# Dave-he/unet-watermark

Hardware: AMD Instinct MI355X
Metric: train_images_per_sec (higher is better)
Workload: dtype f32 storage and accumulation; the convolution products of the encoder and decoder layers (3x3, 7x7 stem, stride-2 and 1x1 layers: forward, data gradients, and the weight gradients of the stride-1 3x3 layers and the stem) as fp16x3 splits - every fp32 operand = two fp16 halves (22 mantissa bits), a*b; 1 GPU; Unet-resnet34 512x512 bs16/GPU train step: fwd + Dice + bwd + Adam (BASELINE.json configs[1]); global_batch=16, parallelism=dp1, grad_allreduce=none

## Files before the change

include/uwm.h:

```cpp
#ifndef UWM_H
#define UWM_H
#include <stddef.h>
#include <stdint.h>

#ifdef __cplusplus
extern "C" {
#endif

typedef struct uwm_model* uwm_handle;
typedef void* uwm_stream;

enum { UWM_ENC_RESNET18 = 18, UWM_ENC_RESNET34 = 34, UWM_ENC_RESNET50 = 50,
       UWM_ENC_EFFICIENTNET_B0 = 100, UWM_ENC_EFFICIENTNET_B1 = 101, UWM_ENC_EFFICIENTNET_B2 = 102,
       UWM_ENC_EFFICIENTNET_B3 = 103, UWM_ENC_EFFICIENTNET_B4 = 104, UWM_ENC_EFFICIENTNET_B5 = 105,
       UWM_ENC_EFFICIENTNET_B6 = 106, UWM_ENC_EFFICIENTNET_B7 = 107 };
enum { UWM_ARCH_UNET = 0, UWM_ARCH_UNETPLUSPLUS = 1 };
enum { UWM_T_F32 = 0, UWM_T_I64 = 1, UWM_T_U8 = 2, UWM_T_I32 = 3 };
enum { UWM_KIND_CONV_W = 0, UWM_KIND_BIAS = 1, UWM_KIND_BN_GAMMA = 2, UWM_KIND_BN_BETA = 3,
       UWM_KIND_BN_MEAN = 4, UWM_KIND_BN_VAR = 5 };
enum { UWM_ARENA_PARAM = 0, UWM_ARENA_BUFFER = 1 };
enum { UWM_PREC_F32 = 0, UWM_PREC_BF16X3 = 1, UWM_PREC_BF16X3_ALL = 2, UWM_PREC_F16X3 = 3, UWM_PREC_F16X3_ALL = 4,
       UWM_PREC_F16X1 = 5, UWM_PREC_F16X3_BWD2 = 6 };

typedef struct {
// ... 96 lines not shown
                            uwm_stream stream);
int  uwm_set_winograd(int on);
int  uwm_set_winograd_mode(uwm_handle h, int mode);
int  uwm_get_winograd_mode(uwm_handle h);
int  uwm_set_precision(uwm_handle h, int mode);
int  uwm_get_precision(uwm_handle h);
int  uwm_set_precision_fill(uwm_handle h, int min_workgroups);
int  uwm_set_routing_batch(uwm_handle h, int batch);
int  uwm_routing_enable(uwm_handle h, int on);
long long uwm_routing_dump(uwm_handle h, char* buf, long long cap, int clear);
int  uwm_set_drop_connect(uwm_handle h, const float* rowscale);
int  uwm_op_depthwise(int mode, const float* a, const float* b, int k, int stride, int pad_begin, int N, int H, int W, int C,
                      int Ho, int Wo, const float* addend, float* out, float* scratch, uwm_stream stream);
long long uwm_op_depthwise_scratch_floats(int k, int N, int C, int Ho, int Wo);
int  uwm_num_mbconv_blocks(uwm_handle h);
float uwm_mbconv_drop_rate(uwm_handle h, int block);
int  uwm_resize_threshold(const float* logits, int ld, int N, int h, int w, int H, int W, float threshold,
                          int apply_sigmoid, uint8_t* mask, float* resized, uwm_stream stream);

enum { UWM_MASK_WATERMARK = 0, UWM_MASK_TEXT = 1, UWM_MASK_MIXED = 2 };
enum { UWM_MORPH_RECT = 0, UWM_MORPH_ELLIPSE = 2 };
int    uwm_mask_element(int shape, int kw, int kh, uint8_t* out);
size_t uwm_mask_workspace_bytes(int N, int H, int W);
int    uwm_optimize_mask(const uint8_t* in, uint8_t* out, int N, int H, int W, int mask_type, long long* summary,
                         void* workspace, size_t workspace_bytes, uwm_stream stream);
int    uwm_op_morph(const uint8_t* in, uint8_t* out, int N, int H, int W, int dilate, int shape, int kw, int kh,
                    int iterations, void* workspace, size_t workspace_bytes, uwm_stream stream);
int    uwm_op_components(const uint8_t* in, int32_t* labels ,
                         int32_t* areas , int N, int H, int W,
                         void* workspace, size_t workspace_bytes, uwm_stream stream);

int  uwm_set_side_stream(uwm_handle h, int on);

int  uwm_prof_enable(int on);
int  uwm_prof_collect(double* out, int max_classes);
const char* uwm_prof_class_name(int cls);

int  uwm_debug_lookup(uwm_handle h, const char* key, long long* offset, long long* count);

typedef struct {
  const float* ptr; const float* scale; const float* shift;
  int C, H, W, up, relu;
} uwm_src;
int  uwm_op_preprocess_u8_nhwc4(const uint8_t* images, long long npix, int C, const float* mean, const float* std, float* out,
                                uwm_stream stream);
int  uwm_op_set_igemm_f16x3(int on);
int  uwm_op_conv(const uwm_src* s0, const uwm_src* s1, const float* w, int wrows, int Kpad, int kh, int kw, int stride,
                 int pad, int N, int Cout, const float* bias, float* y, double* stats, int cfg, uwm_stream stream);
int  uwm_op_dgrad(const float* dy, int N, int Ho, int Wo, int Cout, const float* wd, int Cin, int KpadD, int kh, int kw,
                  int stride, int pad, int H, int W, const float* addend, const float* mask, const float* mscale,
                  const float* mshift, float* dx, uwm_stream stream);
int  uwm_op_wgrad(const uwm_src* s0, const uwm_src* s1, const float* dy, int N, int Ho, int Wo, int Cout, int wrows,
                  int Kpad, int kh, int kw, int stride, int pad, float* dw, int force_igemm, uwm_stream stream);
int  uwm_op_pack_dgrad(const float* w, int Cout, int Kpad, int ntaps, int Cin, float* wd, int KpadD, int CoutP,
                       uwm_stream stream);
int  uwm_op_maxpool(const uwm_src* in, int N, float* out, uint8_t* idx, uwm_stream stream);
int  uwm_op_maxpool_backward(const float* gout, const uint8_t* idx, const float* addend, const uwm_src* in, int N,
                             float* gin, uwm_stream stream);
int  uwm_op_bn_backward(const float* g, const float* y, const float* mean, const float* rstd, const float* gamma,
                        double* scratch2c, float* dy, float* dgamma, float* dbeta, long long npix, int C, uwm_stream stream);
int  uwm_op_bn_backward_act(const float* g, const float* y, const float* mean, const float* rstd, const float* gamma,
                            const float* scale, const float* shift, const float* se_s, const float* gpool, int N, long long hw,
                            int C, double* scratch2c, float* dy, float* dgamma, float* dbeta, float* xmax, uwm_stream stream);
int  uwm_op_dgrad_upsplit(const float* dy, int N, int H, int W, int Cout, const float* wd, int C0, int C1, int KpadD,
                          float* gprev, const float* pmask, const float* pscale, const float* pshift, float* gskip,
                          uwm_stream stream);
int  uwm_op_upsplit(const float* dcat, int N, int H, int W, int C0, int C1, float* gprev, const float* pmask,
                    const float* pscale, const float* pshift, float* gskip, uwm_stream stream);
int  uwm_op_residual(const float* y, const float* s2, const float* b2, const float* id, const float* sd, const float* bd,
                     float* out, long long npix, int C, uwm_stream stream);

#ifdef __cplusplus
}
#endif
#endif
```

unet-watermark_amd/_lib.py:

```python
from __future__ import annotations

import ctypes as C
import os
import subprocess
import sys
from pathlib import Path

os.environ.setdefault("GPU_MAX_HW_QUEUES", "8")

_PKG_DIR = Path(__file__).resolve().parent
_CSRC = _PKG_DIR / "csrc"
LIB_PATH = _PKG_DIR / "libuwm.so"
SOURCES = ["conv_igemm.hip", "conv_patch.hip", "conv_patch16.hip", "conv_wino.hip", "conv_wino8.hip", "conv_wino_x3.hip", "conv_f16x3.hip", "conv_f16x3v2.hip", "conv_stem_f16x3.hip", "conv_up2.hip", "conv_up2_f16.hip", "conv_c16_f16.hip", "conv_gemm.hip", "conv_head.hip", "mbconv.hip", "wgrad_igemm.hip", "wgrad_patch.hip", "wgrad_wino.hip", "wgrad_f16x3.hip", "wgrad_c16.hip", "wgrad_gemm.hip", "wgrad_stem.hip", "elementwise.hip", "loss.hip", "mask_post.hip", "uwm_model.hip"]
HIP_ARCH = "gfx950"
EXTRA_FLAGS = {name: ["-Xclang", "-target-feature", "-Xclang", "-packed-fp32-ops"]
               for name in ("conv_f16x3.hip", "conv_f16x3v2.hip", "wgrad_f16x3.hip", "conv_stem_f16x3.hip")}


class uwm_unet_desc(C.Structure):
    _fields_ = [("encoder", C.c_int), ("in_channels", C.c_int), ("classes", C.c_int),
                ("decoder_channels", C.c_int * 5), ("bn_eps", C.c_float), ("bn_momentum", C.c_float), ("arch", C.c_int)]


class uwm_tensor_info(C.Structure):
# ... 49 lines not shown
    "uwm_adam_clip": (I, [P, P, P, P, L, F, F, F, F, F, L, F, F, P, P]),
    "uwm_adam_graph": (I, [P, P, P, P, L, P, P, P]),
    "uwm_adamw": (I, [P, P, P, P, L, F, F, F, F, F, L, F, P]),
    "uwm_adamw_clip": (I, [P, P, P, P, L, F, F, F, F, F, L, F, F, P, P]),
    "uwm_adamw_graph": (I, [P, P, P, P, L, P, P, P]),
    "uwm_sgd": (I, [P, P, P, L, F, F, F, L, F, F, P, P]),
    "uwm_scale": (I, [P, L, F, P]),
    "uwm_set_winograd": (I, [I]),
    "uwm_set_winograd_mode": (I, [P, I]),
    "uwm_get_winograd_mode": (I, [P]),
    "uwm_set_precision": (I, [P, I]),
    "uwm_get_precision": (I, [P]),
    "uwm_set_precision_fill": (I, [P, I]),
    "uwm_set_routing_batch": (I, [P, I]),
    "uwm_routing_enable": (I, [P, I]),
    "uwm_routing_dump": (L, [P, C.c_char_p, L, I]),
    "uwm_allreduce_grads": (I, [P, P, I, I, P]),
    "uwm_grad_arena": (P, [P]),
    "uwm_set_join_stream": (I, [P, P]),
    "uwm_set_drop_connect": (I, [P, P]),
    "uwm_op_depthwise": (I, [I, P, P, I, I, I, I, I, I, I, I, I, P, P, P, P]),
    "uwm_op_depthwise_scratch_floats": (L, [I, I, I, I, I]),
    "uwm_num_mbconv_blocks": (I, [P]),
    "uwm_mbconv_drop_rate": (F, [P, I]),
    "uwm_preprocess_u8": (I, [P, I, I, I, I, C.POINTER(C.c_float), C.POINTER(C.c_float), P, P, P]),
    "uwm_preprocess_mask_u8": (I, [P, I, I, I, I, P, P, P]),
    "uwm_resize_threshold": (I, [P, I, I, I, I, I, I, F, I, P, P, P]),
    "uwm_mask_element": (I, [I, I, I, P]),
    "uwm_mask_workspace_bytes": (Z, [I, I, I]),
    "uwm_optimize_mask": (I, [P, P, I, I, I, I, P, P, Z, P]),
    "uwm_op_morph": (I, [P, P, I, I, I, I, I, I, I, I, P, Z, P]),
    "uwm_op_components": (I, [P, P, P, I, I, I, P, Z, P]),
    "uwm_set_side_stream": (I, [P, I]),
    "uwm_prof_enable": (I, [I]),
    "uwm_prof_collect": (I, [C.POINTER(C.c_double), I]),
    "uwm_prof_class_name": (C.c_char_p, [I]),
    "uwm_debug_lookup": (I, [P, C.c_char_p, C.POINTER(L), C.POINTER(L)]),
    "uwm_op_set_igemm_f16x3": (I, [I]),
    "uwm_op_conv": (I, [C.POINTER(uwm_src), C.POINTER(uwm_src), P, I, I, I, I, I, I, I, I, P, P, P, I, P]),
    "uwm_op_dgrad": (I, [P, I, I, I, I, P, I, I, I, I, I, I, I, I, P, P, P, P, P, P]),
    "uwm_op_wgrad": (I, [C.POINTER(uwm_src), C.POINTER(uwm_src), P, I, I, I, I, I, I, I, I, I, I, P, I, P]),
    "uwm_op_pack_dgrad": (I, [P, I, I, I, I, P, I, I, P]),
    "uwm_op_maxpool": (I, [C.POINTER(uwm_src), I, P, P, P]),
    "uwm_op_maxpool_backward": (I, [P, P, P, C.POINTER(uwm_src), I, P, P]),
    "uwm_op_bn_backward": (I, [P, P, P, P, P, P, P, P, P, L, I, P]),
    "uwm_op_bn_backward_act": (I, [P, P, P, P, P, P, P, P, P, I, L, I, P, P, P, P, P, P]),
    "uwm_op_dgrad_upsplit": (I, [P, I, I, I, I, P, I, I, I, P, P, P, P, P, P]),
    "uwm_op_upsplit": (I, [P, I, I, I, I, I, P, P, P, P, P, P]),
    "uwm_op_residual": (I, [P, P, P, P, P, P, P, L, I, P]),
}

_lib = None


def build_library(force: bool = False, verbose: bool = False) -> Path:
    srcs = [_CSRC / s for s in SOURCES]
    hdrs = [_CSRC / "uwm_kernels.h", _PKG_DIR.parent / "include" / "uwm.h"] + sorted(_CSRC.glob("*.inc"))
    if LIB_PATH.exists() and not force:
        newest = max(p.stat().st_mtime for p in srcs + hdrs)
        if LIB_PATH.stat().st_mtime >= newest:
            return LIB_PATH
    hipcc = os.environ.get("HIPCC", "/opt/rocm/bin/hipcc")
    objdir = _PKG_DIR / "build"
    objdir.mkdir(exist_ok=True)
    procs = []
    hdr_m = max(p.stat().st_mtime for p in hdrs + [Path(__file__)])
    for s in srcs:
        o = objdir / (s.stem + ".o")
        if not force and o.exists() and o.stat().st_mtime >= max(s.stat().st_mtime, hdr_m):
            procs.append((None, None, o))
            continue
        cmd = [hipcc, f"--offload-arch={HIP_ARCH}", "-O3", "-std=c++17", "-fPIC"] + EXTRA_FLAGS.get(s.name, []) + ["-c", str(s), "-o", str(o)]
        procs.append((cmd, subprocess.Popen(cmd, stdout=subprocess.PIPE, stderr=subprocess.STDOUT), o))
    objs = []
    for cmd, p, o in procs:
        if p is None:
            objs.append(str(o))
            continue
        out, _ = p.communicate()
        if p.returncode != 0:
            raise RuntimeError(f"hipcc failed: {' '.join(cmd)}\n{out.decode(errors='replace')}")
        if verbose and out:
            sys.stderr.write(out.decode(errors="replace"))
        objs.append(str(o))
    cmd = [hipcc, f"--offload-arch={HIP_ARCH}", "-shared", "-fPIC", "-o", str(LIB_PATH)] + objs
    r = subprocess.run(cmd, stdout=subprocess.PIPE, stderr=subprocess.STDOUT)
    if r.returncode != 0:
        raise RuntimeError(f"link failed: {' '.join(cmd)}\n{r.stdout.decode(errors='replace')}")
    return LIB_PATH


def lib():
    global _lib
    if _lib is not None:
        return _lib
    global LIB_PATH
    if os.environ.get("UWM_LIB"):
        LIB_PATH = Path(os.environ["UWM_LIB"])
    if not LIB_PATH.exists():
        raise RuntimeError(
            f"{LIB_PATH} not found: the HIP extension is not built. Run `python -c 'import __graft_entry__ as g; "
            f"g.build()'` (needs hipcc). There is no CPU fallback for this path.")
    try:
        h = C.CDLL(str(LIB_PATH))
    except OSError as e:
        raise RuntimeError(f"cannot load {LIB_PATH}: {e}") from e
    for name, (res, args) in SIGNATURES.items():
        fn = getattr(h, name)
        fn.restype = res
        fn.argtypes = args
    _lib = h
    return _lib


def check(rc: int, exc=RuntimeError):
    if rc != 0:
        msg = lib().uwm_last_error().decode(errors="replace")
        raise exc(msg)


def stream_ptr(device=None) -> int:
    import torch
    return torch.cuda.current_stream(device).cuda_stream


class _NoGuard:
    def __enter__(self):
        return self

    def __exit__(self, *a):
        return False


_NOGUARD = _NoGuard()


def on_device(t):
    import torch
    if t.device.type == "cuda" and t.device.index is not None and t.device.index != torch.cuda.current_device():
        return torch.cuda.device(t.device)
# ... 15 lines not shown
```

unet-watermark_amd/csrc/conv_f16x3.hip:

```cpp
#include "uwm_kernels.h"

namespace uwm {

typedef float f4 __attribute__((ext_vector_type(4)));
typedef _Float16 h8 __attribute__((ext_vector_type(8)));
typedef _Float16 h4 __attribute__((ext_vector_type(4)));

#ifndef UWM_F16_ABL
#define UWM_F16_ABL 0
#endif
constexpr int kFT = 16, kFP = kFT + 2, kFPP = kFP * kFP;
constexpr int kFPix = 40;
constexpr int kFBuf = kFPP * kFPix;
constexpr int kFKs = 5;
constexpr int kFRounds = (kFPP * 4 + 255) / 256;

__host__ __device__ inline int f16x3_nj_(int rows) { return ((rows + 63) / 64) * 4; }
int f16x3_nj(int rows) { return f16x3_nj_(rows); }
size_t f16x3_bank_floats(int rows, int chans) {
  const size_t halfs = (size_t)(chans / 16) * kFKs * f16x3_nj(rows) * 2 * 64 * 8;
  return halfs / 2 + (size_t)f16x3_nj(rows) * 16;
}
size_t f16x3_rinv_off(int rows, int chans) { return f16x3_rinv_off_floats(rows, chans); }

// ... 110 lines not shown
      const int by = b >> 3, bx = b & 7;
      const int y = row0 + 2 * by, x = 2 * bx;
      const int ho = hb + y, wo = wb + x;
      if (ho < a.Ho && wo < a.Wo) {
        const float* q = R + (y * 16 + x) * kQLd + cq * 4;
        f4 v = (*(const f4*)q + *(const f4*)(q + kQLd) + *(const f4*)(q + 16 * kQLd) + *(const f4*)(q + 17 * kQLd)) * rs;
        const size_t o2 = (((size_t)n * (a.Ho >> 1) + (ho >> 1)) * (a.Wo >> 1) + (wo >> 1)) * a.up_c0 + co;
        if (a.up_mask) {
          f4 mk = *(const f4*)(a.up_mask + o2);
          const f4 yr = mk;
          if (a.up_mscale) mk = mk * msc + msh;
          v.x = mk.x > 0.f ? v.x : 0.f; v.y = mk.y > 0.f ? v.y : 0.f;
          v.z = mk.z > 0.f ? v.z : 0.f; v.w = mk.w > 0.f ? v.w : 0.f;
          if (bnb) { ps_ += v; pq_ += v * ((yr - bmu) * brs); }
        }
        if (a.up_accum) v += *(const f4*)(a.out_up + o2);
        *(f4*)(a.out_up + o2) = v;
      }
    }
  } else {
    const int c1n = a.Cout - a.up_c0;
#pragma unroll 4
    for (int r = 0; r < NROWS * 4; ++r) {
      const int p = r * 4 + sub;
      const int y = row0 + (p >> 4), x = p & 15;
      const int ho = hb + y, wo = wb + x;
      if (ho < a.Ho && wo < a.Wo)
        *(f4*)(a.out + (((size_t)n * a.Ho + ho) * a.Wo + wo) * c1n + (co - a.up_c0)) = *(const f4*)(R + (y * 16 + x) * kQLd + cq * 4) * rs;
    }
  }
}

__device__ __forceinline__ float clamp_h(float v) { return __builtin_amdgcn_fmed3f(v, -65504.f, 65504.f); }

template <int NJ, int NP = 3>
__global__ __launch_bounds__(256, (NJ == 1 ? 4 : 2)) void conv_f16x3_kernel(const ConvArgs a) {
  constexpr bool kOne = NJ == 1;
  constexpr int kCo = 16 * NJ;
  constexpr int kCQ = 4 * NJ, kSub = 64 / kCQ;
  extern __shared__ __attribute__((aligned(16))) _Float16 hsm[];

  const int tid = threadIdx.x, lane = tid & 63, wave = __builtin_amdgcn_readfirstlane(tid >> 6);
  const int px16 = lane & 15, g = lane >> 4;

  const unsigned nblk = gridDim.x, bid = blockIdx.x;
  const unsigned q8 = nblk >> 3, r8 = nblk & 7, xcd = bid & 7;
  unsigned tile = (xcd < r8 ? xcd * (q8 + 1) : r8 * (q8 + 1) + (xcd - r8) * q8) + (bid >> 3);
  const int tilesN = (a.Cout + kCo - 1) / kCo;
  const int tilesW = (a.Wo + kFT - 1) / kFT, tilesH = (a.Ho + kFT - 1) / kFT;
  const int tn = tile % tilesN; tile /= tilesN;
  const int tw = tile % tilesW; tile /= tilesW;
  const int th = tile % tilesH; const int n = tile / tilesH;
  const int n0 = tn * kCo, h0 = th * kFT, w0 = tw * kFT;
  const int nJ = a.wu_ncb;

  f4 acc[4][NJ];
#pragma unroll
  for (int i = 0; i < 4; ++i)
#pragma unroll
    for (int j = 0; j < NJ; ++j) acc[i][j] = (f4){0.f, 0.f, 0.f, 0.f};

  int goff[kFRounds];
  unsigned gflags = 0;
  int* const goff_s1 = (int*)(hsm + 2 * kFBuf);
#pragma unroll
  for (int rd = 0; rd < kFRounds; ++rd) {
    const int u = rd * 256 + tid;
    const bool act = u < kFPP * 4;
    const int pp = act ? (u >> 2) : 0;
    const int py = pp / kFP, pxx = pp - py * kFP;
    const int hl = h0 - 1 + py, wl = w0 - 1 + pxx;
    const bool ok = act && hl >= 0 && hl < a.Hl && wl >= 0 && wl < a.Wl;
    const int hc = min(max(hl, 0), a.Hl - 1), wc = min(max(wl, 0), a.Wl - 1);
    goff[rd] = ((n * a.s0.H + (hc >> a.s0.up)) * a.s0.W + (wc >> a.s0.up)) * a.s0.C;
    if (!kOne && a.C0 < a.Ctot) goff_s1[rd * 256 + tid] = ((n * a.s1.H + (hc >> a.s1.up)) * a.s1.W + (wc >> a.s1.up)) * a.s1.C;
    gflags |= (ok ? 1u : 0u) << rd;
  }
  float xs = 1.f;
  if (a.xmax) {
    float mx = a.xmax[lane & 31];
#pragma unroll
    for (int d = 16; d >= 1; d >>= 1) mx = fmaxf(mx, __shfl_xor(mx, d));
    if (mx > 0.f && mx < 3.0e38f) { int e; (void)frexpf(mx, &e); xs = ldexpf(1.f, 14 - e); }
  }
  constexpr int kWR = kFRounds - 1;
  f4 pv[kWR], pvX = {0.f, 0.f, 0.f, 0.f}, psc = {1.f, 1.f, 1.f, 1.f}, psh = {0.f, 0.f, 0.f, 0.f};
  float pfloor = -3.0e38f;
  const bool has_x = tid < kFPP * 4 - kWR * 256;
  const float* lsp = nullptr;
  auto chunk_src = [&](int cc) {
    const int c = cc * 16;
    const bool first = c < a.C0;
    if (c == a.C0 && a.C0 < a.Ctot) {
#pragma unroll
      for (int rd = 0; rd < kFRounds; ++rd) goff[rd] = goff_s1[rd * 256 + tid];
    }
    lsp = (first ? a.s0.ptr : a.s1.ptr) + (first ? c : c - a.C0) + (tid & 3) * 4;
  };
  auto coef_load = [&](int cc) {
    const int c = cc * 16;
    const bool first = c < a.C0;
    const Src& s = first ? a.s0 : a.s1;
    const int cl = (first ? c : c - a.C0) + (tid & 3) * 4;
    pfloor = s.relu ? 0.f : -3.0e38f;
    if (s.scale != nullptr) { psc = *(const f4*)(s.scale + cl); psh = *(const f4*)(s.shift + cl); }
    else { psc = (f4){1.f, 1.f, 1.f, 1.f}; psh = (f4){0.f, 0.f, 0.f, 0.f}; pfloor = -3.0e38f; }
  };
  auto store_unit = [&](int buf, int rd, f4 raw) {
    f4 v = raw * psc + psh;
    v.x = fmaxf(v.x, pfloor); v.y = fmaxf(v.y, pfloor); v.z = fmaxf(v.z, pfloor); v.w = fmaxf(v.w, pfloor);
    v = v * xs;
    if (!((gflags >> rd) & 1u)) v = (f4){0.f, 0.f, 0.f, 0.f};
    h4 hi, lo;
#pragma unroll
    for (int e = 0; e < 4; ++e) {
      const float x = clamp_h(v[e]);
      const _Float16 h = (_Float16)x;
      hi[e] = h; lo[e] = (_Float16)(x - (float)h);
    }
    const int u = rd * 256 + tid;
    _Float16* d = hsm + buf * kFBuf + (u >> 2) * kFPix + (u & 3) * 4;
    *(h4*)d = hi;
    *(h4*)(d + 16) = lo;
  };

  const _Float16* const wb = (const _Float16*)a.wu + (size_t)(n0 / 16) * 1024 + lane * 8;
  const int nchunk = a.Ctot >> 4, nsteps = nchunk * kFKs;
  constexpr int dbg = UWM_F16_ABL;
  auto w_load = [&](int t, h8 (&whi)[NJ], h8 (&wlo)[NJ]) {
    if ((dbg & 2) && t > 0) return;
    const _Float16* p = wb + (size_t)t * nJ * 1024;
#pragma unroll
    for (int j = 0; j < NJ; ++j) { whi[j] = *(const h8*)(p + j * 1024); wlo[j] = *(const h8*)(p + j * 1024 + 512); }
  };
  const int pbase = ((wave * 4) * kFP + px16) * kFPix + (g & 1) * 8;
  const int ghi = g >> 1;
  auto mma_step = [&](int ks, const _Float16* pc, const h8 (&whi)[NJ], const h8 (&wlo)[NJ]) {
    const int slot0 = 2 * ks, slot1 = 2 * ks + 1 > 8 ? 8 : 2 * ks + 1;
    const int off0 = ((slot0 / 3) * kFP + slot0 % 3) * kFPix, off1 = ((slot1 / 3) * kFP + slot1 % 3) * kFPix;
    const _Float16* pp = pc + pbase + (ghi ? off1 : off0);
    h8 xh[4], xl[4];
#pragma unroll
    for (int i = 0; i < 4; ++i) {
      if (dbg & 4) { xh[i] = whi[i % NJ]; xl[i] = wlo[i % NJ]; continue; }
      xh[i] = *(const h8*)(pp + i * kFP * kFPix); xl[i] = *(const h8*)(pp + i * kFP * kFPix + 16);
    }
    if (dbg & 1) { acc[0][0][0] += (float)xh[0][0] + (float)xl[1][1] + (float)whi[NJ > 1 ? NJ - 2 : 0][2] + (float)wlo[NJ - 1][3] + (float)xh[2][0] + (float)xh[3][0]; return; }
#pragma unroll
    for (int i = 0; i < 4; ++i)
#pragma unroll
      for (int j = 0; j < NJ; ++j) acc[i][j] = __builtin_amdgcn_mfma_f32_16x16x32_f16(whi[j], xh[i], acc[i][j], 0, 0, 0);
    if (NP >= 3) {
#pragma unroll
      for (int i = 0; i < 4; ++i)
#pragma unroll
        for (int j = 0; j < NJ; ++j) acc[i][j] = __builtin_amdgcn_mfma_f32_16x16x32_f16(whi[j], xl[i], acc[i][j], 0, 0, 0);
    }
    if (NP >= 2) {
#pragma unroll
      for (int i = 0; i < 4; ++i)
#pragma unroll
        for (int j = 0; j < NJ; ++j) acc[i][j] = __builtin_amdgcn_mfma_f32_16x16x32_f16(wlo[j], xh[i], acc[i][j], 0, 0, 0);
    }
  };

  h8 wA_hi[NJ], wA_lo[NJ], wB_hi[NJ], wB_lo[NJ];
  w_load(0, wA_hi, wA_lo);
  chunk_src(0);
#pragma unroll
  for (int rd = 0; rd < kWR; ++rd) pv[rd] = *(const f4*)(lsp + goff[rd]);
  if (has_x) pvX = *(const f4*)(lsp + goff[kWR]);
  coef_load(0);
#pragma unroll
  for (int rd = 0; rd < kWR; ++rd) store_unit(0, rd, pv[rd]);
  if (has_x) store_unit(0, kWR, pvX);
  if (!kOne && nchunk > 1) {
    chunk_src(1);
#pragma unroll
    for (int rd = 0; rd < kWR; ++rd) pv[rd] = *(const f4*)(lsp + goff[rd]);
    if (has_x) pvX = *(const f4*)(lsp + goff[kWR]);
  }
  __syncthreads();

  for (int cc = 0; cc < nchunk; cc += 2) {
#pragma unroll
    for (int hh = 0; hh < (kOne ? 1 : 2); ++hh) {
      const int c = cc + hh, cur = hh, nxt = hh ^ 1;
      const bool more1 = c + 1 < nchunk;
      if (!kOne) {
        coef_load(more1 ? c + 1 : c);
        chunk_src(c + 2 < nchunk ? c + 2 : nchunk - 1);
      }
      const _Float16* pc = hsm + cur * kFBuf;
      __builtin_amdgcn_sched_barrier(0);
#pragma unroll
      for (int ks = 0; ks < kFKs; ++ks) {
        const int t = c * kFKs + ks;
        const int tnext = t + 1 < nsteps ? t + 1 : t;
        if (((hh * kFKs + ks) & 1) == 0) { w_load(tnext, wB_hi, wB_lo); mma_step(ks, pc, wA_hi, wA_lo); }
        else { w_load(tnext, wA_hi, wA_lo); mma_step(ks, pc, wB_hi, wB_lo); }
        if (!(dbg & 8) && !kOne) {
          store_unit(nxt, ks, pv[ks]);
          pv[ks] = *(const f4*)(lsp + goff[ks]);
        }
        __builtin_amdgcn_sched_group_barrier(0x020, 2 * NJ, 0);
        __builtin_amdgcn_sched_group_barrier(0x100, 8, 0);
#pragma unroll
        for (int q = 0; q < 4 * NJ; ++q) {
          __builtin_amdgcn_sched_group_barrier(0x008, NP, 0);
          __builtin_amdgcn_sched_group_barrier(0x002, 3, 0);
        }
        __builtin_amdgcn_sched_group_barrier(0x200, 2, 0);
        __builtin_amdgcn_sched_group_barrier(0x020, 1, 0);
        __builtin_amdgcn_sched_barrier(0);
      }
      if (!(dbg & 8) && !kOne && has_x) {
        if (more1) store_unit(nxt, kWR, pvX);
        pvX = *(const f4*)(lsp + goff[kWR]);
      }
      __syncthreads();
    }
  }
  if (dbg & 16) { if (acc[0][0][0] + acc[1][1][1] + acc[2][NJ > 1 ? NJ - 2 : 0][2] + acc[3][NJ - 1][3] == 123.456f) a.out[0] = 1.f; return; }

  constexpr int kQLd = kOne ? 20 : 68;
  float* const R = (float*)hsm + wave * 64 * kQLd;
#pragma unroll
  for (int i = 0; i < 4; ++i)
#pragma unroll
    for (int j = 0; j < NJ; ++j) *(f4*)(R + (i * 16 + px16) * kQLd + j * 16 + g * 4) = acc[i][j];
  __syncthreads();
  const float* rinv = (const float*)a.wu + a.wu_rinv_off;
  const float ixs = 1.f / xs;
  const bool do_stats = a.ssum != nullptr;
  const bool bnb = a.bnb_mean != nullptr;
  const int cq = lane & (kCQ - 1), sub = lane / kCQ;
  const int co = n0 + cq * 4;
  const bool cok = co < a.Cout;
  f4 ps_ = {0.f, 0.f, 0.f, 0.f}, pq_ = ps_;
  const int stat_c = a.out_up != nullptr ? a.up_c0 : a.Cout;
  if (NJ == 4 && a.out_up != nullptr) {
    f4 rs = {0.f, 0.f, 0.f, 0.f};
    if (cok) rs = *(const f4*)(rinv + co) * ixs;
    f16x3_split_epilogue<4>(a, R, kQLd, 0, n, h0 + wave * 4, w0, n0, lane, rs, ps_, pq_);
  } else {
    f4 rs = {0.f, 0.f, 0.f, 0.f}, bmu = rs, brs = rs, bia = rs, msc = {1.f, 1.f, 1.f, 1.f}, msh = rs;
    if (cok) rs = *(const f4*)(rinv + co) * ixs;
    if (bnb && cok) { bmu = *(const f4*)(a.bnb_mean + co); brs = *(const f4*)(a.bnb_rstd + co); }
    if (a.bias && cok) bia = *(const f4*)(a.bias + co);
    if (a.mscale && cok) { msc = *(const f4*)(a.mscale + co); msh = *(const f4*)(a.mshift + co); }
#pragma unroll 4
    for (int r = 0; r < 64 / kSub; ++r) {
      const int p = r * kSub + sub;
      const int ho = h0 + wave * 4 + (p >> 4), wo = w0 + (p & 15);
      if (ho < a.Ho && wo < a.Wo && cok) {
        const size_t o = (((size_t)n * a.Ho + ho) * a.Wo + wo) * a.Cout + co;
        f4 v = *(const f4*)(R + p * kQLd + cq * 4) * rs + bia;
        if (a.addend) v += *(const f4*)(a.addend + o);
        f4 yr = {0.f, 0.f, 0.f, 0.f};
        if (a.mask) {
          f4 mk = *(const f4*)(a.mask + o);
          yr = mk;
          if (a.mscale) mk = mk * msc + msh;
          v.x = mk.x > 0.f ? v.x : 0.f; v.y = mk.y > 0.f ? v.y : 0.f;
          v.z = mk.z > 0.f ? v.z : 0.f; v.w = mk.w > 0.f ? v.w : 0.f;
        }
        *(f4*)(a.out + o) = v;
        if (a.bnb_y) yr = *(const f4*)(a.bnb_y + o);
        ps_ += v; pq_ += bnb ? v * ((yr - bmu) * brs) : v * v;
      }
    }
  }
  if (do_stats) {
#pragma unroll
    for (int e = 0; e < 4; ++e) {
      float sv = ps_[e], qv = pq_[e];
#pragma unroll
      for (int d = kCQ; d < 64; d <<= 1) { sv += __shfl_xor(sv, d); qv += __shfl_xor(qv, d); }
      ps_[e] = sv; pq_[e] = qv;
    }
    __syncthreads();
    float* red = (float*)hsm;
    if (sub == 0) {
#pragma unroll
      for (int e = 0; e < 4; ++e) { red[(wave * 64 + cq * 4 + e) * 2] = ps_[e]; red[(wave * 64 + cq * 4 + e) * 2 + 1] = pq_[e]; }
    }
    __syncthreads();
    if (tid < kCo) {
      const int c1 = n0 + tid;
      if (c1 < stat_c) {
        double sv = 0.0, qv = 0.0;
#pragma unroll
        for (int w = 0; w < 4; ++w) { sv += (double)red[(w * 64 + tid) * 2]; qv += (double)red[(w * 64 + tid) * 2 + 1]; }
        const size_t srep_off = a.srep > 1 ? (size_t)(blockIdx.x & (unsigned)(a.srep - 1)) * a.sstride : 0;
        atomicAdd(a.ssum + srep_off + c1, sv);
        atomicAdd(a.ssq + srep_off + c1, qv);
      }
    }
  }
}

template <int NP = 3>
__global__ __launch_bounds__(512, 1) void conv_f16x3s_kernel(const ConvArgs a) {
  extern __shared__ __attribute__((aligned(16))) _Float16 hsm[];

  const int tid = threadIdx.x, lane = tid & 63, wave = __builtin_amdgcn_readfirstlane(tid >> 6);
  const bool is_mma = wave < 4;
  const int mw = wave & 3;
  const int ltid = tid & 255;
  const int px16 = lane & 15, g = lane >> 4;

  const unsigned nblk = gridDim.x, bid = blockIdx.x;
  const unsigned q8 = nblk >> 3, r8 = nblk & 7, xcd = bid & 7;
  unsigned tile = (xcd < r8 ? xcd * (q8 + 1) : r8 * (q8 + 1) + (xcd - r8) * q8) + (bid >> 3);
  const int tilesN = (a.Cout + 63) / 64;
  const int tilesW = (a.Wo + kFT - 1) / kFT, tilesH = (a.Ho + kFT - 1) / kFT;
  const int tn = tile % tilesN; tile /= tilesN;
  const int tw = tile % tilesW; tile /= tilesW;
  const int th = tile % tilesH; const int n = tile / tilesH;
  const int n0 = tn * 64, h0 = th * kFT, w0 = tw * kFT;
  const int nJ = a.wu_ncb;
  const int nchunk = a.Ctot >> 4, nsteps = nchunk * kFKs;

  float xs = 1.f;
  if (a.xmax) {
    float mx = a.xmax[lane & 31];
#pragma unroll
    for (int d = 16; d >= 1; d >>= 1) mx = fmaxf(mx, __shfl_xor(mx, d));
    if (mx > 0.f && mx < 3.0e38f) { int e; (void)frexpf(mx, &e); xs = ldexpf(1.f, 14 - e); }
  }

  f4 acc[4][4];
#pragma unroll
  for (int i = 0; i < 4; ++i)
#pragma unroll
    for (int j = 0; j < 4; ++j) acc[i][j] = (f4){0.f, 0.f, 0.f, 0.f};

  if (!is_mma) {
    int goff0[kFRounds], goff1[kFRounds];
    unsigned gflags = 0;
#pragma unroll
    for (int rd = 0; rd < kFRounds; ++rd) {
      const int u = rd * 256 + ltid;
      const bool act = u < kFPP * 4;
      const int pp = act ? (u >> 2) : 0;
      const int py = pp / kFP, pxx = pp - py * kFP;
      const int hl = h0 - 1 + py, wl = w0 - 1 + pxx;
      const bool ok = act && hl >= 0 && hl < a.Hl && wl >= 0 && wl < a.Wl;
      const int hc = min(max(hl, 0), a.Hl - 1), wc = min(max(wl, 0), a.Wl - 1);
      goff0[rd] = ((n * a.s0.H + (hc >> a.s0.up)) * a.s0.W + (wc >> a.s0.up)) * a.s0.C;
      goff1[rd] = a.C0 < a.Ctot ? ((n * a.s1.H + (hc >> a.s1.up)) * a.s1.W + (wc >> a.s1.up)) * a.s1.C : goff0[rd];
      gflags |= ((ok ? 1u : 0u) | (act ? 2u : 0u)) << (2 * rd);
    }
    struct Stage { f4 pv[kFRounds]; f4 sc, sh; int relu; bool has; };
    auto patch_load = [&](int cc, Stage& st) {
      const int c = cc * 16;
      const bool first = c < a.C0;
      const Src& s = first ? a.s0 : a.s1;
      st.relu = s.relu;
      const int cl = (first ? c : c - a.C0) + (ltid & 3) * 4;
      st.has = s.scale != nullptr;
      if (st.has) { st.sc = *(const f4*)(s.scale + cl); st.sh = *(const f4*)(s.shift + cl); }
      const float* sp = s.ptr + cl;
#pragma unroll
      for (int rd = 0; rd < kFRounds; ++rd) st.pv[rd] = *(const f4*)(sp + (first ? goff0[rd] : goff1[rd]));
    };
    auto patch_store = [&](int buf, const Stage& st) {
#pragma unroll
      for (int rd = 0; rd < kFRounds; ++rd) {
        f4 v = st.pv[rd];
        if (st.has) {
          v = v * st.sc + st.sh;
          if (st.relu) { v.x = fmaxf(v.x, 0.f); v.y = fmaxf(v.y, 0.f); v.z = fmaxf(v.z, 0.f); v.w = fmaxf(v.w, 0.f); }
        }
        v = v * xs;
        if (!((gflags >> (2 * rd)) & 1u)) v = (f4){0.f, 0.f, 0.f, 0.f};
        if ((gflags >> (2 * rd)) & 2u) {
          h4 hi, lo;
#pragma unroll
          for (int e = 0; e < 4; ++e) {
            const float x = clamp_h(v[e]);
            const _Float16 h = (_Float16)x;
            hi[e] = h; lo[e] = (_Float16)(x - (float)h);
          }
          const int u = rd * 256 + ltid;
          _Float16* d = hsm + buf * kFBuf + (u >> 2) * kFPix + (u & 3) * 4;
          *(h4*)d = hi;
          *(h4*)(d + 16) = lo;
        }
      }
    };
    Stage sA, sB;
    patch_load(0, sA);
    patch_load(nchunk > 1 ? 1 : 0, sB);
    patch_store(0, sA);
    __syncthreads();
    for (int cc = 0; cc < nchunk; cc += 2) {
      {
        const int c2 = cc + 2 < nchunk ? cc + 2 : nchunk - 1;
        if (cc + 1 < nchunk) patch_store(1, sB);
        patch_load(c2, sA);
        __syncthreads();
      }
      {
        const int c3 = cc + 3 < nchunk ? cc + 3 : nchunk - 1;
        if (cc + 2 < nchunk) patch_store(0, sA);
        patch_load(c3, sB);
        __syncthreads();
      }
    }
  } else {
    const _Float16* const wb = (const _Float16*)a.wu + (size_t)(n0 / 16) * 1024 + lane * 8;
    auto w_load = [&](int t, h8 (&whi)[4], h8 (&wlo)[4]) {
      const _Float16* p = wb + (size_t)t * nJ * 1024;
#pragma unroll
      for (int j = 0; j < 4; ++j) { whi[j] = *(const h8*)(p + j * 1024); wlo[j] = *(const h8*)(p + j * 1024 + 512); }
    };
    const int pbase = ((mw * 4) * kFP + px16) * kFPix + (g & 1) * 8;
    const int ghi = g >> 1;
    auto x_load = [&](int ks, const _Float16* pc, h8 (&xh)[4], h8 (&xl)[4]) {
      const int slot0 = 2 * ks, slot1 = 2 * ks + 1 > 8 ? 8 : 2 * ks + 1;
      const int off0 = ((slot0 / 3) * kFP + slot0 % 3) * kFPix, off1 = ((slot1 / 3) * kFP + slot1 % 3) * kFPix;
      const _Float16* pp = pc + pbase + (ghi ? off1 : off0);
#pragma unroll
      for (int i = 0; i < 4; ++i) { xh[i] = *(const h8*)(pp + i * kFP * kFPix); xl[i] = *(const h8*)(pp + i * kFP * kFPix + 16); }
    };
    auto mma = [&](const h8 (&whi)[4], const h8 (&wlo)[4], const h8 (&xh)[4], const h8 (&xl)[4]) {
#pragma unroll
      for (int i = 0; i < 4; ++i)
#pragma unroll
        for (int j = 0; j < 4; ++j) acc[i][j] = __builtin_amdgcn_mfma_f32_16x16x32_f16(whi[j], xh[i], acc[i][j], 0, 0, 0);
      if (NP >= 3) {
#pragma unroll
        for (int i = 0; i < 4; ++i)
#pragma unroll
          for (int j = 0; j < 4; ++j) acc[i][j] = __builtin_amdgcn_mfma_f32_16x16x32_f16(whi[j], xl[i], acc[i][j], 0, 0, 0);
      }
      if (NP >= 2) {
#pragma unroll
        for (int i = 0; i < 4; ++i)
// ... 12 lines not shown
#pragma unroll
        for (int ks = 0; ks < kFKs; ++ks) {
          const int t = c * kFKs + ks;
          const int tnext = t + 1 < nsteps ? t + 1 : t;
          x_load(ks, pc, xh, xl);
          if (((hh * kFKs + ks) & 1) == 0) { w_load(tnext, wB_hi, wB_lo); __builtin_amdgcn_sched_barrier(0); mma(wA_hi, wA_lo, xh, xl); }
          else { w_load(tnext, wA_hi, wA_lo); __builtin_amdgcn_sched_barrier(0); mma(wB_hi, wB_lo, xh, xl); }
          __builtin_amdgcn_sched_barrier(0);
        }
        __syncthreads();
      }
    }
  }

  constexpr int kQLd = 68;
  if (is_mma) {
    float* const Rw = (float*)hsm + mw * 64 * kQLd;
#pragma unroll
    for (int i = 0; i < 4; ++i)
#pragma unroll
      for (int j = 0; j < 4; ++j) *(f4*)(Rw + (i * 16 + px16) * kQLd + j * 16 + g * 4) = acc[i][j];
  }
  __syncthreads();
  const float* const R = (const float*)hsm + mw * 64 * kQLd;
  const float* rinv = (const float*)a.wu + a.wu_rinv_off;
  const float ixs = 1.f / xs;
  const bool do_stats = a.ssum != nullptr;
  const bool bnb = a.bnb_mean != nullptr;
  const int cq = lane & 15, sub = lane >> 4;
  const int co = n0 + cq * 4;
  const bool cok = co < a.Cout;
  const int phalf = (wave >> 2) * 32;
  f4 ps_ = {0.f, 0.f, 0.f, 0.f}, pq_ = ps_;
  const int stat_c = a.out_up != nullptr ? a.up_c0 : a.Cout;
  if (a.out_up != nullptr) {
    f4 rs = {0.f, 0.f, 0.f, 0.f};
    if (cok) rs = *(const f4*)(rinv + co) * ixs;
    f16x3_split_epilogue<2>(a, R, kQLd, phalf >> 4, n, h0 + mw * 4, w0, n0, lane, rs, ps_, pq_);
  } else {
    f4 rs = {0.f, 0.f, 0.f, 0.f}, bmu = rs, brs = rs, bia = rs, msc = {1.f, 1.f, 1.f, 1.f}, msh = rs;
    if (cok) rs = *(const f4*)(rinv + co) * ixs;
    if (bnb && cok) { bmu = *(const f4*)(a.bnb_mean + co); brs = *(const f4*)(a.bnb_rstd + co); }
    if (a.bias && cok) bia = *(const f4*)(a.bias + co);
    if (a.mscale && cok) { msc = *(const f4*)(a.mscale + co); msh = *(const f4*)(a.mshift + co); }
#pragma unroll 4
    for (int r = 0; r < 8; ++r) {
      const int p = phalf + r * 4 + sub;
      const int ho = h0 + mw * 4 + (p >> 4), wo = w0 + (p & 15);
      if (ho < a.Ho && wo < a.Wo && cok) {
        const size_t o = (((size_t)n * a.Ho + ho) * a.Wo + wo) * a.Cout + co;
        f4 v = *(const f4*)(R + p * kQLd + cq * 4) * rs + bia;
        if (a.addend) v += *(const f4*)(a.addend + o);
        f4 yr = {0.f, 0.f, 0.f, 0.f};
        if (a.mask) {
          f4 mk = *(const f4*)(a.mask + o);
          yr = mk;
          if (a.mscale) mk = mk * msc + msh;
          v.x = mk.x > 0.f ? v.x : 0.f; v.y = mk.y > 0.f ? v.y : 0.f;
          v.z = mk.z > 0.f ? v.z : 0.f; v.w = mk.w > 0.f ? v.w : 0.f;
        }
        *(f4*)(a.out + o) = v;
        if (a.bnb_y) yr = *(const f4*)(a.bnb_y + o);
        ps_ += v; pq_ += bnb ? v * ((yr - bmu) * brs) : v * v;
      }
    }
  }
  if (do_stats) {
#pragma unroll
    for (int e = 0; e < 4; ++e) {
      float sv = ps_[e], qv = pq_[e];
      sv += __shfl_xor(sv, 16); qv += __shfl_xor(qv, 16);
      sv += __shfl_xor(sv, 32); qv += __shfl_xor(qv, 32);
      ps_[e] = sv; pq_[e] = qv;
    }
    __syncthreads();
    float* red = (float*)hsm;
    if (sub == 0) {
#pragma unroll
      for (int e = 0; e < 4; ++e) { red[(wave * 64 + cq * 4 + e) * 2] = ps_[e]; red[(wave * 64 + cq * 4 + e) * 2 + 1] = pq_[e]; }
    }
    __syncthreads();
    if (tid < 64) {
      const int c1 = n0 + tid;
      if (c1 < stat_c) {
        double sv = 0.0, qv = 0.0;
#pragma unroll
        for (int w = 0; w < 8; ++w) { sv += (double)red[(w * 64 + tid) * 2]; qv += (double)red[(w * 64 + tid) * 2 + 1]; }
        const size_t srep_off = a.srep > 1 ? (size_t)(blockIdx.x & (unsigned)(a.srep - 1)) * a.sstride : 0;
        atomicAdd(a.ssum + srep_off + c1, sv);
        atomicAdd(a.ssq + srep_off + c1, qv);
      }
    }
  }
}

bool conv_f16x3_applicable(const ConvArgs& a) {
  return a.wu != nullptr && a.ntaps == 9 && a.kw == 3 && a.smul == 1 && a.sdiv == 1 && (a.rmul == 1 ? a.off == -1 : a.off == 1) &&
         ((a.Ctot & 31) == 0 || (a.Ctot == 16 && a.C0 == 16 && a.Cout <= 16 && !a.out_up)) && (a.C0 & 15) == 0 && (a.s0.C & 3) == 0 && (a.s1.C & 3) == 0 && (a.Cout & 3) == 0 && a.Cout >= 16 &&
         a.Hl == a.Ho && a.Wl == a.Wo && a.Ho >= 8 && a.Wo >= 16 && a.Hl < 32768 && a.Wl < 32768 &&
         (!a.out_up || (((a.Ho | a.Wo) & 1) == 0 && (a.up_c0 & 63) == 0 && a.up_c0 <= a.Cout)) &&
         (size_t)a.N * a.s0.H * a.s0.W * a.s0.C < (1ull << 31) && (size_t)a.N * a.s1.H * a.s1.W * a.s1.C < (1ull << 31);
}

template <int NJ, int NP>
static hipError_t launch_f3(const ConvArgs& a, hipStream_t st, dim3 grid, size_t lds) {
  static DevOnce lds_attr;
  { hipError_t e = lds_attr.set_max_lds((const void*)conv_f16x3_kernel<NJ, NP>, lds); if (e != hipSuccess) return e; }
  UWM_LAUNCH(42, a.flops, a.bytes, (conv_f16x3_kernel<NJ, NP>), grid, dim3(256), lds, st, a);
  return hipGetLastError();
}
template <int NP>
static hipError_t launch_f3s(const ConvArgs& a, hipStream_t st, dim3 grid, size_t lds) {
  static DevOnce lds_attr;
  { hipError_t e = lds_attr.set_max_lds((const void*)conv_f16x3s_kernel<NP>, lds); if (e != hipSuccess) return e; }
  UWM_LAUNCH(42, a.flops, a.bytes, (conv_f16x3s_kernel<NP>), grid, dim3(512), lds, st, a);
  return hipGetLastError();
}
hipError_t launch_conv_f16x3(const ConvArgs& a, hipStream_t st, int variant) {
  if (a.wu_layout == 1) return launch_conv_f16x3v2(a, st, variant >= 4 ? variant : 0);
  if (variant >= 4) return hipErrorInvalidValue;
  if (!conv_f16x3_applicable(a)) return hipErrorInvalidValue;
  if (a.out_up && (a.addend || a.mask || a.bias || a.bnb_y || (a.ssum && !a.bnb_mean) || (a.up_c0 < a.Cout && !a.out))) return hipErrorInvalidValue;
  if (a.bnb_mean && (!a.ssum || !a.ssq || !a.bnb_rstd || !(a.out_up ? a.up_mask : (a.bnb_y ? a.bnb_y : a.mask)) || a.up_accum)) return hipErrorInvalidValue;
  const int tilesN = (a.Cout + 63) / 64;
  const int tilesW = (a.Wo + kFT - 1) / kFT, tilesH = (a.Ho + kFT - 1) / kFT;
  const size_t main_lds = (size_t)2 * kFBuf * sizeof(_Float16) + 6 * 256 * sizeof(int), q_lds = (size_t)4 * 64 * 68 * sizeof(float);
  const size_t lds = main_lds > q_lds ? main_lds : q_lds;
  static const bool force4 = dbg_flag("UWM_F16X3_4WAVE"), force8 = dbg_flag("UWM_F16X3_8WAVE");
  const long wgs = (long)route_N(a) * tilesH * tilesW * tilesN;
  const int np = (a.nprod >= 1 && a.nprod <= 3) ? a.nprod : 3;
  if (a.Ctot == 16) {
    const size_t lds1 = (size_t)kFBuf * sizeof(_Float16);
    return np == 3 ? launch_f3<1, 3>(a, st, dim3((unsigned)(a.N * tilesH * tilesW)), lds1)
         : np == 2 ? launch_f3<1, 2>(a, st, dim3((unsigned)(a.N * tilesH * tilesW)), lds1) : launch_f3<1, 1>(a, st, dim3((unsigned)(a.N * tilesH * tilesW)), lds1);
  }
  const bool four = variant == 1 || variant == 3 || (variant != 2 && (force4 || (!force8 && wgs >= 2L * device_cu_count())));
  if (variant == 3 && a.out_up) return hipErrorInvalidValue;
  const bool fwd_alone = a.rmul == 1 && !a.xmax;
  const bool narrow = !a.out_up && (a.Cout <= 32 ? four : (fwd_alone && variant == 0 && wgs < device_cu_count()));
  if (variant == 3 || (variant == 0 && narrow)) {
    const dim3 g((unsigned)(a.N * tilesH * tilesW * ((a.Cout + 31) / 32)));
    return np == 3 ? launch_f3<2, 3>(a, st, g, lds) : np == 2 ? launch_f3<2, 2>(a, st, g, lds) : launch_f3<2, 1>(a, st, g, lds);
  }
  const dim3 g((unsigned)(a.N * tilesH * tilesW * tilesN));
  if (four) return np == 3 ? launch_f3<4, 3>(a, st, g, lds) : np == 2 ? launch_f3<4, 2>(a, st, g, lds) : launch_f3<4, 1>(a, st, g, lds);
  return np == 3 ? launch_f3s<3>(a, st, g, lds) : np == 2 ? launch_f3s<2>(a, st, g, lds) : launch_f3s<1>(a, st, g, lds);
}

}
```

unet-watermark_amd/csrc/conv_igemm.hip:

```cpp
#include "uwm_kernels.h"
#include <cstdlib>
#include <cstdio>

namespace uwm {

typedef float f4 __attribute__((ext_vector_type(4)));

__device__ __forceinline__ unsigned fdiv(unsigned n, FastDiv f) {
  return f.d <= 1 ? n : __umulhi(n, f.mg);
}

constexpr float kIgWScale = 4096.f;
typedef _Float16 ig_h8 __attribute__((ext_vector_type(8)));
template <int BM, int BN, int WM, int WN, bool PC = false, bool F16 = false>
__global__ __launch_bounds__(256, 2) void conv_igemm_kernel(const ConvArgs a) {
  constexpr int MI = BM / WM / 16;
  constexpr int NI = BN / WN / 16;
  constexpr int XR = BM / 32;
  constexpr int WR = (BN + 31) / 32;
  static_assert(WM * WN == 4, "4 waves");
  extern __shared__ __attribute__((aligned(16))) float smem[];
  float* const Xs = smem;
  float* const Ws = smem + 2 * BM * 32;

// ... 332 lines not shown
  int dev = 0; (void)hipGetDevice(&dev);
  if (dev < 0 || dev >= 64) return 256;
  if (!cus[dev] && (hipDeviceGetAttribute(&cus[dev], hipDeviceAttributeMultiprocessorCount, dev) != hipSuccess || cus[dev] <= 0)) cus[dev] = 256;
  return cus[dev];
}

bool conv_epilogue_carries_bnb(const ConvArgs& a) {
  if (a.ig16 && a.prec != 2 && (conv_c16_f16_applicable(a) || conv_c32_f16_applicable(a))) return true;
  if (a.prec == 2) return !a.out_up && (a.wu_layout == 1 ? conv_f16x3v2_applicable(a) : conv_f16x3_applicable(a));
  if (a.bnb_y) {
    if (a.out_up || a.prec == 1) return false;
    static const bool no_y = dbg_flag("UWM_NO_BNB_Y");
    if (no_y || conv_up2_applicable(a) || conv_head_applicable(a) || conv_head_dgrad_applicable(a) || conv_patch16_applicable(a)) return false;
    if (wino_mode_of(a.wino) != 0 && conv_wino_applicable(a)) return true;
    return !conv_patch_applicable(a);
  }
  static const bool no_up2 = dbg_flag("UWM_NO_UP2");
  if (a.out_up) return (!no_up2 && conv_up2_dgrad_applicable(a)) || (a.prec == 1 ? conv_wino_x3_applicable(a) : conv_wino_applicable(a));
  static const bool no_head = dbg_flag("UWM_NO_CONV_HEAD");
  if (!no_up2 && conv_up2_applicable(a)) return false;
  if (!no_head && conv_head_applicable(a)) return false;
  if (!no_head && conv_head_dgrad_applicable(a)) return true;
  if (wino_mode_of(a.wino) != 0 && conv_wino_applicable(a) && !conv_patch16_applicable(a))
    return a.prec == 1 || !conv_wino8_applicable(a);
  if (conv_patch16_applicable(a)) return true;
  if (conv_patch_applicable(a)) return false;
  static const bool no_igemm_bnb = dbg_flag("UWM_NO_IGEMM_BNB");
  return !no_igemm_bnb;
}

hipError_t launch_conv(const ConvArgs& a, hipStream_t st, int force_cfg) {
  if (a.M <= 0 || a.Cout <= 0 || (a.Cout & 3) || (a.Kpad & 31) || (a.Ctot & 3) || (a.C0 & 3)) return hipErrorInvalidValue;
  int cfg = force_cfg;
  static const bool trace = dbg_flag("UWM_TRACE_CONV");
  if (trace)
    fprintf(stderr, "conv %s N=%d Ctot=%d(C0=%d up=%d) Cout=%d Ho=%d Wo=%d Hl=%d Wl=%d taps=%d smul=%d sdiv=%d wino=%d gflop=%.2f\n",
            a.rmul < 0 ? "dgrad" : "fwd", a.N, a.Ctot, a.C0, a.s0.up, a.Cout, a.Ho, a.Wo, a.Hl, a.Wl, a.ntaps, a.smul, a.sdiv,
            (int)(cfg < 0 && wino_mode_of(a.wino) != 0 && conv_wino_applicable(a)), a.flops * 1e-9);
  if (cfg == 700) return launch_conv_up2(a, st);
  if (cfg == 710 || (cfg < 0 && a.ig16 && a.prec != 2 && conv_c16_f16_applicable(a))) return launch_conv_c16_f16(a, st);
  if (cfg == 711 || (cfg < 0 && a.ig16 && a.prec != 2 && conv_c32_f16_applicable(a))) return launch_conv_c32_f16(a, st);
  if (cfg >= 800 && cfg < 1000) return launch_conv_gemm(a, st, cfg - 800);
  if (cfg == 500) return launch_conv_head(a, st);
  if ((cfg >= 600 && cfg <= 607) || (cfg < 0 && a.prec == 2)) return launch_conv_f16x3(a, st, cfg >= 600 ? cfg - 600 : 0);
  if (cfg == 400) return launch_conv_wino_x3(a, st);
  if (cfg >= 300) return launch_conv_wino(a, st, cfg - 300);
  if (a.out_up) {
    static const bool no_up2d = dbg_flag("UWM_NO_UP2");
    if (cfg < 0 && !no_up2d && conv_up2_dgrad_applicable(a)) return launch_conv_up2_dgrad(a, st);
    if (a.prec == 1) return launch_conv_wino_x3(a, st);
    return conv_wino_applicable(a) ? launch_conv_wino(a, st) : hipErrorInvalidValue;
  }
  if (cfg == 200) return launch_conv_patch16(a, st);
  static const bool no_up2 = dbg_flag("UWM_NO_UP2");
  if (cfg < 0 && !no_up2 && conv_up2_applicable(a)) return launch_conv_up2(a, st);
  static const bool no_head = dbg_flag("UWM_NO_CONV_HEAD");
  if (cfg < 0 && !no_head && conv_head_applicable(a)) return launch_conv_head(a, st);
  if (cfg < 0 && !no_head && conv_head_dgrad_applicable(a)) return launch_conv_head_dgrad(a, st);
  if (cfg < 0 && wino_mode_of(a.wino) != 0 && conv_wino_applicable(a) && !conv_patch16_applicable(a))
    return a.prec == 1 ? launch_conv_wino_x3(a, st) : launch_conv_wino(a, st);
  if (cfg >= 100) return launch_conv_patch(a, st, cfg - 100);
  if (cfg < 0 && conv_patch16_applicable(a)) return launch_conv_patch16(a, st);
  if (cfg < 0 && conv_patch_applicable(a)) {
    const long sp = (long)route_N(a) * ((a.Ho + 7) / 8) * ((a.Wo + 15) / 16);
    int bn = a.Cout >= 128 ? 128 : (a.Cout > 32 ? 64 : (a.Cout > 16 ? 32 : 16));
    if (bn == 128 && sp * ((a.Cout + 127) / 128) < 512) bn = 64;
// ... 37 lines not shown
```

unet-watermark_amd/csrc/elementwise.hip:

```cpp
#include "uwm_kernels.h"
#include <vector>
#include <mutex>
#include <cstdlib>

namespace uwm {

typedef float f4 __attribute__((ext_vector_type(4)));
static constexpr int kMaxBlocks = 256 * 8;

static inline unsigned nblocks(size_t work, int per_block) {
  size_t b = (work + per_block - 1) / per_block;
  if (b > (size_t)kMaxBlocks) b = kMaxBlocks;
  if (b < 1) b = 1;
  return (unsigned)b;
}

__global__ void nchw_to_nhwc4_kernel(const float* __restrict__ x, float* __restrict__ y, int C, size_t HW,
                                     size_t total, int CP) {
  for (size_t i = blockIdx.x * (size_t)blockDim.x + threadIdx.x; i < total; i += (size_t)gridDim.x * blockDim.x) {
    const size_t n = i / HW, p = i - n * HW;
    const float* xp = x + n * C * HW + p;
    float* yp = y + i * CP;
    for (int c0 = 0; c0 < CP; c0 += 4) {
      f4 v;
// ... 354 lines not shown
    if (xmax) amax4(o);
    *(f4*)(dy + i * 4) = o;
  }
  if (xmax) {
#pragma unroll
    for (int d = 32; d >= 1; d >>= 1) amax = fmaxf(amax, __shfl_xor(amax, d));
    if ((threadIdx.x & 63) == 0) wmax[threadIdx.x >> 6] = amax;
    __syncthreads();
    if (threadIdx.x == 0) {
      const float mx = fmaxf(fmaxf(wmax[0], wmax[1]), fmaxf(wmax[2], wmax[3]));
      if (mx > 0.f) atomicMax((unsigned*)xmax + (blockIdx.x & 31), __float_as_uint(mx));
    }
  }
}
hipError_t launch_bn_bwd_apply(const float* g, const float* y, const float* mean, const float* rstd, const float* gamma,
                               const double* dgamma, const double* dbeta, float* dy, float* gamma_grad, float* beta_grad,
                               size_t npix, int C, hipStream_t st, const double* rep, int nrep, int rep_stride, hipEvent_t done, float* xmax) {
  const size_t n4 = npix * C / 4;
  unsigned nb = nblocks(n4, 256 * 4);
  const unsigned q = (unsigned)(C / 4);
  unsigned unit = q;
  { unsigned a = q, b = 256; while (b) { unsigned t = a % b; a = b; b = t; } unit = q / a; }
  nb = ((nb + unit - 1) / unit) * unit;
  if ((size_t)nb * 256 < q) nb = ((q + 255) / 256 + unit - 1) / unit * unit;
  if (done)
    hipExtLaunchKernelGGL(bn_bwd_apply_kernel, dim3(nb), dim3(256), 0, st, nullptr, done, 0, g, y, mean, rstd, gamma, dgamma,
                          dbeta, dy, gamma_grad, beta_grad, n4, C, (float)(1.0 / (double)npix), rep, rep ? (nrep < 1 ? 1 : nrep) : 0, rep_stride, xmax);
  else
    hipLaunchKernelGGL(bn_bwd_apply_kernel, dim3(nb), dim3(256), 0, st, g, y, mean, rstd, gamma, dgamma,
                       dbeta, dy, gamma_grad, beta_grad, n4, C, (float)(1.0 / (double)npix), rep, rep ? (nrep < 1 ? 1 : nrep) : 0, rep_stride, xmax);
  return hipGetLastError();
}

__global__ void upsplit_prev_kernel(const float* __restrict__ dcat, int H, int W, int C0, int Ct, float* __restrict__ gprev,
                                    const float* __restrict__ pmask, const float* __restrict__ pscale,
                                    const float* __restrict__ pshift, size_t total, int accumulate) {
  const int C4 = C0 / 4, H2 = H / 2, W2 = W / 2;
  for (size_t i = blockIdx.x * (size_t)blockDim.x + threadIdx.x; i < total; i += (size_t)gridDim.x * blockDim.x) {
    const int c = (int)(i % C4) * 4;
    size_t p = i / C4;
    const int w2 = (int)(p % W2); p /= W2;
    const int h2 = (int)(p % H2); const int n = (int)(p / H2);
    const float* b = dcat + ((size_t)((size_t)n * H + 2 * h2) * W + 2 * w2) * Ct + c;
    f4 g = *(const f4*)b + *(const f4*)(b + Ct) + *(const f4*)(b + (size_t)W * Ct) + *(const f4*)(b + (size_t)W * Ct + Ct);
    if (pmask) {
      f4 z = *(const f4*)(pmask + i * 4);
      if (pscale) z = z * *(const f4*)(pscale + c) + *(const f4*)(pshift + c);
      g.x = z.x > 0.f ? g.x : 0.f; g.y = z.y > 0.f ? g.y : 0.f; g.z = z.z > 0.f ? g.z : 0.f; g.w = z.w > 0.f ? g.w : 0.f;
    }
    if (accumulate) g += *(const f4*)(gprev + i * 4);
    *(f4*)(gprev + i * 4) = g;
  }
}
__global__ void upsplit_skip_kernel(const float* __restrict__ dcat, int C0, int C1, float* __restrict__ gskip, size_t total) {
  const int C4 = C1 / 4, Ct = C0 + C1;
  for (size_t i = blockIdx.x * (size_t)blockDim.x + threadIdx.x; i < total; i += (size_t)gridDim.x * blockDim.x) {
    const int c = (int)(i % C4) * 4;
    const size_t p = i / C4;
    *(f4*)(gskip + i * 4) = *(const f4*)(dcat + p * Ct + C0 + c);
  }
}
hipError_t launch_upsplit(const float* dcat, int N, int H, int W, int C0, int C1, float* gprev, const float* pmask,
                          const float* pscale, const float* pshift, float* gskip, hipStream_t st, int accumulate_prev) {
  const size_t t0 = (size_t)N * (H / 2) * (W / 2) * (C0 / 4);
  hipLaunchKernelGGL(upsplit_prev_kernel, dim3(nblocks(t0, 256)), dim3(256), 0, st, dcat, H, W, C0, C0 + C1, gprev, pmask,
                     pscale, pshift, t0, accumulate_prev);
// ... 427 lines not shown
```

unet-watermark_amd/csrc/uwm_abi.inc:

```
extern "C" {

const char* uwm_last_error(void) { return g_err; }
int uwm_version(void) { return 1; }

int uwm_create(const uwm_unet_desc* desc, uwm_handle* out) {
  if (!desc || !out) return fail("uwm_create: null argument");
  uwm_model* m = new uwm_model();
  m->desc = *desc;
  if (m->desc.bn_eps <= 0.f) m->desc.bn_eps = 1e-5f;
  if (m->desc.bn_momentum <= 0.f) m->desc.bn_momentum = 0.1f;
  if (build_model(m)) { delete m; return 1; }
  const char* e = getenv("UWM_SIDE_STREAM");
  m->use_side = e ? atoi(e) : 1;
  if (const char* pe = getenv("UWM_PRECISION")) {
    static const char* names[7] = {"f32", "bf16x3", "bf16x3_all", "f16x3", "f16x3_all", "f16x1", "f16x3_bwd2"};
    int found = -1;
    for (int i = 0; i < 7; ++i) if (!strcmp(pe, names[i]) || (pe[0] == '0' + i && !pe[1])) found = i;
    if (found < 0) { delete m; return fail("uwm_create: UWM_PRECISION=%s is not a precision mode (f32 | bf16x3 | bf16x3_all | f16x3 | f16x3_all | f16x1 | f16x3_bwd2 or 0..6)", pe); }
    m->prec = found; m->plan.prec = found; m->prec_from_env = found != UWM_PREC_F32;
  }
  if (const char* pf = getenv("UWM_F16X3_MIN_WGS")) m->f3_min_wgs = atoi(pf) > 0 ? atoi(pf) : 0;
  m->wino_mode = winograd_mode();
  m->plan.wino_mode = m->wino_mode;
  *out = m; return 0;
}
void uwm_destroy(uwm_handle h) {
  if (!h) return;
  if (h->ev_fork) (void)hipEventDestroy(h->ev_fork);
  if (h->ev_join) (void)hipEventDestroy(h->ev_join);
  if (h->ev_pack) (void)hipEventDestroy(h->ev_pack);
  if (h->ev_disp) (void)hipEventDestroy(h->ev_disp);
  if (h->side) (void)hipStreamDestroy(h->side);
  delete h;
}

long long uwm_param_arena_floats(uwm_handle h) { return h ? h->param_floats : 0; }
long long uwm_buffer_arena_floats(uwm_handle h) { return h ? h->buffer_floats : 0; }
long long uwm_param_count(uwm_handle h) { return h ? h->param_count : 0; }
int uwm_num_tensors(uwm_handle h) { return h ? (int)h->infos.size() : 0; }
int uwm_tensor_info_get(uwm_handle h, int i, uwm_tensor_info* out) {
  if (!h || !out || i < 0 || i >= (int)h->infos.size()) return fail("uwm_tensor_info_get: bad index %d", i);
  *out = h->infos[i]; return 0;
}
int uwm_logits_channels(uwm_handle h) { return h ? h->CP : 0; }
int uwm_num_stages(uwm_handle h) { return h ? h->nstages : 0; }
int uwm_stage_range(uwm_handle h, int stage, long long* b, long long* e) {
// ... 329 lines not shown
}
int uwm_op_components(const uint8_t* in, int32_t* labels, int32_t* areas, int N, int H, int W, void* ws, size_t ws_bytes,
                      uwm_stream stream) {
  if (!in || !labels || !areas) return fail("uwm_op_components: null argument");
  if (((uintptr_t)labels | (uintptr_t)areas) & 3) return fail("uwm_op_components: labels and areas must be 4-byte aligned");
  if (mask_shape_check("uwm_op_components", N, H, W, ws, ws_bytes)) return 1;
  LCHK(launch_mask_components(in, labels, areas, N, H, W, ws, (hipStream_t)stream));
  return 0;
}
int uwm_preprocess_u8(const uint8_t* images, int N, int H, int W, int C, const float* mean, const float* std, const int* flags,
                      float* out_nchw, uwm_stream stream) {
  if (!images || !mean || !std || !out_nchw || N < 1 || H < 1 || W < 1 || C < 1 || C > 4) return fail("uwm_preprocess_u8: bad argument");
  for (int c = 0; c < C; ++c) if (!(std[c] > 0.f)) return fail("uwm_preprocess_u8: std[%d] must be positive", c);
  LCHK(launch_preprocess_u8(images, N, H, W, C, mean, std, flags, out_nchw, (hipStream_t)stream));
  return 0;
}
int uwm_preprocess_mask_u8(const uint8_t* masks, int N, int H, int W, int threshold, const int* flags, uint8_t* out,
                           uwm_stream stream) {
  if (!masks || !out || N < 1 || H < 1 || W < 1) return fail("uwm_preprocess_mask_u8: bad argument");
  LCHK(launch_preprocess_mask(masks, N, H, W, threshold, flags, out, (hipStream_t)stream));
  return 0;
}
int uwm_scale(float* p, long long n, float s, uwm_stream stream) {
  if (!p || n < 1) return fail("uwm_scale: bad argument");
  LCHK(launch_scale(p, (size_t)n, s, (hipStream_t)stream));
  return 0;
}

int uwm_set_side_stream(uwm_handle h, int on) {
  if (!h) return fail("uwm_set_side_stream: null handle");
  h->use_side = on != 0; return 0;
}

int uwm_prof_enable(int on) { prof_enable(on != 0); return 0; }
int uwm_prof_collect(double* out, int max_classes) {
  if (!out || max_classes < kProfClasses) return fail("uwm_prof_collect: need room for %d classes (4 doubles each)", (int)kProfClasses);
  prof_collect(out); return kProfClasses;
}
const char* uwm_prof_class_name(int cls) { return prof_class_name(cls); }

int uwm_debug_lookup(uwm_handle h, const char* key, long long* off, long long* count) {
  if (!h || !key || !off || !count) return fail("uwm_debug_lookup: null argument");
  const Plan& p = h->plan;
  const std::string k(key);
  if (k == "fixed") { *off = 0; *count = (long long)h->fixed_floats; return 0; }
  if (k.rfind("bnf:", 0) == 0) {
    for (auto& b : h->bns) if (b.name == k.substr(4)) { *off = (long long)(b.f_off + 2 * (size_t)b.C); *count = 2LL * b.C; return 0; }
    return fail("uwm_debug_lookup: unknown BatchNorm %s", k.c_str() + 4);
  }
  if (k.rfind("wu:", 0) == 0 || k.rfind("wud:", 0) == 0 || k.rfind("wd:", 0) == 0) {
    const std::string name = k.substr(k.find(':') + 1);
    for (auto& cv : h->convs) if (cv.name == name) {
      if (k[1] == 'd') { *off = (long long)cv.wd_off; *count = cv.dgrad ? (long long)cv.CinP * cv.KpadD : 0; }
      else if (k[2] == 'd') { *off = (long long)cv.wud_off; *count = cv.wud_off ? (long long)std::max(wino_weights_floats(cv.CinP, cv.CoutP), cv.f3_d() ? f16x3_bank_floats(cv.CinP, cv.CoutP) : 0) : 0; }
      else { *off = (long long)cv.wu_off; *count = (long long)cv.wu_floats; }
      return 0;
    }
    return fail("uwm_debug_lookup: unknown conv %s", name.c_str());
  }
  if (p.N == 0) return fail("uwm_debug_lookup: no plan yet");
  const int N = p.N, H = p.H, W = p.W;
  auto conv_geo = [&](int ci, long long* cnt) { *cnt = (long long)N * p.oh[ci] * p.ow[ci] * h->convs[ci].CoutP; };
  if (k.rfind("y:", 0) == 0 || k.rfind("g:", 0) == 0) {
    const std::string name = k.substr(2);
    for (size_t i = 0; i < h->convs.size(); ++i) if (h->convs[i].name == name) {
      if ((int)i == h->head) return fail("uwm_debug_lookup: head output is the caller's logits buffer");
// ... 255 lines not shown
  if (!s0 || !dy || !dw) return fail("uwm_op_wgrad: null argument");
  WgradArgs a; memset(&a, 0, sizeof(a));
  a.s0 = to_src(s0); a.C0 = a.s0.C;
  if (s1) { a.s1 = to_src(s1); a.Ctot = a.C0 + a.s1.C; } else { a.s1 = a.s0; a.Ctot = a.C0; }
  a.dy = dy; a.dw = dw; a.wrows = wrows; a.Kpad = Kpad; a.ntaps = kh * kw; a.kw = kw;
  a.N = N; a.Ho = Ho; a.Wo = Wo; a.Cout = Cout; a.M = N * Ho * Wo;
  a.Hl = a.s0.H << a.s0.up; a.Wl = a.s0.W << a.s0.up; a.stride = stride; a.pad = pad;
  a.dv_ctot = make_fastdiv(a.Ctot); a.dv_kw = make_fastdiv(a.kw);
  a.force_igemm = force_igemm;
  if ((force_igemm & 0xff) == 6 || (force_igemm & 0xff) == 7) {
    static float* xm = nullptr;
    if (!xm) HIPCHK(hipMalloc((void**)&xm, 32 * sizeof(float)));
    LCHK(launch_absmax32(dy, (size_t)N * Ho * Wo * Cout, xm, (hipStream_t)stream));
    a.prec = 2; a.xmax = xm;
  }
  LCHK(launch_wgrad(a, (hipStream_t)stream));
  return 0;
}
int uwm_op_pack_dgrad(const float* w, int Cout, int Kpad, int ntaps, int Cin, float* wd, int KpadD, int CoutP,
                      uwm_stream stream) {
  if (!w || !wd) return fail("uwm_op_pack_dgrad: null argument");
  LCHK(launch_pack_dgrad(w, Cout, Kpad, ntaps, Cin, wd, KpadD, CoutP, (hipStream_t)stream));
  return 0;
}
int uwm_op_bn_backward(const float* g, const float* y, const float* mean, const float* rstd, const float* gamma,
                       double* scratch2c, float* dy, float* dgamma, float* dbeta, long long npix, int C, uwm_stream stream) {
  if (!g || !y || !mean || !rstd || !gamma || !scratch2c || !dy || !dgamma || !dbeta || npix < 1) return fail("uwm_op_bn_backward: bad argument");
  hipStream_t st = (hipStream_t)stream;
  HIPCHK(hipMemsetAsync(scratch2c, 0, 2 * (size_t)C * sizeof(double), st));
  LCHK(launch_bn_bwd_reduce(g, y, mean, rstd, scratch2c, scratch2c + C, (size_t)npix, C, st));
  LCHK(launch_bn_bwd_apply(g, y, mean, rstd, gamma, scratch2c, scratch2c + C, dy, dgamma, dbeta, (size_t)npix, C, st));
  return 0;
}
int uwm_op_bn_backward_act(const float* g, const float* y, const float* mean, const float* rstd, const float* gamma,
                           const float* scale, const float* shift, const float* se_s, const float* gpool, int N, long long hw,
                           int C, double* scratch2c, float* dy, float* dgamma, float* dbeta, float* xmax, uwm_stream stream) {
  if (!g || !y || !mean || !rstd || !gamma || !scale || !shift || !scratch2c || !dy || !dgamma || !dbeta || N < 1 || hw < 1 ||
      C < 4 || (C & 3) || (!se_s != !gpool))
    return fail("uwm_op_bn_backward_act: bad argument");
  hipStream_t st = (hipStream_t)stream;
  HIPCHK(hipMemsetAsync(scratch2c, 0, 2 * (size_t)C * sizeof(double), st));
  if (xmax) HIPCHK(hipMemsetAsync(xmax, 0, 32 * sizeof(float), st));
  LCHK(launch_bn_bwd_act(g, y, mean, rstd, gamma, scale, shift, se_s, gpool, N, (size_t)hw, scratch2c, scratch2c + C, dy, dgamma,
                         dbeta, C, st, xmax));
  return 0;
}
int uwm_op_upsplit(const float* dcat, int N, int H, int W, int C0, int C1, float* gprev, const float* pmask,
                   const float* pscale, const float* pshift, float* gskip, uwm_stream stream) {
  if (!dcat || !gprev) return fail("uwm_op_upsplit: null argument");
  LCHK(launch_upsplit(dcat, N, H, W, C0, C1, gprev, pmask, pscale, pshift, gskip, (hipStream_t)stream));
  return 0;
}
int uwm_op_residual(const float* y, const float* s2, const float* b2, const float* id, const float* sd, const float* bd,
                    float* out, long long npix, int C, uwm_stream stream) {
  if (!y || !s2 || !b2 || !id || !out) return fail("uwm_op_residual: null argument");
  LCHK(launch_residual(y, s2, b2, id, sd, bd, out, (size_t)npix, C, (hipStream_t)stream));
  return 0;
}
int uwm_op_maxpool_backward(const float* gout, const uint8_t* idx, const float* addend, const uwm_src* in, int N, float* gin,
                            uwm_stream stream) {
  if (!gout || !idx || !in || !gin) return fail("uwm_op_maxpool_backward: null argument");
  Src s = to_src(in);
  LCHK(launch_maxpool_bwd(gout, idx, addend, s, gin, N, (s.H - 1) / 2 + 1, (s.W - 1) / 2 + 1, (hipStream_t)stream));
  return 0;
}
int uwm_op_maxpool(const uwm_src* in, int N, float* out, uint8_t* idx, uwm_stream stream) {
// ... 8 lines not shown
```

unet-watermark_amd/csrc/uwm_backward.inc:

```
static int do_backward(uwm_model* m, const float* dlogits, float* ws, int sb, int se, hipStream_t st) {
  const Plan& p = m->plan;
  const int N = p.N, H = p.H, W = p.W;
  Ctx c{m, ws, st, N};
  c.wst = (m->use_side && m->side) ? m->side : st;
  const int h1 = H / 2, w1 = W / 2;
  int sh[4], sw[4];
  { int h = H / 4, w = W / 4; for (int s = 0; s < 4; ++s) { if (s > 0) { h /= 2; w /= 2; } sh[s] = h; sw[s] = w; } }
  std::vector<size_t> first_blk(4); { size_t b = 0; for (int s = 0; s < 4; ++s) { first_blk[s] = b; b += m->stages[s].size(); } }
  const bool effnet = !m->mb.empty();
  auto feat_blk = [&](int s) -> size_t { return effnet ? (size_t)m->feat_blk[s] : first_blk[s] + m->stages[s].size() - 1; };
  auto feat_src = [&](int s) {
    return mk_src(c.F(p.xn[feat_blk(s)]), m->featC[s], sh[s], sw[s]);
  };
  auto feat_mask = [&](const Src& f) -> const float* { return effnet ? nullptr : f.ptr; };
  Src f1 = effnet ? mk_src(c.F(p.stem_a), m->f1C, h1, w1) : lazy_src(c, m->stem, h1, w1);

  std::vector<char>& out_sums = m->out_sums;
  if (sb <= 0 || out_sums.size() != first_blk[3] + m->stages[3].size()) out_sums.assign(first_blk[3] + m->stages[3].size(), 0);
  if (sb <= 0 || m->dy_max_made.size() != m->bns.size()) m->dy_max_made.assign(m->bns.size(), 0);
  m->disp_cov.clear();
  if (sb <= 0) m->rq = ReduceQueue();
  if (sb <= 0 && se > 0) {
    HIPCHK(hipMemsetAsync(m->grads, 0, (size_t)m->param_floats * sizeof(float), st));
    HIPCHK(hipMemsetAsync(c.D(p.stat_d), 0, p.stat_d_count * sizeof(double), st));
    if (p.se_gs_floats) HIPCHK(hipMemsetAsync(c.F(p.se_gs_all), 0, p.se_gs_floats * sizeof(float), st));
    if (m->packed_in_fwd && m->pack_mode == pack_key(m)) {
      HIPCHK(hipStreamWaitEvent(st, m->ev_pack, 0));
      m->packed_in_fwd = false;
    } else {
      if (m->packed_in_fwd) { HIPCHK(hipStreamWaitEvent(st, m->ev_pack, 0)); m->packed_in_fwd = false; }
      for (size_t ci = 0; ci < m->convs.size(); ++ci) {
        const ConvL& cv = m->convs[ci];
        if (cv.dgrad && (!(cv.wud_off && p.wino_ok(ci)) || cv.CoutP == 16 || c16_f16_on(m, ci, true)))
          LCHK(launch_pack_dgrad(m->params + cv.w_off, cv.Cout, cv.Kpad, cv.k * cv.k, cv.CinP, c.F(cv.wd_off), cv.KpadD,
                                 cv.CoutP, st));
      }
      LCHK(wino_jobs(c, true, st));
    }
    const ConvL& hd = m->convs[m->head];
    const int last_c2 = m->nodes.empty() ? m->dec.back().c2 : m->nodes.back().c2;
    Src d4 = lazy_src(c, last_c2, H, W);
    LCHK(run_wgrad(c, m->head, d4, nullptr, dlogits, H, W));
    LCHK(launch_colsum(dlogits, (size_t)N * H * W, hd.CoutP, m->grads + hd.bias_off, (double*)c.F(p.colsum_scr), st));
    bool head_sums = false;
    LCHK(run_dgrad(c, m->head, dlogits, H, W, H, W, c.F(p.g[last_c2]), nullptr, d4.ptr, d4.scale, d4.shift, nullptr,
                   m->convs[last_c2].bn, &head_sums));
    int h = H, w = W;
    bool c2_sums = head_sums;
    for (int i = (int)m->dec.size() - 1; i >= 0; --i) {
      const DecL& dl = m->dec[i];
      const size_t npix = (size_t)N * h * w;
      LCHK(run_bn_bwd(c, dl.c2, c.F(p.g[dl.c2]), c.F(p.g[dl.c2]), npix, c2_sums));
// ... 209 lines not shown
```

unet-watermark_amd/csrc/uwm_kernels.h:

```cpp
#pragma once
#include <hip/hip_runtime.h>
#include <hip/hip_ext.h>
#include <stdint.h>
#include <stddef.h>
#include <atomic>

namespace uwm {

struct Src {
  const float* ptr;
  const float* scale;
  const float* shift;
  int C, H, W;
  int up;
  int relu;
};

struct FastDiv {
  unsigned mg, d;
};
static inline FastDiv make_fastdiv(unsigned d) {
  FastDiv f; f.d = d; f.mg = (d <= 1) ? 0u : (unsigned)((0x100000000ull / d) + 1ull); return f;
}

// ... 16 lines not shown
  Src s0, s1;
  int C0, Ctot;
  const float* w;
  int wrows, Kpad, ntaps, kw;
  int N, Ho, Wo, Cout, M;
  int Hl, Wl;
  int smul, rmul, off, sdiv;
  float* out;
  const float* bias;
  const float* addend;
  const float* mask;
  const float* mscale; const float* mshift;
  double* ssum; double* ssq;
  int srep, sstride;
  const float* bnb_mean; const float* bnb_rstd;
  const float* bnb_y;
  FastDiv dv_ctot, dv_kw;
  double flops;
  double bytes;
  float* out_up; int up_c0; const float* up_mask; const float* up_mscale; const float* up_mshift;
  int up_accum;
  int pc_ntaps[4]; unsigned pc_taps[4];
  int live_ch;
  const float* wu;
  int wu_ncb;
  int wino;
  int prec;
  int wu_rinv_off;
  const float* xmax;
  int route_n;
  int ig16;
  int nprod;
  int wu_layout;
};

template <class A> static inline int route_N(const A& a) { return a.route_n > 0 ? a.route_n : a.N; }
template <class A> static inline long route_M(const A& a) { return a.N > 0 ? (long)a.M / a.N * route_N(a) : (long)a.M; }

#if defined(__HIPCC__)
typedef unsigned uwm_u2 __attribute__((ext_vector_type(2)));
__device__ __forceinline__ void uwm_split4(float x0, float x1, float x2, float x3, uwm_u2& hi, uwm_u2& lo) {
  typedef _Float16 h2_ __attribute__((ext_vector_type(2)));
  const h2_ a = {(_Float16)x0, (_Float16)x1}, b = {(_Float16)x2, (_Float16)x3};
  hi.x = __builtin_bit_cast(unsigned, a); hi.y = __builtin_bit_cast(unsigned, b);
  unsigned l0, l1;
  asm("v_fma_mixlo_f16 %0, %1, -1.0, %2 op_sel_hi:[1,0,0]\n\t"
      "v_fma_mixhi_f16 %0, %1, -1.0, %3 op_sel:[1,0,0] op_sel_hi:[1,0,0]"
      : "=&v"(l0) : "v"(hi.x), "v"(x0), "v"(x1));
  asm("v_fma_mixlo_f16 %0, %1, -1.0, %2 op_sel_hi:[1,0,0]\n\t"
      "v_fma_mixhi_f16 %0, %1, -1.0, %3 op_sel:[1,0,0] op_sel_hi:[1,0,0]"
      : "=&v"(l1) : "v"(hi.y), "v"(x2), "v"(x3));
  lo.x = l0; lo.y = l1;
}
#endif

struct ReduceJob { const float* part; float* dw; unsigned long long n4; int nsplit; unsigned block0; };
struct ReduceQueue {
  enum { kMax = 48 };
  ReduceJob j[kMax]; int n = 0; unsigned blocks = 0; size_t used_floats = 0;
};
struct ReduceJobs { ReduceJob j[ReduceQueue::kMax]; int n; };

struct WgradArgs {
  Src s0, s1; int C0, Ctot;
  const float* dy;
  float* dw;
  int wrows, Kpad, ntaps, kw;
  int N, Ho, Wo, Cout, M;
  int Hl, Wl, stride, pad;
  int nsplit, msplit;
  float* part;
  size_t part_floats;
  int force_igemm;
  FastDiv dv_ctot, dv_kw;
  double flops;
  double bytes;
  int wino;
  int prec;
  const float* xmax;
  ReduceQueue* rq;
  int cu_share;
  int route_n;
  int nprod;
};

enum { kProfClasses = 64 };
void prof_enable(bool on);
bool prof_on();
void prof_pair(int cls, double flops, double bytes, hipEvent_t* e0, hipEvent_t* e1);
void route_note(const char* kernel);
const char* route_last();
#define UWM_LAUNCH(cls, flops, bytes, kernel, grid, block, lds, st, ...)                                     \
  do {                                                                                                       \
    route_note(#kernel);                                                                                     \
    if (prof_on()) {                                                                                         \
      hipEvent_t e0_, e1_; prof_pair((cls), (flops), (bytes), &e0_, &e1_);                                   \
      hipExtLaunchKernelGGL(kernel, grid, block, lds, st, e0_, e1_, 0, __VA_ARGS__);                         \
    } else {                                                                                                 \
      hipLaunchKernelGGL(kernel, grid, block, lds, st, __VA_ARGS__);                                         \
    }                                                                                                        \
  } while (0)
int  prof_collect(double* out );
const char* prof_class_name(int cls);

hipError_t launch_conv(const ConvArgs& a, hipStream_t st, int force_cfg = -1);
bool conv_epilogue_carries_bnb(const ConvArgs& a);
hipError_t launch_wgrad(const WgradArgs& a, hipStream_t st);
bool wgrad_patch_applicable(const WgradArgs& a);
hipError_t launch_wgrad_patch(const WgradArgs& a, hipStream_t st);
bool wgrad_wino_applicable(const WgradArgs& a);
hipError_t launch_wgrad_wino(const WgradArgs& a, hipStream_t st);
size_t wgrad_wino_scratch_floats();
float* wgrad_op_scratch();
bool wgrad_c16_applicable(const WgradArgs& a);
hipError_t launch_wgrad_c16(const WgradArgs& a, hipStream_t st);
hipError_t launch_wgrad_reduce(const float* part, int nsplit, size_t n4, float* dw, hipStream_t st, ReduceQueue* rq = nullptr);
// ... 17 lines not shown
hipError_t launch_conv_up2_f16(const ConvArgs& a, hipStream_t st);
hipError_t launch_conv_up2_dgrad_f16(const ConvArgs& a, hipStream_t st);
bool conv_c16_f16_applicable(const ConvArgs& a);
hipError_t launch_conv_c16_f16(const ConvArgs& a, hipStream_t st);
bool conv_c32_f16_applicable(const ConvArgs& a);
hipError_t launch_conv_c32_f16(const ConvArgs& a, hipStream_t st);
bool wgrad_up2_f16_shape(const WgradArgs& a);
int wgrad_up2_f16_parts(const WgradArgs& a);
hipError_t launch_wgrad_up2_f16(const WgradArgs& a, hipStream_t st);
bool conv_patch_applicable(const ConvArgs& a);
bool conv_patch16_applicable(const ConvArgs& a);
hipError_t launch_conv_patch16(const ConvArgs& a, hipStream_t st);
hipError_t launch_conv_patch(const ConvArgs& a, hipStream_t st, int bn);
bool conv_wino_applicable(const ConvArgs& a);
hipError_t launch_conv_wino(const ConvArgs& a, hipStream_t st, int bn = 0);
bool conv_head_applicable(const ConvArgs& a);
hipError_t launch_conv_head(const ConvArgs& a, hipStream_t st);
bool conv_head_dgrad_applicable(const ConvArgs& a);
hipError_t launch_conv_head_dgrad(const ConvArgs& a, hipStream_t st);
bool conv_wino8_applicable(const ConvArgs& a);
hipError_t launch_conv_wino8(const ConvArgs& a, hipStream_t st);
size_t wino_weights_floats(int wrows, int Ctot);
int wino_ncb(int wrows);
hipError_t launch_wino_weights(const float* w, int wrows, int Kpad, int Ctot, int mirror, float* ut, hipStream_t st);
struct WinoJob { const float* w; float* ut; int rows, chans, Kpad, mode, src_rows, pad_; };
struct WinoJobs { WinoJob j[40]; int n; };
hipError_t launch_wino_weights_multi(const WinoJobs& jobs, hipStream_t st);
hipError_t launch_wino_weights_x3_multi(const WinoJobs& jobs, hipStream_t st);
int f16x3_nj(int rows);
size_t f16x3_bank_floats(int rows, int chans);
size_t f16x3_rinv_off(int rows, int chans);
hipError_t launch_f16x3_weights_multi(const WinoJobs& jobs, hipStream_t st);
bool conv_f16x3_applicable(const ConvArgs& a);
static inline __host__ __device__ size_t f16x3_rinv_off_floats(int rows, int chans) { return (size_t)(chans / 16) * 5 * (size_t)(((rows + 63) / 64) * 4) * 512; }
bool f16x3v2_shape(int Ho, int Wo, int rows, int chans, int dgrad);
int f16x3v2_nf(int rows);
hipError_t launch_f16x3v2_weights_multi(const WinoJobs& jobs, hipStream_t st);
bool conv_f16x3v2_applicable(const ConvArgs& a);
hipError_t launch_conv_f16x3v2(const ConvArgs& a, hipStream_t st, int variant = 0);
size_t stem_f16x3_bank_floats();
hipError_t launch_stem_f16x3_weights(const float* w, int Kpad, int cin_p, float* bank, hipStream_t st);
bool conv_stem_f16x3_applicable(const ConvArgs& a);
hipError_t launch_conv_stem_f16x3(const ConvArgs& a, hipStream_t st);
hipError_t launch_conv_f16x3(const ConvArgs& a, hipStream_t st, int variant = 0);
bool conv_wino_x3_applicable(const ConvArgs& a);
hipError_t launch_conv_wino_x3(const ConvArgs& a, hipStream_t st);
bool winograd_enabled();
void winograd_set_mode(int mode);
int winograd_mode();
static inline int wino_mode_of(int wino) { return wino > 0 ? wino - 1 : winograd_mode(); }

hipError_t launch_nchw_to_nhwc4(const float* x, float* y, int N, int C, int H, int W, int CP, hipStream_t st);
hipError_t launch_bn_finalize(const double* ssum, const double* ssq, const float* gamma, const float* beta,
                              float* run_mean, float* run_var, float* mean, float* rstd, float* scale, float* shift,
                              int C, double count, float eps, float momentum, int update_running, hipStream_t st,
                              int nrep = 1, int rep_stride = 0);
hipError_t launch_bn_eval(const float* gamma, const float* beta, const float* run_mean, const float* run_var,
                          float* scale, float* shift, int C, float eps, hipStream_t st);
struct BnEvalJob { unsigned g_off, rm_off, out_off; int C; float eps; };
struct BnEvalJobs { static constexpr int kMax = 128; BnEvalJob j[kMax]; int n; };
hipError_t launch_bn_eval_multi(const float* params, const float* buffers, float* out, const BnEvalJobs& jobs, hipStream_t st);
hipError_t launch_residual(const float* y, const float* s2, const float* b2, const float* id, const float* sd,
                           const float* bd, float* out, size_t npix, int C, hipStream_t st);
hipError_t launch_maxpool_fwd(const Src& in, float* out, uint8_t* idx, int N, int Ho, int Wo, hipStream_t st);
hipError_t launch_maxpool_bwd(const float* gout, const uint8_t* idx, const float* addend, const Src& in, float* gin,
                              int N, int Ho, int Wo, hipStream_t st, const float* bn_mean = nullptr, const float* bn_rstd = nullptr,
                              double* ssum = nullptr, double* ssq = nullptr, int srep = 0, int sstride = 0);
hipError_t launch_bn_bwd_reduce(const float* g, const float* y, const float* mean, const float* rstd,
                                double* dgamma, double* dbeta, size_t npix, int C, hipStream_t st);
hipError_t launch_bn_bwd_apply(const float* g, const float* y, const float* mean, const float* rstd,
                               const float* gamma, const double* dgamma, const double* dbeta, float* dy,
                               float* gamma_grad, float* beta_grad, size_t npix, int C, hipStream_t st,
                               const double* rep = nullptr, int nrep = 0, int rep_stride = 0, hipEvent_t done = nullptr,
                               float* xmax = nullptr);
hipError_t launch_upsplit(const float* dcat, int N, int H, int W, int C0, int C1, float* gprev,
                          const float* pmask, const float* pscale, const float* pshift, float* gskip,
                          hipStream_t st, int accumulate_prev = 0);
hipError_t launch_concat_copy(const Src& s, size_t npix, float* dst, int Cd, int dst_off, hipStream_t st);
hipError_t launch_split_accum(const float* gcat, int Cc, int off, int C, size_t npix, float* dst, const float* m,
                              const float* mscale, const float* mshift, int accumulate, hipStream_t st);
hipError_t launch_pack_dgrad(const float* w, int Cout, int Kpad, int ntaps, int Cin, float* wd, int KpadD,
                             int CoutP, hipStream_t st);
hipError_t launch_colsum(const float* g, size_t npix, int C, float* out, double* scratch, hipStream_t st);
size_t colsum_scratch_doubles(int C);
hipError_t launch_adam(float* p, const float* g, float* m, float* v, size_t n, float lr, float b1, float b2,
                       float eps, float wd, float bc1, float bc2, float gscale, hipStream_t st,
                       const double* sumsq = nullptr, float max_norm = 0.f, bool decoupled = false);
hipError_t launch_adam_graph(float* p, const float* g, float* m, float* v, size_t n, float* hyp , const double* sumsq, hipStream_t st,
                             bool decoupled = false);
hipError_t launch_sumsq(const float* g, size_t n, double* out, hipStream_t st);
hipError_t launch_sgd(float* p, const float* g, float* buf, size_t n, float lr, float momentum, float wd, int first, float gscale,
                      hipStream_t st, const double* sumsq = nullptr, float max_norm = 0.f);
hipError_t launch_resize_threshold(const float* logits, int ld, int N, int h, int w, int H, int W, float thr,
                                   int apply_sigmoid, uint8_t* out, float* out_f, hipStream_t st);
hipError_t launch_scale(float* p, size_t n, float s, hipStream_t st);
hipError_t launch_absmax32(const float* x, size_t n, float* out32, hipStream_t st);
hipError_t launch_preprocess_u8(const uint8_t* img, int N, int H, int W, int C, const float* mean, const float* std,
                                const int* flags, float* out, hipStream_t st);
hipError_t launch_preprocess_u8_nhwc4(const uint8_t* img, size_t npix, int C, const float* mean, const float* std, float* out,
                                      hipStream_t st);
hipError_t launch_preprocess_mask(const uint8_t* m, int N, int H, int W, int thr, const int* flags, uint8_t* out, hipStream_t st);

hipError_t launch_swish_fwd(const float* y, const float* sc, const float* sh, int C, float* out, size_t npix, hipStream_t st);
hipError_t launch_dw_fwd(const float* x, const float* w, int k, int stride, int pb, int N, int H, int W, int C,
                         int Ho, int Wo, float* y, hipStream_t st);
hipError_t launch_dw_dgrad(const float* dy, const float* w, int k, int stride, int pb, int N, int H, int W, int C,
                           int Ho, int Wo, const float* addend, float* dx, hipStream_t st);
// ... 44 lines not shown
```

unet-watermark_amd/csrc/uwm_launch.inc:

```
struct Ctx {
  uwm_model* m; float* ws; hipStream_t st; int N;
  hipStream_t wst = nullptr;
  float* fz = nullptr;
  float* F(size_t off) const { return ws + off; }
  const float* bn_ss(const BNL& b) const { return fz ? fz + b.fz_off : ws + b.f_off + 2 * b.C; }
  float* wu(const ConvL& cv) const { return fz ? fz + cv.fz_wu : ws + cv.wu_off; }
  double* D(size_t doff) const { return (double*)ws + doff; }
};
static Src mk_src(const float* ptr, int C, int H, int W, const float* scale = nullptr, const float* shift = nullptr,
                  int relu = 0, int up = 0) {
  Src s; s.ptr = ptr; s.scale = scale; s.shift = shift; s.C = C; s.H = H; s.W = W; s.up = up; s.relu = relu; return s;
}
static Src lazy_src(const Ctx& c, int conv, int H, int W, int relu = 1, int up = 0) {
  const ConvL& cv = c.m->convs[conv];
  const BNL& b = c.m->bns[cv.bn];
  return mk_src(c.F(c.m->plan.y[conv]), cv.CoutP, H, W, c.bn_ss(b), c.bn_ss(b) + b.C, relu, up);
}

static thread_local bool g_err_own = false;
static hipError_t fail_launch(const char* fmt, ...) {
  va_list ap; va_start(ap, fmt); vsnprintf(g_err, sizeof(g_err), fmt, ap); va_end(ap);
  g_err_own = true;
  return hipErrorInvalidValue;
}

static bool dy_max_needed(const uwm_model* m, size_t ci) {
  return m->convs[ci].bn >= 0 &&
         (f3_dgrad_on(m, ci) || f3_wgrad_on(m, ci) || ig16_on(m, ci, true) || up2_f16_on(m, ci, true) || stem_wg16_on(m, ci) ||
          c16_wg16_on(m, ci) || c16_f16_on(m, ci, true));
}
static hipError_t dy_max_slot(const Ctx& c, int ci, const char* pass, const float** slot) {
  const ConvL& cv = c.m->convs[ci];
  if (!dy_max_needed(c.m, (size_t)ci) || cv.bn >= (int)c.m->dy_max_made.size() || !c.m->dy_max_made[cv.bn])
    return fail_launch("internal: the fp16x3 %s of %s has no max|dY| producer (dy_max_needed / run_bn_bwd*)", pass, cv.name.c_str());
  *slot = (const float*)c.D(c.m->bns[cv.bn].xmax_off());
  return hipSuccess;
}

static hipError_t route_rec(const Ctx& c, const char* pass, int ci, hipError_t e) {
  if (c.m->route_log_on && e == hipSuccess) { c.m->route_log += pass; c.m->route_log += ' '; c.m->route_log += c.m->convs[ci].name; c.m->route_log += ' '; c.m->route_log += route_last(); c.m->route_log += '\n'; }
  return e;
}

static hipError_t run_conv_fwd(const Ctx& c, int ci, const Src& s0, const Src* s1, int Ho, int Wo, float* out,
                               bool stats, int cfg = -1) {
  const ConvL& cv = c.m->convs[ci];
  ConvArgs a; memset(&a, 0, sizeof(a));
  a.s0 = s0; a.C0 = s0.C;
  if (s1) { a.s1 = *s1; a.Ctot = s0.C + s1->C; } else { a.s1 = s0; a.Ctot = s0.C; }
  a.w = c.m->params + cv.w_off; a.wrows = cv.Cout; a.Kpad = cv.Kpad; a.ntaps = cv.k * cv.k; a.kw = cv.k;
  a.N = c.N; a.Ho = Ho; a.Wo = Wo; a.Cout = cv.CoutP; a.M = c.N * Ho * Wo;
  a.Hl = s0.H << s0.up; a.Wl = s0.W << s0.up;
  a.smul = cv.stride; a.rmul = 1; a.off = -cv.pad; a.sdiv = 1;
  a.out = out; a.bias = cv.bias_off >= 0 ? c.m->params + cv.bias_off : nullptr;
  if (stats && cv.bn >= 0) {
    const BNL& b = c.m->bns[cv.bn];
    a.ssum = c.D(b.d_off) + 2 * b.C; a.ssq = a.ssum + b.C; a.srep = b.nrep; a.sstride = 2 * b.C;
  }
  a.dv_ctot = make_fastdiv(a.Ctot); a.dv_kw = make_fastdiv(a.kw);
  a.flops = 2.0 * (double)a.M * cv.Cout * cv.Cin * cv.k * cv.k;
  a.bytes = 4.0 * ((double)c.N * s0.H * s0.W * s0.C + (s1 ? (double)c.N * s1->H * s1->W * s1->C : 0.0) + (double)cv.Cout * cv.Kpad +
                   (double)a.M * cv.CoutP);
  if (ci == c.m->stem && cfg < 0 && stem_f3_on(c.m)) {
    a.wu = c.wu(cv);
    if (conv_stem_f16x3_applicable(a)) return route_rec(c, "fwd", ci, launch_conv_stem_f16x3(a, c.st));
    a.wu = nullptr;
  }
  if (cv.wu_off && !cv.stem7() && a.Ctot == cv.CinP && c.m->plan.wino_ok((size_t)ci)) {
    a.wu = c.wu(cv); a.wu_ncb = wino_ncb(cv.Cout);
// ... 13 lines not shown

struct UpSplit { float* gprev; int C0; const float* pmask; const float* pscale; const float* pshift; int accumulate = 0; };
static hipError_t run_dgrad(const Ctx& c, int ci, const float* dy, int Ho, int Wo, int Hin, int Win, float* dx,
                            const float* addend, const float* mask, const float* mscale, const float* mshift,
                            const UpSplit* us = nullptr, int bn_fuse = -1, bool* fused = nullptr, const float* bn_y = nullptr) {
  const ConvL& cv = c.m->convs[ci];
  ConvArgs a; memset(&a, 0, sizeof(a));
  a.s0 = mk_src(dy, cv.CoutP, Ho, Wo); a.s1 = a.s0; a.C0 = cv.CoutP; a.Ctot = cv.CoutP;
  a.w = c.F(cv.wd_off); a.wrows = cv.CinP; a.Kpad = cv.KpadD; a.ntaps = cv.k * cv.k; a.kw = cv.k;
  a.N = c.N; a.Ho = Hin; a.Wo = Win; a.Cout = cv.CinP; a.M = c.N * Hin * Win;
  a.Hl = Ho; a.Wl = Wo; a.smul = 1; a.rmul = -1; a.off = cv.pad; a.sdiv = cv.stride;
  a.out = dx; a.addend = addend; a.mask = mask; a.mscale = mscale; a.mshift = mshift; a.live_ch = cv.Cout;
  a.dv_ctot = make_fastdiv(a.Ctot); a.dv_kw = make_fastdiv(a.kw);
  a.flops = 2.0 * (double)c.N * Ho * Wo * cv.Cout * cv.Cin * cv.k * cv.k;
  a.bytes = 4.0 * ((double)c.N * Ho * Wo * cv.CoutP + (double)cv.CinP * cv.KpadD +
                   (double)a.M * cv.CinP * (1.0 + (addend ? 1.0 : 0.0) + (mask ? 1.0 : 0.0)));
  if (cv.wud_off && c.m->plan.wino_ok((size_t)ci)) {
    a.wu = c.F(cv.wud_off); a.wu_ncb = wino_ncb(cv.CinP);
    const int pm = c.m->plan.prec;
    if ((pm == UWM_PREC_BF16X3 || pm == UWM_PREC_BF16X3_ALL) && cv.x3_d()) a.prec = 1;
    if (f3_dgrad_on(c.m, (size_t)ci) && (!us || (us->C0 & 63) == 0)) {
      a.prec = 2; a.wu_layout = f3_layout(c.m, (size_t)ci, true); a.nprod = f3_nprod(c.m, true);
      a.wu_ncb = a.wu_layout == 1 ? f16x3v2_nf(cv.CinP) : f16x3_nj(cv.CinP); a.wu_rinv_off = (int)f16x3_rinv_off(cv.CinP, cv.CoutP);
      const hipError_t e = dy_max_slot(c, ci, "dgrad", &a.xmax);
      if (e != hipSuccess) return e;
    }
  }
  a.wino = c.m->plan.wino_mode + 1;
  if (ig16_on(c.m, (size_t)ci, true) || up2_f16_on(c.m, (size_t)ci, true) || c16_f16_on(c.m, (size_t)ci, true)) {
    a.ig16 = 1;
    const hipError_t e = dy_max_slot(c, ci, "dgrad", &a.xmax);
    if (e != hipSuccess) return e;
  }
  if (us) { a.out_up = us->gprev; a.up_c0 = us->C0; a.up_mask = us->pmask; a.up_mscale = us->pscale; a.up_mshift = us->pshift; a.up_accum = us->accumulate; }
  if (fused) *fused = false;
  static const bool no_fuse = dbg_flag("UWM_NO_BN_FUSE");
  a.bnb_y = bn_y;
  if (bn_fuse >= 0 && fused && !no_fuse && (us ? (us->pmask != nullptr && !us->accumulate) : (mask != nullptr || bn_y != nullptr)) && conv_epilogue_carries_bnb(a)) {
    const BNL& b = c.m->bns[bn_fuse];
    if (b.C == (us ? us->C0 : cv.CinP)) {
      const float* f = c.F(b.f_off);
      a.bnb_mean = f; a.bnb_rstd = f + b.C;
      a.ssum = c.D(b.d_off) + 2 * b.C; a.ssq = a.ssum + b.C; a.srep = b.nrep; a.sstride = 2 * b.C;
      *fused = true;
    }
  }
  if (!fused || !*fused) a.bnb_y = nullptr;
  a.route_n = c.m->route_n;
  return route_rec(c, "dgrad", ci, launch_conv(a, c.st));
}

static hipError_t run_wgrad(const Ctx& c, int ci, const Src& s0, const Src* s1, const float* dy, int Ho, int Wo) {
  const ConvL& cv = c.m->convs[ci];
  WgradArgs a; memset(&a, 0, sizeof(a));
  a.s0 = s0; a.C0 = s0.C;
  if (s1) { a.s1 = *s1; a.Ctot = s0.C + s1->C; } else { a.s1 = s0; a.Ctot = s0.C; }
  a.dy = dy; a.dw = c.m->grads + cv.w_off; a.wrows = cv.Cout; a.Kpad = cv.Kpad; a.ntaps = cv.k * cv.k; a.kw = cv.k;
  a.N = c.N; a.Ho = Ho; a.Wo = Wo; a.Cout = cv.CoutP; a.M = c.N * Ho * Wo;
  a.Hl = s0.H << s0.up; a.Wl = s0.W << s0.up; a.stride = cv.stride; a.pad = cv.pad;
  a.dv_ctot = make_fastdiv(a.Ctot); a.dv_kw = make_fastdiv(a.kw);
  a.flops = 2.0 * (double)a.M * cv.Cout * cv.Cin * cv.k * cv.k;
  a.bytes = 4.0 * ((double)a.M * cv.CoutP + (double)c.N * s0.H * s0.W * s0.C + (s1 ? (double)c.N * s1->H * s1->W * s1->C : 0.0) +
                   (double)cv.Cout * cv.Kpad);
  a.wino = c.m->plan.wino_mode + 1; a.route_n = c.m->route_n;
  if (stem_wg16_on(c.m, (size_t)ci) || c16_wg16_on(c.m, (size_t)ci) || up2_f16_on(c.m, (size_t)ci, true)) a.prec = 2;
  if (ig16_on(c.m, (size_t)ci, true)) a.prec = 2;
  if (f3_wgrad_on(c.m, (size_t)ci)) { a.prec = 2; a.nprod = f3_nprod(c.m, true); a.cu_share = (c.wst && c.wst != c.st) ? 3 : 0; }
  if (a.prec == 2) {
    const hipError_t e = dy_max_slot(c, ci, "wgrad", &a.xmax);
    if (e != hipSuccess) return e;
  }
  static const bool no_defer = dbg_flag("UWM_NO_DEFER_REDUCE");
  ReduceQueue& rq = c.m->rq;
  const size_t cap = wgrad_wino_scratch_floats();
  if (rq.n + 1 >= ReduceQueue::kMax || rq.used_floats + cap > kWgParts * cap) {
    hipError_t e = launch_wgrad_reduce_multi(rq, (c.wst && c.wst != c.st) ? c.wst : c.st);
    if (e != hipSuccess) return e;
  }
  a.part = c.F(c.m->plan.wg_part) + rq.used_floats; a.part_floats = cap; a.rq = no_defer ? nullptr : &rq;
  if (c.wst && c.wst != c.st) {
    const bool covered = std::find(c.m->disp_cov.begin(), c.m->disp_cov.end(), dy) != c.m->disp_cov.end();
    hipError_t e = hipSuccess;
    if (!covered) e = hipEventRecord(c.m->ev_fork, c.st);
    if (e != hipSuccess) return e;
    e = hipStreamWaitEvent(c.wst, covered ? c.m->ev_disp : c.m->ev_fork, 0);
    if (e != hipSuccess) return e;
    return route_rec(c, "wgrad", ci, launch_wgrad(a, c.wst));
  }
  return route_rec(c, "wgrad", ci, launch_wgrad(a, c.st));
}

static hipError_t run_bn_finalize(const Ctx& c, int bi, size_t count, int training) {
  uwm_model* m = c.m; const BNL& b = m->bns[bi];
  float* f = c.F(b.f_off);
  const float eps = b.eps > 0.f ? b.eps : m->desc.bn_eps, mom = b.mom > 0.f ? b.mom : m->desc.bn_momentum;
  if (training)
    return launch_bn_finalize(c.D(b.d_off) + 2 * b.C, c.D(b.d_off) + 3 * b.C, m->params + b.g_off, m->params + b.b_off,
                              m->buffers + b.rm_off, m->buffers + b.rv_off, f, f + b.C, f + 2 * b.C, f + 3 * b.C, b.C,
                              (double)count, eps, mom, 1, c.st, b.nrep, 2 * b.C);
  ++m->prep_launches;
  return launch_bn_eval(m->params + b.g_off, m->params + b.b_off, m->buffers + b.rm_off, m->buffers + b.rv_off,
                        f + 2 * b.C, f + 3 * b.C, b.C, eps, c.st);
}

static hipError_t run_bn_bwd(const Ctx& c, int ci, const float* g, float* dy, size_t npix, bool sums_fused = false) {
  uwm_model* m = c.m; const ConvL& cv = m->convs[ci]; const BNL& b = m->bns[cv.bn];
  const float* f = c.F(b.f_off); const float* y = c.F(m->plan.y[ci]);
  double* dg = c.D(b.d_off); double* db = c.D(b.d_off) + b.C;
  hipEvent_t done = nullptr;
  if (c.wst && c.wst != c.st && m->ev_disp && m->disp_fork) {
    hipStreamCaptureStatus cs = hipStreamCaptureStatusNone;
    if (hipStreamIsCapturing(c.st, &cs) != hipSuccess) { cs = hipStreamCaptureStatusNone; (void)hipGetLastError(); }
    if (cs == hipStreamCaptureStatusNone) done = m->ev_disp;
  }
  hipError_t e = hipSuccess;
  float* xmax = dy_max_needed(m, (size_t)ci) ? (float*)c.D(b.xmax_off()) : nullptr;
  if (sums_fused)
    e = launch_bn_bwd_apply(g, y, f, f + b.C, m->params + b.g_off, nullptr, nullptr, dy, m->grads + b.g_off, m->grads + b.b_off,
                            npix, b.C, c.st, c.D(b.d_off) + 2 * b.C, b.nrep, 2 * b.C, done, xmax);
  else {
    e = launch_bn_bwd_reduce(g, y, f, f + b.C, dg, db, npix, b.C, c.st);
    if (e != hipSuccess) return e;
    e = launch_bn_bwd_apply(g, y, f, f + b.C, m->params + b.g_off, dg, db, dy, m->grads + b.g_off, m->grads + b.b_off,
                            npix, b.C, c.st, nullptr, 0, 0, done, xmax);
  }
  if (e == hipSuccess && done) m->disp_cov.push_back(dy);
  if (e == hipSuccess && xmax) m->dy_max_made[cv.bn] = 1;
  return e;
}

static hipError_t run_bn_bwd_act(const Ctx& c, int ci, const float* g, float* dy, int N, size_t hw, const float* se_s, const float* gpool) {
  uwm_model* m = c.m; const ConvL& cv = m->convs[ci]; const BNL& b = m->bns[cv.bn];
  const float* f = c.F(b.f_off);
  float* xmax = dy_max_needed(m, (size_t)ci) ? (float*)c.D(b.xmax_off()) : nullptr;
  const hipError_t e = launch_bn_bwd_act(g, c.F(m->plan.y[ci]), f, f + b.C, m->params + b.g_off, f + 2 * b.C, f + 3 * b.C, se_s, gpool,
                                         N, hw, c.D(b.d_off), c.D(b.d_off) + b.C, dy, m->grads + b.g_off, m->grads + b.b_off, b.C, c.st, xmax);
  if (e == hipSuccess && xmax) m->dy_max_made[cv.bn] = 1;
  return e;
}

#define LCHK(expr)                                                                                     \
  do { hipError_t e_ = (expr); if (e_ != hipSuccess) { if (g_err_own) { g_err_own = false; return 1; }     \
       return fail("launch failed: %s at %s:%d (%s)", hipGetErrorString(e_), __FILE__, __LINE__, #expr); } } while (0)

static hipError_t wino_jobs(const Ctx& c, bool dgrad, hipStream_t st) {
  if (c.m->plan.wino_mode == 0) return hipSuccess;
  uwm_model* m = c.m;
  const int prec = m->plan.prec;
  const bool bf = prec == UWM_PREC_BF16X3 || prec == UWM_PREC_BF16X3_ALL;
// ... 22 lines not shown
```

unet-watermark_amd/csrc/uwm_model.hip:

```cpp
#include "../../include/uwm.h"
#include "uwm_kernels.h"

#include <cstdarg>
#include <dlfcn.h>
#include <cstdio>
#include <cstdlib>
#include <cstring>
#include <string>
#include <vector>
#include <algorithm>
#include <cmath>

using namespace uwm;

static thread_local char g_err[512] = "";
static int fail(const char* fmt, ...) {
  va_list ap; va_start(ap, fmt); vsnprintf(g_err, sizeof(g_err), fmt, ap); va_end(ap);
  return 1;
}
#define HIPCHK(expr)                                                                           \
  do { hipError_t e_ = (expr); if (e_ != hipSuccess) return fail("%s failed: %s (%s:%d)", #expr, \
       hipGetErrorString(e_), __FILE__, __LINE__); } while (0)

static inline long long rup(long long v, long long a) { return (v + a - 1) / a * a; }

struct BNL {
  std::string name; int C; int stage;
  long long g_off, b_off;
  long long rm_off, rv_off;
  size_t d_off;
  int nrep;
  size_t dcount() const { return 2 * (size_t)C + (size_t)nrep * 2 * C + 16; }
  size_t xmax_off() const { return d_off + dcount() - 16; }
  size_t f_off;
  size_t fz_off = 0;
  float eps = 0.f, mom = 0.f;
};
struct ConvL {
  std::string name; int Cin, CinP, Cout, CoutP, k, stride, pad, Kpad, KpadD, stage;
  long long w_off, bias_off; int bn; bool dgrad;
  bool dw = false;
  long long wfloats() const { return dw ? (long long)k * k * CoutP : (long long)Cout * Kpad; }
  size_t wd_off;
  size_t wu_off, wud_off;
  size_t wu_floats = 0, fz_wu = 0;
  bool wino() const { return k == 3 && stride == 1 && pad == 1 && (CinP & 7) == 0; }
  bool wino_d() const { return dgrad && k == 3 && stride == 1 && pad == 1 && (CoutP & 7) == 0; }
  int c0 = 0;
  bool x3() const { return wino() && (CinP & 15) == 0 && (c0 & 15) == 0; }
  bool x3_d() const { return wino_d() && (CoutP & 15) == 0; }
  bool f3() const { return wino() && (((CinP & 31) == 0 && (c0 & 15) == 0 && Cout >= 32) || (CinP == 16 && c0 == 16 && Cout == 16)); }
  bool stem7() const { return k == 7 && stride == 2 && pad == 3 && CinP == 4 && Cout == 64 && CoutP == 64 && !dw; }
  bool f3_d() const { return wino_d() && (((CoutP & 31) == 0 && CinP >= 16) || (CoutP == 16 && CinP == 16 && Cout == 16)); }
};
struct BlockL { int c1, c2, cd, c3 = -1, stride = 1, Cin = 0, Cout = 0; int last() const { return c3 >= 0 ? c3 : c2; } };
struct DecL { int c1, c2, C0, C1; };
struct NodeL { int c1, c2, prev; std::vector<int> skips; int C0, C1, lvl; };
struct MBL { int ce = -1, cdw = -1, cr = -1, cx = -1, cp = -1, Cin = 0, Cout = 0, mid = 0, nsq = 0, k = 3, stride = 1, pb = 0; bool skip = false; float drop = 0.f; };

constexpr size_t kWgParts = 8;
struct Plan {
  int N = 0, H = 0, W = 0, training = -1;
  size_t bytes = 0;
  size_t x4 = 0, pool = 0, pool_idx = 0, g_pool = 0, tmp = 0, loss_scr = 0;
  std::vector<size_t> y, g;
  std::vector<int> oh, ow;
// ... 34 lines not shown
  long long param_floats = 0, buffer_floats = 0, param_count = 0;
  long long stage_begin[6] = {0, 0, 0, 0, 0, 0};
  std::vector<uwm_tensor_info> infos;
  float *params = nullptr, *grads = nullptr, *buffers = nullptr;
  size_t fixed_floats = 0;
  Plan plan;
  bool have_fwd = false;
  hipStream_t side = nullptr;
  hipEvent_t ev_fork = nullptr, ev_join = nullptr, ev_pack = nullptr;
  hipEvent_t ev_disp = nullptr;
  std::vector<const float*> disp_cov;
  int disp_fork = 1;
  int use_side = 1;
  hipStream_t join_stream = nullptr;
  bool packed_in_fwd = false;
  int pack_mode = -1;
  int wino_mode = 1;
  int prec = 0;
  int device = -1;
  int nstages = 5;
  bool hwq_warned = false;
  ReduceQueue rq;
  int f3_min_wgs = 0;
  int route_n = 0;
  bool route_log_on = false;
  std::string route_log;
  bool prec_from_env = false;
  std::vector<char> dy_max_made;
  float* frozen = nullptr;
  size_t frozen_floats = 0;
  std::vector<signed char> fz_form;
  long long prep_launches = 0;
  std::vector<char> out_sums;
};

static int add_bn(uwm_model* m, const std::string& name, int C, int stage, float eps = 0.f, float mom = 0.f) {
  BNL b; b.eps = eps; b.mom = mom; b.name = name; b.C = C; b.stage = stage; b.nrep = C <= 64 ? 32 : (C <= 128 ? 16 : (C <= 256 ? 8 : 4)); b.g_off = b.b_off = b.rm_off = b.rv_off = -1; b.d_off = b.f_off = 0;
  m->bns.push_back(b); return (int)m->bns.size() - 1;
}
static int add_conv(uwm_model* m, const std::string& name, int Cin, int Cout, int k, int stride, int pad, int stage,
                    bool dgrad, const std::string& bn_name, bool bias = false, float bn_eps = 0.f, float bn_mom = 0.f) {
  ConvL c; c.name = name; c.Cin = Cin; c.CinP = (int)rup(Cin, 4); c.Cout = Cout; c.CoutP = (int)rup(Cout, 4);
  c.k = k; c.stride = stride; c.pad = pad; c.stage = stage; c.dgrad = dgrad;
  c.Kpad = (int)rup((long long)k * k * c.CinP, 32);
  c.KpadD = (int)rup((long long)k * k * c.CoutP, 32);
  c.w_off = -1; c.bias_off = bias ? 0 : -1; c.wd_off = 0; c.wu_off = c.wud_off = 0; c.c0 = c.CinP;
  c.bn = bn_name.empty() ? -1 : add_bn(m, bn_name, Cout, stage, bn_eps, bn_mom);
  m->convs.push_back(c); return (int)m->convs.size() - 1;
}

static void push_info(uwm_model* m, const std::string& name, int kind, int arena, long long off, int ndim,
                      const long long* shape, const long long* stride) {
  uwm_tensor_info t; memset(&t, 0, sizeof(t));
  snprintf(t.name, sizeof(t.name), "%s", name.c_str());
  t.kind = kind; t.arena = arena; t.ndim = ndim; t.offset = off;
  for (int i = 0; i < ndim; ++i) { t.shape[i] = shape[i]; t.stride[i] = stride[i]; }
  m->infos.push_back(t);
}

static int build_model(uwm_model* m) {
  const uwm_unet_desc& d = m->desc;
  int nb[4] = {0, 0, 0, 0}; int expn = 1;
  const bool effnet = d.encoder >= UWM_ENC_EFFICIENTNET_B0 && d.encoder <= UWM_ENC_EFFICIENTNET_B7;
  if (d.encoder == UWM_ENC_RESNET18) { nb[0] = 2; nb[1] = 2; nb[2] = 2; nb[3] = 2; }
  else if (d.encoder == UWM_ENC_RESNET34) { nb[0] = 3; nb[1] = 4; nb[2] = 6; nb[3] = 3; }
  else if (d.encoder == UWM_ENC_RESNET50) { nb[0] = 3; nb[1] = 4; nb[2] = 6; nb[3] = 3; expn = 4; }
// ... 202 lines not shown
```

unet-watermark_amd/csrc/wgrad_f16x3.hip:

```cpp
#include "uwm_kernels.h"

namespace uwm {

typedef float f4 __attribute__((ext_vector_type(4)));
typedef _Float16 h8 __attribute__((ext_vector_type(8)));
typedef _Float16 h4 __attribute__((ext_vector_type(4)));
typedef __fp16 fp16x4 __attribute__((__vector_size__(4 * sizeof(__fp16))));
typedef __attribute__((address_space(3))) fp16x4 lds_fp16x4;

#ifndef UWM_WG16_ABL
#define UWM_WG16_ABL 0
#endif
#ifndef UWM_WG16_XCD
#define UWM_WG16_XCD 1
#endif
template <int WX> struct WG16 {
  static constexpr int kWR = 128 / WX, kWX = WX, kWPW = WX + 2, kWPH = kWR + 2;
  static constexpr int kWXB = kWPH * kWPW * 136;
  static constexpr int kWStage = 32768 + ((kWXB + 255) & ~255);
  static constexpr int kWXRounds = (kWPH * kWPW * 8 + 511) / 512;
};
constexpr int kWDyB = 128 * 256;
constexpr int kWXS = 136;
constexpr int kWLT = 512;
constexpr int kWDyRounds = 128 * 16 / kWLT;

__device__ __forceinline__ int off_dy(int row, int ch) { return 256 * row + 16 * (ch ^ (((row & 3) << 2) | ((row >> 2) & 3))); }
__device__ __forceinline__ float clamp_hw(float v) { return __builtin_amdgcn_fmed3f(v, -65504.f, 65504.f); }
__device__ __forceinline__ h8 tr_pair(const char* base, int o0, int o1) {
  const fp16x4 lo = __builtin_amdgcn_ds_read_tr16_b64_v4f16((lds_fp16x4*)(uintptr_t)(base + o0));
  const fp16x4 hi = __builtin_amdgcn_ds_read_tr16_b64_v4f16((lds_fp16x4*)(uintptr_t)(base + o1));
  typedef __fp16 fp16x8 __attribute__((__vector_size__(8 * sizeof(__fp16))));
  const fp16x8 v = __builtin_shufflevector(lo, hi, 0, 1, 2, 3, 4, 5, 6, 7);
  return __builtin_bit_cast(h8, v);
}

template <int WX, int NP = 3>
__global__ __launch_bounds__(768, 1) void wgrad_f16x3_kernel(const WgradArgs a, int stages_per_split, int nstages) {
  constexpr int kWR = WG16<WX>::kWR, kWX = WX, kWPW = WG16<WX>::kWPW, kWPH = WG16<WX>::kWPH, kWStage = WG16<WX>::kWStage, kWXRounds = WG16<WX>::kWXRounds;
  constexpr int kKS = 4, kRK = 32 / WX;
  extern __shared__ __attribute__((aligned(256))) char wsm[];
  const int tid = threadIdx.x, lane = tid & 63, wave = __builtin_amdgcn_readfirstlane(tid >> 6);
  const bool is_mma = wave < 4;
  const int ltid = tid - 256;

  const int tilesA = (a.wrows + 63) / 64, tilesB = a.Ctot / 32;
  const int pairs = tilesA * tilesB;
#if UWM_WG16_XCD
  const unsigned nblk = gridDim.x, bid = blockIdx.x;
  const unsigned q8 = nblk >> 3, r8 = nblk & 7, xcd = bid & 7;
  const int lin = (int)((xcd < r8 ? xcd * (q8 + 1) : r8 * (q8 + 1) + (xcd - r8) * q8) + (bid >> 3));
#else
  const int lin = blockIdx.x;
#endif
  const int split = lin / pairs, pr = lin - split * pairs;
  const int ta = pr / tilesB, tb = pr - ta * tilesB;
  const int a0 = ta * 64, b0 = tb * 32;
  const int st0 = split * stages_per_split, st1 = min(nstages, st0 + stages_per_split);
  const int tilesX = a.Wo / kWX, tilesY = a.Ho / kWR;

  float xs = 1.f;
  if (a.xmax) {
    float mx = a.xmax[lane & 31];
#pragma unroll
    for (int d = 16; d >= 1; d >>= 1) mx = fmaxf(mx, __shfl_xor(mx, d));
    if (mx > 0.f && mx < 3.0e38f) { int e; (void)frexpf(mx, &e); xs = ldexpf(1.f, 14 - e); }
  }

  f4 acc[2][9];
#pragma unroll
  for (int cf = 0; cf < 2; ++cf)
#pragma unroll
    for (int t = 0; t < 9; ++t) acc[cf][t] = (f4){0.f, 0.f, 0.f, 0.f};

  if (!is_mma) {
    const bool first = b0 < a.C0;
    const Src& s = first ? a.s0 : a.s1;
    const int cl = first ? b0 : b0 - a.C0;
    const int dcu = ltid & 15;
    const bool dok = a0 + dcu * 4 < a.Cout;
    const int xcu = ltid & 7;
    f4 xsc = {1.f, 1.f, 1.f, 1.f}, xsh = {0.f, 0.f, 0.f, 0.f};
    const bool xhas = s.scale != nullptr;
    if (xhas) { xsc = *(const f4*)(s.scale + cl + xcu * 4); xsh = *(const f4*)(s.shift + cl + xcu * 4); }
    const int xrelu = s.relu;
    struct Stage { f4 dv[kWDyRounds]; f4 xv[kWXRounds]; unsigned xok; };
    int dgo[kWDyRounds], dlo[kWDyRounds], xpy[kWXRounds], xlo[kWXRounds];
#pragma unroll
    for (int rd = 0; rd < kWDyRounds; ++rd) {
      const int px = (rd * kWLT + ltid) >> 4;
      dgo[rd] = ((px / kWX) * a.Wo + (px % kWX)) * a.Cout;
      dlo[rd] = off_dy(px, dcu >> 1) + (dcu & 1) * 8;
    }
#pragma unroll
    for (int rd = 0; rd < kWXRounds; ++rd) {
      const int pp = (rd * kWLT + ltid) >> 3;
      const bool act = pp < kWPH * kWPW;
      const int py = act ? pp / kWPW : 0, px = act ? pp - py * kWPW : 0;
      xpy[rd] = act ? ((py << 8) | px) : -1;
      xlo[rd] = pp * kWXS + xcu * 8;
    }
    const float* const dyp = a.dy + a0 + dcu * 4;
    const float* const xp = s.ptr + cl + xcu * 4;
    auto stage_load = [&](int st, Stage& sg) {
      int q = st;
      const int tx = q % tilesX; q /= tilesX;
      const int ty = q % tilesY; const int n = q / tilesY;
      const int y0 = ty * kWR, x0 = tx * kWX;
      const float* const dbase = dyp + (((size_t)n * a.Ho + y0) * a.Wo + x0) * a.Cout;
#pragma unroll
      for (int rd = 0; rd < kWDyRounds; ++rd) sg.dv[rd] = dok ? *(const f4*)(dbase + dgo[rd]) : (f4){0.f, 0.f, 0.f, 0.f};
      sg.xok = 0;
      const int nb = n * s.H;
#pragma unroll
      for (int rd = 0; rd < kWXRounds; ++rd) {
        const int hl = y0 - 1 + (xpy[rd] >> 8), wl = x0 - 1 + (xpy[rd] & 255);
        const bool ok = xpy[rd] >= 0 && hl >= 0 && hl < a.Hl && wl >= 0 && wl < a.Wl;
        const int hc = min(max(hl, 0), a.Hl - 1), wc = min(max(wl, 0), a.Wl - 1);
        sg.xv[rd] = *(const f4*)(xp + (size_t)(((nb + (hc >> s.up)) * s.W + (wc >> s.up))) * s.C);
        sg.xok |= (ok ? 1u : 0u) << rd;
      }
    };
    auto split_store = [&](char* dst_hi, char* dst_lo, f4 v, bool clamp) {
      h4 hi, lo;
#pragma unroll
      for (int e = 0; e < 4; ++e) {
        const float x = clamp ? clamp_hw(v[e]) : v[e];
        const _Float16 h = (_Float16)x;
        hi[e] = h; lo[e] = (_Float16)(x - (float)h);
      }
      *(h4*)dst_hi = hi; *(h4*)dst_lo = lo;
    };
    auto stage_store = [&](int buf, const Stage& sg) {
      char* const dyb = wsm + buf * kWStage;
      char* const xb = dyb + kWDyB;
#pragma unroll
      for (int rd = 0; rd < kWDyRounds; ++rd) split_store(dyb + dlo[rd], dyb + (dlo[rd] ^ 128), sg.dv[rd] * xs, false);
#pragma unroll
      for (int rd = 0; rd < kWXRounds; ++rd) {
        if (xpy[rd] >= 0) {
          f4 v = sg.xv[rd];
          if (xhas) {
            v = v * xsc + xsh;
            if (xrelu) { v.x = fmaxf(v.x, 0.f); v.y = fmaxf(v.y, 0.f); v.z = fmaxf(v.z, 0.f); v.w = fmaxf(v.w, 0.f); }
          }
          if (!((sg.xok >> rd) & 1u)) v = (f4){0.f, 0.f, 0.f, 0.f};
          split_store(xb + xlo[rd], xb + xlo[rd] + 64, v, true);
        }
      }
    };
    Stage sA, sB;
    const int ns = st1 - st0;
    if (ns > 0) {
      stage_load(st0, sA);
      stage_load(ns > 1 ? st0 + 1 : st0, sB);
      stage_store(0, sA);
    }
    __syncthreads();
    constexpr bool skip = (UWM_WG16_ABL & 4) != 0;
    for (int i = 0; i < ns; i += 2) {
      {
        if (i + 1 < ns && !(skip && i > 0)) stage_store(1, sB);
        if (!skip) stage_load(st0 + (i + 2 < ns ? i + 2 : ns - 1), sA);
        __syncthreads();
      }
      if (i + 1 < ns) {
        if (i + 2 < ns && !skip) stage_store(0, sA);
        if (!skip) stage_load(st0 + (i + 3 < ns ? i + 3 : ns - 1), sB);
        __syncthreads();
      }
// ... 51 lines not shown
#pragma unroll
    for (int cf = 0; cf < 2; ++cf)
#pragma unroll
      for (int t = 0; t < 9; ++t)
#pragma unroll
        for (int e = 0; e < 4; ++e) {
          const int row = a0 + 16 * (2 * cp + cf) + 4 * (lane >> 4) + e;
          if (row < a.wrows && ci < a.Ctot) {
            float* pd = dst + (size_t)row * a.Kpad + t * a.Ctot + ci;
            const float v = acc[cf][t][e] * ixs;
            if (UWM_WG16_ABL & 8) { if (v == 123.456f) *pd = v; }
            else if (a.nsplit > 1) *pd = v; else *pd += v;
          }
        }
  }
}

static int wgrad_f16x3_wx(const WgradArgs& a) {
  if ((a.Wo % 32) == 0 && (a.Ho % 4) == 0) return 32;
  if ((a.Wo % 16) == 0 && (a.Ho % 8) == 0) return 16;
  return 0;
}
bool wgrad_f16x3_applicable(const WgradArgs& a) {
  return a.xmax != nullptr && a.ntaps == 9 && a.kw == 3 && a.stride == 1 && a.pad == 1 && (a.Ctot & 31) == 0 && (a.C0 & 31) == 0 &&
         (a.Cout & 3) == 0 && a.wrows <= a.Cout && a.Kpad == 9 * a.Ctot && a.Hl == a.Ho && a.Wl == a.Wo &&
         wgrad_f16x3_wx(a) != 0 && (a.s0.C & 3) == 0 && (a.s1.C & 3) == 0 && a.Wo < 256 * 128 &&
         (size_t)a.N * a.s0.H * a.s0.W < (1ull << 31) && (size_t)a.N * a.s1.H * a.s1.W < (1ull << 31) && (size_t)8 * a.Wo * a.Cout < (1ull << 31);
}

template <int WX, int NP>
static hipError_t launch_wg16p(WgradArgs& a, hipStream_t st, int pairs, int sps, int nstages) {
  const size_t lds = (size_t)2 * WG16<WX>::kWStage;
  static DevOnce lds_attr;
  { hipError_t e = lds_attr.set_max_lds((const void*)wgrad_f16x3_kernel<WX, NP>, lds); if (e != hipSuccess) return e; }
  UWM_LAUNCH(43, a.flops, a.bytes, (wgrad_f16x3_kernel<WX, NP>), dim3((unsigned)(pairs * a.nsplit)), dim3(768), lds, st, a, sps, nstages);
  return hipGetLastError();
}
template <int WX>
static hipError_t launch_wg16(WgradArgs& a, hipStream_t st, int pairs, int sps, int nstages) {
  const int np = (a.nprod >= 1 && a.nprod <= 3) ? a.nprod : 3;
  return np == 3 ? launch_wg16p<WX, 3>(a, st, pairs, sps, nstages) : np == 2 ? launch_wg16p<WX, 2>(a, st, pairs, sps, nstages) : launch_wg16p<WX, 1>(a, st, pairs, sps, nstages);
}

hipError_t launch_wgrad_f16x3(const WgradArgs& a0, hipStream_t st) {
  WgradArgs a = a0;
  if (!wgrad_f16x3_applicable(a)) return hipErrorInvalidValue;
  const int wx = wgrad_f16x3_wx(a);
  const int pairs = ((a.wrows + 63) / 64) * (a.Ctot / 32);
  const int nstages = a.N * (a.Ho / (128 / wx)) * (a.Wo / wx);
  static const int cu_cap = dbg_int("UWM_WG16_CUS", 0);
  const int cus = cu_cap > 0 ? cu_cap : (a.cu_share > 0 ? device_cu_count() * a.cu_share / 4 : device_cu_count());
  int nsplit = (cus + pairs - 1) / pairs;
  if (nsplit > nstages / 4) nsplit = nstages / 4;
  if (nsplit < 1) nsplit = 1;
  const size_t image = (size_t)a.wrows * a.Kpad;
  if (nsplit > 1 && (!a.part || a.part_floats < 2 * image)) { a.part = wgrad_op_scratch(); a.part_floats = wgrad_wino_scratch_floats(); a.rq = nullptr; }
  if (nsplit > 1 && (!a.part || (size_t)nsplit * image > a.part_floats)) nsplit = a.part ? (int)(a.part_floats / image) : 1;
  if (nsplit < 1) nsplit = 1;
  const int sps = (nstages + nsplit - 1) / nsplit;
  nsplit = (nstages + sps - 1) / sps;
  a.nsplit = nsplit; a.msplit = sps;
  hipError_t e = wx == 32 ? launch_wg16<32>(a, st, pairs, sps, nstages) : launch_wg16<16>(a, st, pairs, sps, nstages);
  if (e != hipSuccess) return e;
  if (nsplit > 1) return launch_wgrad_reduce(a.part, nsplit, image / 4, a.dw, st, a.rq);
  return hipSuccess;
}

}
```

unet-watermark_amd/csrc/wgrad_igemm.hip:

```cpp
#include "uwm_kernels.h"
#include <cstdio>
#include <cstdlib>

namespace uwm {

typedef float f4 __attribute__((ext_vector_type(4)));

__device__ __forceinline__ unsigned fdivw(unsigned n, FastDiv f) {
  return f.d <= 1 ? n : __umulhi(n, f.mg);
}

typedef _Float16 wi_h8 __attribute__((ext_vector_type(8)));
typedef __fp16 wi_fp16x4 __attribute__((__vector_size__(4 * sizeof(__fp16))));
typedef __attribute__((address_space(3))) wi_fp16x4 wi_lds_fp16x4;
__device__ __forceinline__ wi_h8 wi_tr_pair(const char* base, int o0, int o1) {
  const wi_fp16x4 lo = __builtin_amdgcn_ds_read_tr16_b64_v4f16((wi_lds_fp16x4*)(uintptr_t)(base + o0));
  const wi_fp16x4 hi = __builtin_amdgcn_ds_read_tr16_b64_v4f16((wi_lds_fp16x4*)(uintptr_t)(base + o1));
  typedef __fp16 fp16x8 __attribute__((__vector_size__(8 * sizeof(__fp16))));
  const fp16x8 v = __builtin_shufflevector(lo, hi, 0, 1, 2, 3, 4, 5, 6, 7);
  return __builtin_bit_cast(wi_h8, v);
}

template <int TA, int TB, int WA, int WB, bool F16 = false>
__global__ __launch_bounds__(256, 2) void wgrad_igemm_kernel(const WgradArgs a) {
// ... 223 lines not shown
#pragma unroll
      for (int e = 0; e < 4; ++e) {
        const int row = a0 + wa * (TA / WA) + i * 16 + lq * 4 + e;
        if (row < a.wrows && kc < a.Kpad) {
          if (a.nsplit > 1) a.part[((size_t)split * a.wrows + row) * a.Kpad + kc] = acc[i][j][e] * ixs;
          else a.dw[(size_t)row * a.Kpad + kc] += acc[i][j][e] * ixs;
        }
      }
    }
}

template <int TA, int TB, int WA, int WB, bool F16 = false>
static hipError_t launch_w(const WgradArgs& a, hipStream_t st, int cls) {
  const int tilesA = (a.wrows + TA - 1) / TA, tilesB = (a.Kpad + TB - 1) / TB;
  const size_t lds = (F16 ? (size_t)2 * (2 * 32 * (TA * 2 + 32) + 2 * 32 * (TB * 2 + 32)) : (size_t)2 * 32 * (TA + 16 + TB + 16) * sizeof(float)) + 2 * 32 * 4 * sizeof(int);
  static DevOnce lds_attr;
  { hipError_t e = lds_attr.set_max_lds((const void*)wgrad_igemm_kernel<TA, TB, WA, WB, F16>, lds); if (e != hipSuccess) return e; }
  UWM_LAUNCH(cls, a.flops, a.bytes, (wgrad_igemm_kernel<TA, TB, WA, WB, F16>), dim3((unsigned)(tilesA * tilesB * a.nsplit)), dim3(256), lds, st, a);
  if (F16) route_note("(wgrad_igemm_kernel<TA, TB, WA, WB, true>)");
  if (a.nsplit > 1) {
    hipError_t e = hipGetLastError();
    if (e != hipSuccess) return e;
    return launch_wgrad_reduce(a.part, a.nsplit, (size_t)a.wrows * a.Kpad / 4, a.dw, st, a.rq);
  }
  return hipGetLastError();
}

hipError_t launch_wgrad(const WgradArgs& a0, hipStream_t st) {
  static const bool trace = dbg_flag("UWM_TRACE_CONV");
  if (trace)
    fprintf(stderr, "wgrad N=%d Ctot=%d(C0=%d) Cout=%d wrows=%d Ho=%d Wo=%d Hl=%d Wl=%d taps=%d stride=%d wino=%d patch=%d gflop=%.2f\n", a0.N, a0.Ctot,
            a0.C0, a0.Cout, a0.wrows, a0.Ho, a0.Wo, a0.Hl, a0.Wl, a0.ntaps, a0.stride, (int)(wino_mode_of(a0.wino) != 0 && wgrad_wino_applicable(a0)),
            (int)wgrad_patch_applicable(a0), a0.flops * 1e-9);
  if ((a0.force_igemm & 0xff) == 4) return launch_wgrad_gemm(a0, st);
  static const bool no_up2 = dbg_flag("UWM_NO_UP2") || dbg_flag("UWM_NO_UP2_WGRAD");
  if (((a0.force_igemm & 0xff) == 0 || (a0.force_igemm & 0xff) == 6) && a0.prec == 2 && a0.xmax && !no_up2 && wgrad_up2_applicable(a0) && wgrad_up2_f16_shape(a0))
    return launch_wgrad_up2(a0, st);
  if (((a0.force_igemm & 0xff) == 0 || (a0.force_igemm & 0xff) == 6) && a0.prec == 2 && wgrad_f16x3_applicable(a0)) return launch_wgrad_f16x3(a0, st);
  if ((a0.force_igemm & 0xff) == 6 && a0.prec == 2 && wgrad_stem_applicable(a0)) return launch_wgrad_stem(a0, st);
  if ((a0.force_igemm & 0xff) == 6 && a0.prec == 2 && a0.Cout == 16 && wgrad_c16_applicable(a0)) return launch_wgrad_c16(a0, st);
  if ((a0.force_igemm & 0xff) == 6) return hipErrorInvalidValue;
  if ((a0.force_igemm & 0xff) == 0 && !no_up2 && wgrad_up2_applicable(a0)) return launch_wgrad_up2(a0, st);
  if ((a0.force_igemm & 0xff) == 0 && wgrad_stem_applicable(a0)) return launch_wgrad_stem(a0, st);
  if ((a0.force_igemm & 0xff) == 0 && wgrad_gemm_preferred(a0)) return launch_wgrad_gemm(a0, st);
  if ((a0.force_igemm & 0xff) == 0 && wgrad_c16_applicable(a0)) return launch_wgrad_c16(a0, st);
  if ((a0.force_igemm & 0xff) == 0 && wino_mode_of(a0.wino) != 0 && wgrad_wino_applicable(a0)) return launch_wgrad_wino(a0, st);
  if ((a0.force_igemm & 0xff) != 1 && (a0.force_igemm & 0xff) != 7 && wgrad_patch_applicable(a0)) return launch_wgrad_patch(a0, st);
  WgradArgs a = a0;
  if (a.M <= 0 || (a.Cout & 3) || (a.Kpad & 31) || (a.Ctot & 3) || (a.C0 & 3)) return hipErrorInvalidValue;
  int TA, TB;
  static const bool narrow = !dbg_flag("UWM_NO_NARROW_WGRAD");
  auto padded = [&](int tb) { return (a.Kpad + tb - 1) / tb * tb; };
  if (a.wrows <= 16) { TA = 16; TB = 256; }
  else if (a.wrows <= 32) {
    TA = 32; TB = 256;
    if (narrow && a.ntaps == 1) {
      if (padded(128) * 100 <= padded(TB) * 85) TB = 128;
      if (padded(64) * 100 <= padded(TB) * 85) TB = 64;
    }
  }
  else if (a.wrows <= 64) { TA = 64; TB = 128; }
  else {
    TA = 128; TB = 128;
    if (narrow && a.ntaps == 1) {
      if (padded(64) * 100 <= padded(TB) * 85) TB = 64;
      if (a.Kpad <= 96 && padded(32) * 100 <= padded(TB) * 85) TB = 32;
// ... 35 lines not shown
```

unet-watermark_amd/model.py:

```python
from __future__ import annotations

import ctypes as C
from typing import Optional, Sequence

import torch
import torch.nn as nn

from . import _lib as L


class _Node(nn.Module):
    """Plain container used to reproduce smp's module tree (names only)."""


def _get_node(root: nn.Module, path: Sequence[str]) -> nn.Module:
    cur = root
    for name in path:
        nxt = cur._modules.get(name)
        if nxt is None:
            nxt = _Node()
            cur.add_module(name, nxt)
        cur = nxt
    return cur

# ... 205 lines not shown
    def freeze(self, batch_shape: Optional[Sequence[int]] = None):
        if self.training:
            raise RuntimeError("freeze() needs eval mode (call .eval() first): a training forward moves the running statistics")
        self._require_gpu()
        L.check(L.lib().uwm_unfreeze(self._h))
        self._frozen = True
        if batch_shape is not None:
            n, h, w = (int(v) for v in batch_shape)
            self._ensure_bound()
            self._freeze_now(n, h, w)
        return self

    def unfreeze(self):
        if getattr(self, "_h", None) is not None and getattr(self, "_frozen", False):
            L.check(L.lib().uwm_unfreeze(self._h))
        self._frozen = False
        self._fz_arena = None
        return self

    def _freeze_now(self, n: int, h: int, w: int):
        need = int(L.lib().uwm_frozen_bytes(self._h))
        if self._fz_arena is None or self._fz_arena.numel() < need or self._fz_arena.device != self.device:
            self._fz_arena = torch.empty(need, dtype=torch.uint8, device=self.device)
        with L.on_device(self._fz_arena):
            L.check(L.lib().uwm_freeze(self._h, C.c_void_p(self._fz_arena.data_ptr()), self._fz_arena.numel(), n, h, w,
                                       C.c_void_p(L.stream_ptr(self.device))), SegmentationModelError)

    def frozen_serves(self, n: int, h: int, w: int) -> bool:
        return bool(self.frozen and L.lib().uwm_frozen_serves(self._h, int(n), int(h), int(w)))

    def prep_launches(self) -> int:
        return int(L.lib().uwm_prep_launches(self._h))

    def train(self, mode: bool = True):
        if mode:
            self.unfreeze()
        return super().train(mode)

    def load_state_dict(self, *args, **kwargs):
        self.unfreeze()
        return super().load_state_dict(*args, **kwargs)

    def routing(self, enable: Optional[bool] = None, clear: bool = True):
        if enable is not None:
            L.check(L.lib().uwm_routing_enable(self._h, int(bool(enable))))
            return self
        need = int(L.lib().uwm_routing_dump(self._h, None, 0, 0))
        buf = C.create_string_buffer(max(1, need))
        L.lib().uwm_routing_dump(self._h, buf, need, int(clear))
        out = []
        for line in buf.value.decode().splitlines():
            if line:
                pas, layer, kern = line.split(" ", 2)
                out.append((pas, layer, kern.strip("()")))
        return out

    def conv_flops(self, h: int, w: int):
        f, fb = C.c_double(), C.c_double()
        L.check(L.lib().uwm_conv_flops(self._h, int(h), int(w), C.byref(f), C.byref(fb)))
        return f.value, fb.value

    def _require_gpu(self, x: Optional[torch.Tensor] = None):
        if self._param_arena.device.type != "cuda":
            raise RuntimeError("uwm.Unet runs only on a HIP device (no CPU fallback): call .to('cuda') first")
        if x is not None and x.device != self._param_arena.device:
            raise RuntimeError(f"input is on {x.device} but the model is on {self._param_arena.device}")
# ... 177 lines not shown
```

Measured before the change: 1186 images/s.

## Fold BatchNorm backward apply into f16x3 dgrad and wgrad operand loads

Instead of running a separate BN-backward apply kernel that materializes dy, the BN backward now only computes per-channel coefficients. The f16x3 dgrad and wgrad kernels rebuild dy on the fly from the incoming gradient and the BN output using those coefficients. The forward/dgrad epilogue also publishes per-tensor max magnitudes so the fp16 split scaling stays valid without a separate max pass. This removes one full read-write pass over each activation-sized gradient, but each consumer must now load two tensors instead of one, which raises load pressure and register use inside the GEMM loops.

```diff
diff --git a/include/uwm.h b/include/uwm.h
--- a/include/uwm.h
+++ b/include/uwm.h
@@ -152,6 +152,10 @@
 
 int  uwm_set_side_stream(uwm_handle h, int on);
 
+int  uwm_set_dy_fold(uwm_handle h, int on);
+int  uwm_get_dy_fold(uwm_handle h);
+long long uwm_apply_launches(uwm_handle h);
+
 int  uwm_prof_enable(int on);
 int  uwm_prof_collect(double* out, int max_classes);
 const char* uwm_prof_class_name(int cls);
@@ -179,6 +183,14 @@
                              float* gin, uwm_stream stream);
 int  uwm_op_bn_backward(const float* g, const float* y, const float* mean, const float* rstd, const float* gamma,
                         double* scratch2c, float* dy, float* dgamma, float* dbeta, long long npix, int C, uwm_stream stream);
+int  uwm_op_bn_backward_fold(const float* g, const float* y, const float* mean, const float* rstd, const float* gamma,
+                             double* scratch, float* coef, float* xmax, float* dgamma, float* dbeta, long long npix, int C,
+                             uwm_stream stream);
+int  uwm_op_dgrad_fold(const float* g, const float* y, const float* coef, const float* xmax, int N, int H, int W, int Cout,
+                       const float* w, int Kpad, int Cin, float* dx, float* gprev, int up_c0, const float* up_mask, int variant,
+                       int nprod, uwm_stream stream);
+int  uwm_op_wgrad_fold(const uwm_src* s0, const uwm_src* s1, const float* g, const float* y, const float* coef, const float* xmax,
+                       int N, int Ho, int Wo, int Cout, int wrows, int Kpad, float* dw, int nprod, uwm_stream stream);
 int  uwm_op_bn_backward_act(const float* g, const float* y, const float* mean, const float* rstd, const float* gamma,
                             const float* scale, const float* shift, const float* se_s, const float* gpool, int N, long long hw,
                             int C, double* scratch2c, float* dy, float* dgamma, float* dbeta, float* xmax, uwm_stream stream);
diff --git a/unet-watermark_amd/_lib.py b/unet-watermark_amd/_lib.py
--- a/unet-watermark_amd/_lib.py
+++ b/unet-watermark_amd/_lib.py
@@ -105,6 +105,9 @@
     "uwm_op_morph": (I, [P, P, I, I, I, I, I, I, I, I, P, Z, P]),
     "uwm_op_components": (I, [P, P, P, I, I, I, P, Z, P]),
     "uwm_set_side_stream": (I, [P, I]),
+    "uwm_set_dy_fold": (I, [P, I]),
+    "uwm_get_dy_fold": (I, [P]),
+    "uwm_apply_launches": (L, [P]),
     "uwm_prof_enable": (I, [I]),
     "uwm_prof_collect": (I, [C.POINTER(C.c_double), I]),
     "uwm_prof_class_name": (C.c_char_p, [I]),
@@ -117,11 +120,17 @@
     "uwm_op_maxpool": (I, [C.POINTER(uwm_src), I, P, P, P]),
     "uwm_op_maxpool_backward": (I, [P, P, P, C.POINTER(uwm_src), I, P, P]),
     "uwm_op_bn_backward": (I, [P, P, P, P, P, P, P, P, P, L, I, P]),
+    "uwm_op_bn_backward_fold": (I, [P, P, P, P, P, P, P, P, P, P, L, I, P]),
+    "uwm_op_dgrad_fold": (I, [P, P, P, P, I, I, I, I, P, I, I, P, P, I, P, I, I, P]),
+    "uwm_op_wgrad_fold": (I, [C.POINTER(uwm_src), C.POINTER(uwm_src), P, P, P, P, I, I, I, I, I, I, P, I, P]),
     "uwm_op_bn_backward_act": (I, [P, P, P, P, P, P, P, P, P, I, L, I, P, P, P, P, P, P]),
     "uwm_op_dgrad_upsplit": (I, [P, I, I, I, I, P, I, I, I, P, P, P, P, P, P]),
     "uwm_op_upsplit": (I, [P, I, I, I, I, I, P, P, P, P, P, P]),
     "uwm_op_residual": (I, [P, P, P, P, P, P, P, L, I, P]),
 }
+
+NEWER_SYMBOLS = {"uwm_set_dy_fold", "uwm_get_dy_fold", "uwm_apply_launches", "uwm_op_bn_backward_fold", "uwm_op_dgrad_fold",
+                 "uwm_op_wgrad_fold"}
 
 _lib = None
 
@@ -179,6 +188,8 @@
     except OSError as e:
         raise RuntimeError(f"cannot load {LIB_PATH}: {e}") from e
     for name, (res, args) in SIGNATURES.items():
+        if name in NEWER_SYMBOLS and os.environ.get("UWM_LIB") and not hasattr(h, name):
+            continue
         fn = getattr(h, name)
         fn.restype = res
         fn.argtypes = args
diff --git a/unet-watermark_amd/csrc/conv_f16x3.hip b/unet-watermark_amd/csrc/conv_f16x3.hip
--- a/unet-watermark_amd/csrc/conv_f16x3.hip
+++ b/unet-watermark_amd/csrc/conv_f16x3.hip
@@ -166,8 +166,15 @@
 }
 
 __device__ __forceinline__ float clamp_h(float v) { return __builtin_amdgcn_fmed3f(v, -65504.f, 65504.f); }
-
-template <int NJ, int NP = 3>
+__device__ __forceinline__ float max_abs4(const f4& v) { return fmaxf(fmaxf(fabsf(v.x), fabsf(v.y)), fmaxf(fabsf(v.z), fabsf(v.w))); }
+__device__ __forceinline__ void bnb_max_publish(float* dst, const float* wv, int nw) {
+  float g = 0.f, y = 0.f;
+  for (int w = 0; w < nw; ++w) { g = fmaxf(g, wv[w * 2]); y = fmaxf(y, wv[w * 2 + 1]); }
+  if (g > 0.f) atomicMax((unsigned*)dst, __float_as_uint(g));
+  if (y > 0.f) atomicMax((unsigned*)dst + 1, __float_as_uint(y));
+}
+
+template <int NJ, int NP = 3, bool FOLD = false>
 __global__ __launch_bounds__(256, (NJ == 1 ? 4 : 2)) void conv_f16x3_kernel(const ConvArgs a) {
   constexpr bool kOne = NJ == 1;
   constexpr int kCo = 16 * NJ;
@@ -207,7 +214,7 @@
     const bool ok = act && hl >= 0 && hl < a.Hl && wl >= 0 && wl < a.Wl;
     const int hc = min(max(hl, 0), a.Hl - 1), wc = min(max(wl, 0), a.Wl - 1);
     goff[rd] = ((n * a.s0.H + (hc >> a.s0.up)) * a.s0.W + (wc >> a.s0.up)) * a.s0.C;
-    if (!kOne && a.C0 < a.Ctot) goff_s1[rd * 256 + tid] = ((n * a.s1.H + (hc >> a.s1.up)) * a.s1.W + (wc >> a.s1.up)) * a.s1.C;
+    if (!kOne && !FOLD && a.C0 < a.Ctot) goff_s1[rd * 256 + tid] = ((n * a.s1.H + (hc >> a.s1.up)) * a.s1.W + (wc >> a.s1.up)) * a.s1.C;
     gflags |= (ok ? 1u : 0u) << rd;
   }
   float xs = 1.f;
@@ -219,11 +226,14 @@
   }
   constexpr int kWR = kFRounds - 1;
   f4 pv[kWR], pvX = {0.f, 0.f, 0.f, 0.f}, psc = {1.f, 1.f, 1.f, 1.f}, psh = {0.f, 0.f, 0.f, 0.f};
+  f4 py[kWR], pyX = {0.f, 0.f, 0.f, 0.f}, pcb = {0.f, 0.f, 0.f, 0.f};
   float pfloor = -3.0e38f;
   const bool has_x = tid < kFPP * 4 - kWR * 256;
   const float* lsp = nullptr;
+  const ptrdiff_t ydel = FOLD ? a.dy_y - a.s0.ptr : 0;
   auto chunk_src = [&](int cc) {
     const int c = cc * 16;
+    if (FOLD) { lsp = a.s0.ptr + c + (tid & 3) * 4; return; }
     const bool first = c < a.C0;
     if (c == a.C0 && a.C0 < a.Ctot) {
 #pragma unroll
@@ -233,6 +243,11 @@
   };
   auto coef_load = [&](int cc) {
     const int c = cc * 16;
+    if (FOLD) {
+      const float* cf = a.dy_coef + c + (tid & 3) * 4;
+      psc = *(const f4*)cf; pcb = *(const f4*)(cf + a.Ctot); psh = *(const f4*)(cf + 2 * a.Ctot);
+      return;
+    }
     const bool first = c < a.C0;
     const Src& s = first ? a.s0 : a.s1;
     const int cl = (first ? c : c - a.C0) + (tid & 3) * 4;
@@ -240,9 +255,13 @@
     if (s.scale != nullptr) { psc = *(const f4*)(s.scale + cl); psh = *(const f4*)(s.shift + cl); }
     else { psc = (f4){1.f, 1.f, 1.f, 1.f}; psh = (f4){0.f, 0.f, 0.f, 0.f}; pfloor = -3.0e38f; }
   };
-  auto store_unit = [&](int buf, int rd, f4 raw) {
-    f4 v = raw * psc + psh;
-    v.x = fmaxf(v.x, pfloor); v.y = fmaxf(v.y, pfloor); v.z = fmaxf(v.z, pfloor); v.w = fmaxf(v.w, pfloor);
+  auto store_unit = [&](int buf, int rd, f4 raw, f4 rawy) {
+    f4 v;
+    if (FOLD) v = bn_dy(raw, rawy, psc, pcb, psh);
+    else {
+      v = raw * psc + psh;
+      v.x = fmaxf(v.x, pfloor); v.y = fmaxf(v.y, pfloor); v.z = fmaxf(v.z, pfloor); v.w = fmaxf(v.w, pfloor);
+    }
     v = v * xs;
     if (!((gflags >> rd) & 1u)) v = (f4){0.f, 0.f, 0.f, 0.f};
     h4 hi, lo;
@@ -301,18 +320,23 @@
   h8 wA_hi[NJ], wA_lo[NJ], wB_hi[NJ], wB_lo[NJ];
   w_load(0, wA_hi, wA_lo);
   chunk_src(0);
-#pragma unroll
-  for (int rd = 0; rd < kWR; ++rd) pv[rd] = *(const f4*)(lsp + goff[rd]);
-  if (has_x) pvX = *(const f4*)(lsp + goff[kWR]);
+  auto raw_load = [&](const float* sp, int rd, f4& g_, f4& y_) {
+    g_ = *(const f4*)(sp + goff[rd]);
+    if (FOLD) y_ = *(const f4*)(sp + goff[rd] + ydel);
+  };
+#pragma unroll
+  for (int rd = 0; rd < kWR; ++rd) raw_load(lsp, rd, pv[rd], py[rd]);
+  if (has_x) raw_load(lsp, kWR, pvX, pyX);
   coef_load(0);
 #pragma unroll
-  for (int rd = 0; rd < kWR; ++rd) store_unit(0, rd, pv[rd]);
-  if (has_x) store_unit(0, kWR, pvX);
+  for (int rd = 0; rd < kWR; ++rd) store_unit(0, rd, pv[rd], py[rd]);
+  if (has_x) store_unit(0, kWR, pvX, pyX);
+  constexpr int kAhead = 2;
   if (!kOne && nchunk > 1) {
     chunk_src(1);
 #pragma unroll
-    for (int rd = 0; rd < kWR; ++rd) pv[rd] = *(const f4*)(lsp + goff[rd]);
-    if (has_x) pvX = *(const f4*)(lsp + goff[kWR]);
+    for (int rd = 0; rd < (FOLD ? kAhead : kWR); ++rd) raw_load(lsp, rd, pv[rd], py[rd]);
+    if (!FOLD && has_x) raw_load(lsp, kWR, pvX, pyX);
   }
   __syncthreads();
 
@@ -334,8 +358,14 @@
         if (((hh * kFKs + ks) & 1) == 0) { w_load(tnext, wB_hi, wB_lo); mma_step(ks, pc, wA_hi, wA_lo); }
         else { w_load(tnext, wA_hi, wA_lo); mma_step(ks, pc, wB_hi, wB_lo); }
         if (!(dbg & 8) && !kOne) {
-          store_unit(nxt, ks, pv[ks]);
-          pv[ks] = *(const f4*)(lsp + goff[ks]);
+          store_unit(nxt, ks, pv[ks], py[ks]);
+          if (FOLD) {
+            constexpr int kW5 = kFKs;
+            const int r2 = (ks + kAhead) % kW5;
+            const float* sp = a.s0.ptr + (ks + kAhead < kW5 ? (more1 ? c + 1 : c) : (c + 2 < nchunk ? c + 2 : nchunk - 1)) * 16 + (tid & 3) * 4;
+            raw_load(sp, r2, pv[r2], py[r2]);
+            if (ks == 2 && has_x) raw_load(sp, kWR, pvX, pyX);
+          } else raw_load(lsp, ks, pv[ks], py[ks]);
         }
         __builtin_amdgcn_sched_group_barrier(0x020, 2 * NJ, 0);
         __builtin_amdgcn_sched_group_barrier(0x100, 8, 0);
@@ -345,12 +375,12 @@
           __builtin_amdgcn_sched_group_barrier(0x002, 3, 0);
         }
         __builtin_amdgcn_sched_group_barrier(0x200, 2, 0);
-        __builtin_amdgcn_sched_group_barrier(0x020, 1, 0);
+        __builtin_amdgcn_sched_group_barrier(0x020, FOLD ? 2 : 1, 0);
         __builtin_amdgcn_sched_barrier(0);
       }
       if (!(dbg & 8) && !kOne && has_x) {
-        if (more1) store_unit(nxt, kWR, pvX);
-        pvX = *(const f4*)(lsp + goff[kWR]);
+        if (more1) store_unit(nxt, kWR, pvX, pyX);
+        if (!FOLD) raw_load(lsp, kWR, pvX, pyX);
       }
       __syncthreads();
     }
@@ -372,6 +402,7 @@
   const int co = n0 + cq * 4;
   const bool cok = co < a.Cout;
   f4 ps_ = {0.f, 0.f, 0.f, 0.f}, pq_ = ps_;
+  float gmx = 0.f, ymx = 0.f;
   const int stat_c = a.out_up != nullptr ? a.up_c0 : a.Cout;
   if (NJ == 4 && a.out_up != nullptr) {
     f4 rs = {0.f, 0.f, 0.f, 0.f};
@@ -401,7 +432,9 @@
         }
         *(f4*)(a.out + o) = v;
         if (a.bnb_y) yr = *(const f4*)(a.bnb_y + o);
-        ps_ += v; pq_ += bnb ? v * ((yr - bmu) * brs) : v * v;
+        const f4 yh = (yr - bmu) * brs;
+        ps_ += v; pq_ += bnb ? v * yh : v * v;
+        if (a.bnb_max) { gmx = fmaxf(gmx, max_abs4(v)); ymx = fmaxf(ymx, max_abs4(yh)); }
       }
     }
   }
@@ -412,6 +445,10 @@
 #pragma unroll
       for (int d = kCQ; d < 64; d <<= 1) { sv += __shfl_xor(sv, d); qv += __shfl_xor(qv, d); }
       ps_[e] = sv; pq_[e] = qv;
+    }
+    if (a.bnb_max) {
+#pragma unroll
+      for (int d = 32; d >= 1; d >>= 1) { gmx = fmaxf(gmx, __shfl_xor(gmx, d)); ymx = fmaxf(ymx, __shfl_xor(ymx, d)); }
     }
     __syncthreads();
     float* red = (float*)hsm;
@@ -419,7 +456,9 @@
 #pragma unroll
       for (int e = 0; e < 4; ++e) { red[(wave * 64 + cq * 4 + e) * 2] = ps_[e]; red[(wave * 64 + cq * 4 + e) * 2 + 1] = pq_[e]; }
     }
+    if (a.bnb_max && lane == 0) { red[512 + wave * 2] = gmx; red[512 + wave * 2 + 1] = ymx; }
     __syncthreads();
+    if (a.bnb_max && tid == 64) bnb_max_publish(a.bnb_max, red + 512, 4);
     if (tid < kCo) {
       const int c1 = n0 + tid;
       if (c1 < stat_c) {
@@ -434,7 +473,7 @@
   }
 }
 
-template <int NP = 3>
+template <int NP = 3, bool FOLD = false>
 __global__ __launch_bounds__(512, 1) void conv_f16x3s_kernel(const ConvArgs a) {
   extern __shared__ __attribute__((aligned(16))) _Float16 hsm[];
 
@@ -487,8 +526,19 @@
       gflags |= ((ok ? 1u : 0u) | (act ? 2u : 0u)) << (2 * rd);
     }
     struct Stage { f4 pv[kFRounds]; f4 sc, sh; int relu; bool has; };
-    auto patch_load = [&](int cc, Stage& st) {
+    struct StageY { f4 py[FOLD ? kFRounds : 1]; f4 sb; };
+    const ptrdiff_t ydel = FOLD ? a.dy_y - a.s0.ptr : 0;
+    auto patch_load = [&](int cc, Stage& st, StageY& sy) {
       const int c = cc * 16;
+      if (FOLD) {
+        const int cl = c + (ltid & 3) * 4;
+        const float* cf = a.dy_coef + cl;
+        st.sc = *(const f4*)cf; sy.sb = *(const f4*)(cf + a.Ctot); st.sh = *(const f4*)(cf + 2 * a.Ctot);
+        const float* sp = a.s0.ptr + cl;
+#pragma unroll
+        for (int rd = 0; rd < kFRounds; ++rd) { st.pv[rd] = *(const f4*)(sp + goff0[rd]); sy.py[FOLD ? rd : 0] = *(const f4*)(sp + goff0[rd] + ydel); }
+        return;
+      }
       const bool first = c < a.C0;
       const Src& s = first ? a.s0 : a.s1;
       st.relu = s.relu;
@@ -499,11 +549,12 @@
 #pragma unroll
       for (int rd = 0; rd < kFRounds; ++rd) st.pv[rd] = *(const f4*)(sp + (first ? goff0[rd] : goff1[rd]));
     };
-    auto patch_store = [&](int buf, const Stage& st) {
+    auto patch_store = [&](int buf, const Stage& st, const StageY& sy) {
 #pragma unroll
       for (int rd = 0; rd < kFRounds; ++rd) {
         f4 v = st.pv[rd];
-        if (st.has) {
+        if (FOLD) v = bn_dy(st.pv[rd], sy.py[FOLD ? rd : 0], st.sc, sy.sb, st.sh);
+        else if (st.has) {
           v = v * st.sc + st.sh;
           if (st.relu) { v.x = fmaxf(v.x, 0.f); v.y = fmaxf(v.y, 0.f); v.z = fmaxf(v.z, 0.f); v.w = fmaxf(v.w, 0.f); }
         }
@@ -524,22 +575,22 @@
         }
       }
     };
-    Stage sA, sB;
-    patch_load(0, sA);
-    patch_load(nchunk > 1 ? 1 : 0, sB);
-    patch_store(0, sA);
+    Stage sA, sB; StageY yA, yB;
+    patch_load(0, sA, yA);
+    patch_load(nchunk > 1 ? 1 : 0, sB, yB);
+    patch_store(0, sA, yA);
     __syncthreads();
     for (int cc = 0; cc < nchunk; cc += 2) {
       {
         const int c2 = cc + 2 < nchunk ? cc + 2 : nchunk - 1;
-        if (cc + 1 < nchunk) patch_store(1, sB);
-        patch_load(c2, sA);
+        if (cc + 1 < nchunk) patch_store(1, sB, yB);
+        patch_load(c2, sA, yA);
         __syncthreads();
       }
       {
         const int c3 = cc + 3 < nchunk ? cc + 3 : nchunk - 1;
-        if (cc + 2 < nchunk) patch_store(0, sA);
-        patch_load(c3, sB);
+        if (cc + 2 < nchunk) patch_store(0, sA, yA);
+        patch_load(c3, sB, yB);
         __syncthreads();
       }
     }
@@ -618,6 +669,7 @@
   const bool cok = co < a.Cout;
   const int phalf = (wave >> 2) * 32;
   f4 ps_ = {0.f, 0.f, 0.f, 0.f}, pq_ = ps_;
+  float gmx = 0.f, ymx = 0.f;
   const int stat_c = a.out_up != nullptr ? a.up_c0 : a.Cout;
   if (a.out_up != nullptr) {
     f4 rs = {0.f, 0.f, 0.f, 0.f};
@@ -647,7 +699,9 @@
         }
         *(f4*)(a.out + o) = v;
         if (a.bnb_y) yr = *(const f4*)(a.bnb_y + o);
-        ps_ += v; pq_ += bnb ? v * ((yr - bmu) * brs) : v * v;
+        const f4 yh = (yr - bmu) * brs;
+        ps_ += v; pq_ += bnb ? v * yh : v * v;
+        if (a.bnb_max) { gmx = fmaxf(gmx, max_abs4(v)); ymx = fmaxf(ymx, max_abs4(yh)); }
       }
     }
   }
@@ -659,13 +713,19 @@
       sv += __shfl_xor(sv, 32); qv += __shfl_xor(qv, 32);
       ps_[e] = sv; pq_[e] = qv;
     }
+    if (a.bnb_max) {
+#pragma unroll
+      for (int d = 32; d >= 1; d >>= 1) { gmx = fmaxf(gmx, __shfl_xor(gmx, d)); ymx = fmaxf(ymx, __shfl_xor(ymx, d)); }
+    }
     __syncthreads();
     float* red = (float*)hsm;
     if (sub == 0) {
 #pragma unroll
       for (int e = 0; e < 4; ++e) { red[(wave * 64 + cq * 4 + e) * 2] = ps_[e]; red[(wave * 64 + cq * 4 + e) * 2 + 1] = pq_[e]; }
     }
+    if (a.bnb_max && lane == 0) { red[1024 + wave * 2] = gmx; red[1024 + wave * 2 + 1] = ymx; }
     __syncthreads();
+    if (a.bnb_max && tid == 64) bnb_max_publish(a.bnb_max, red + 1024, 8);
     if (tid < 64) {
       const int c1 = n0 + tid;
       if (c1 < stat_c) {
@@ -678,6 +738,11 @@
       }
     }
   }
+}
+
+bool conv_f16x3_four_wave(long wgs) {
+  static const bool force4 = dbg_flag("UWM_F16X3_4WAVE"), force8 = dbg_flag("UWM_F16X3_8WAVE");
+  return force4 || (!force8 && wgs >= 2L * device_cu_count());
 }
 
 bool conv_f16x3_applicable(const ConvArgs& a) {
@@ -690,6 +755,13 @@
 
 template <int NJ, int NP>
 static hipError_t launch_f3(const ConvArgs& a, hipStream_t st, dim3 grid, size_t lds) {
+  if (NJ > 1 && a.dy_y) {
+    static DevOnce lds_attr_f;
+    { hipError_t e = lds_attr_f.set_max_lds((const void*)conv_f16x3_kernel<(NJ > 1 ? NJ : 2), NP, true>, lds); if (e != hipSuccess) return e; }
+    UWM_LAUNCH(42, a.flops, a.bytes, (conv_f16x3_kernel<(NJ > 1 ? NJ : 2), NP, true>), grid, dim3(256), lds, st, a);
+    route_note("(conv_f16x3_kernel<NJ, NP>)");
+    return hipGetLastError();
+  }
   static DevOnce lds_attr;
   { hipError_t e = lds_attr.set_max_lds((const void*)conv_f16x3_kernel<NJ, NP>, lds); if (e != hipSuccess) return e; }
   UWM_LAUNCH(42, a.flops, a.bytes, (conv_f16x3_kernel<NJ, NP>), grid, dim3(256), lds, st, a);
@@ -697,6 +769,13 @@
 }
 template <int NP>
 static hipError_t launch_f3s(const ConvArgs& a, hipStream_t st, dim3 grid, size_t lds) {
+  if (a.dy_y) {
+    static DevOnce lds_attr_f;
+    { hipError_t e = lds_attr_f.set_max_lds((const void*)conv_f16x3s_kernel<NP, true>, lds); if (e != hipSuccess) return e; }
+    UWM_LAUNCH(42, a.flops, a.bytes, (conv_f16x3s_kernel<NP, true>), grid, dim3(512), lds, st, a);
+    route_note("(conv_f16x3s_kernel<NP>)");
+    return hipGetLastError();
+  }
   static DevOnce lds_attr;
   { hipError_t e = lds_attr.set_max_lds((const void*)conv_f16x3s_kernel<NP>, lds); if (e != hipSuccess) return e; }
   UWM_LAUNCH(42, a.flops, a.bytes, (conv_f16x3s_kernel<NP>), grid, dim3(512), lds, st, a);
@@ -708,11 +787,12 @@
   if (!conv_f16x3_applicable(a)) return hipErrorInvalidValue;
   if (a.out_up && (a.addend || a.mask || a.bias || a.bnb_y || (a.ssum && !a.bnb_mean) || (a.up_c0 < a.Cout && !a.out))) return hipErrorInvalidValue;
   if (a.bnb_mean && (!a.ssum || !a.ssq || !a.bnb_rstd || !(a.out_up ? a.up_mask : (a.bnb_y ? a.bnb_y : a.mask)) || a.up_accum)) return hipErrorInvalidValue;
+  if (a.bnb_max && (!a.bnb_mean || a.out_up)) return hipErrorInvalidValue;
+  if (a.dy_y && (!a.dy_coef || !a.xmax || a.rmul != -1 || a.C0 != a.Ctot || (a.Ctot & 31) || a.s0.C != a.Ctot || a.s0.up || a.s0.scale || a.s0.relu)) return hipErrorInvalidValue;
   const int tilesN = (a.Cout + 63) / 64;
   const int tilesW = (a.Wo + kFT - 1) / kFT, tilesH = (a.Ho + kFT - 1) / kFT;
   const size_t main_lds = (size_t)2 * kFBuf * sizeof(_Float16) + 6 * 256 * sizeof(int), q_lds = (size_t)4 * 64 * 68 * sizeof(float);
   const size_t lds = main_lds > q_lds ? main_lds : q_lds;
-  static const bool force4 = dbg_flag("UWM_F16X3_4WAVE"), force8 = dbg_flag("UWM_F16X3_8WAVE");
   const long wgs = (long)route_N(a) * tilesH * tilesW * tilesN;
   const int np = (a.nprod >= 1 && a.nprod <= 3) ? a.nprod : 3;
   if (a.Ctot == 16) {
@@ -720,7 +800,7 @@
     return np == 3 ? launch_f3<1, 3>(a, st, dim3((unsigned)(a.N * tilesH * tilesW)), lds1)
          : np == 2 ? launch_f3<1, 2>(a, st, dim3((unsigned)(a.N * tilesH * tilesW)), lds1) : launch_f3<1, 1>(a, st, dim3((unsigned)(a.N * tilesH * tilesW)), lds1);
   }
-  const bool four = variant == 1 || variant == 3 || (variant != 2 && (force4 || (!force8 && wgs >= 2L * device_cu_count())));
+  const bool four = variant == 1 || variant == 3 || (variant != 2 && conv_f16x3_four_wave(wgs));
   if (variant == 3 && a.out_up) return hipErrorInvalidValue;
   const bool fwd_alone = a.rmul == 1 && !a.xmax;
   const bool narrow = !a.out_up && (a.Cout <= 32 ? four : (fwd_alone && variant == 0 && wgs < device_cu_count()));
diff --git a/unet-watermark_amd/csrc/conv_igemm.hip b/unet-watermark_amd/csrc/conv_igemm.hip
--- a/unet-watermark_amd/csrc/conv_igemm.hip
+++ b/unet-watermark_amd/csrc/conv_igemm.hip
@@ -388,6 +388,7 @@
 hipError_t launch_conv(const ConvArgs& a, hipStream_t st, int force_cfg) {
   if (a.M <= 0 || a.Cout <= 0 || (a.Cout & 3) || (a.Kpad & 31) || (a.Ctot & 3) || (a.C0 & 3)) return hipErrorInvalidValue;
   int cfg = force_cfg;
+  if ((a.dy_y || a.bnb_max) && !(a.prec == 2 && a.wu_layout == 0 && (cfg < 0 || (cfg >= 600 && cfg <= 603)))) return hipErrorInvalidValue;
   static const bool trace = dbg_flag("UWM_TRACE_CONV");
   if (trace)
     fprintf(stderr, "conv %s N=%d Ctot=%d(C0=%d up=%d) Cout=%d Ho=%d Wo=%d Hl=%d Wl=%d taps=%d smul=%d sdiv=%d wino=%d gflop=%.2f\n",
diff --git a/unet-watermark_amd/csrc/elementwise.hip b/unet-watermark_amd/csrc/elementwise.hip
--- a/unet-watermark_amd/csrc/elementwise.hip
+++ b/unet-watermark_amd/csrc/elementwise.hip
@@ -410,6 +410,96 @@
   return hipGetLastError();
 }
 
+__global__ __launch_bounds__(256) void bn_bwd_coef_kernel(const float* __restrict__ mean, const float* __restrict__ rstd, const float* __restrict__ gamma,
+                                                          float* gamma_grad, float* beta_grad, int C, float invM,
+                                                          const double* __restrict__ rep, int nrep, int rep_stride,
+                                                          const float* __restrict__ gymax, float* __restrict__ coef, float* xmax) {
+  __shared__ float wmax[4];
+  __shared__ double part[2 * 256];
+  const int Q = C >> 2, nq = Q < 256 ? Q : 256, L = 256 / nq;
+  const int CB = 256 / L;
+  const int cl = threadIdx.x % CB, l = threadIdx.x / CB;
+  const int c = blockIdx.x * CB + cl;
+  if (l < L && c < C) {
+#pragma unroll
+    for (int half = 0; half < 2; ++half) {
+      const double* pr = rep + half * C + c;
+      double b = 0.0;
+      for (int r = l; r < nrep; r += L) b += pr[(size_t)r * rep_stride];
+      part[half * 256 + l * CB + cl] = b;
+    }
+  }
+  __syncthreads();
+  float bnd = 0.f;
+  if (l == 0 && c < C) {
+    double s[2];
+#pragma unroll
+    for (int half = 0; half < 2; ++half) {
+      double t = 0.0;
+      for (int k = 0; k < L; ++k) t += part[half * 256 + k * CB + cl];
+      s[half] = t;
+    }
+    if (beta_grad) beta_grad[c] = (float)s[0];
+    if (gamma_grad) gamma_grad[c] = (float)s[1];
+    const float db = (float)s[0] * invM, dg = (float)s[1] * invM;
+    const float mu = mean[c], rs = rstd[c], gm = gamma[c];
+    const float A = gm * rs, B = -(gm * rs * rs * dg), K = -(A * db) - B * mu;
+    coef[c] = A; coef[C + c] = B; coef[2 * C + c] = K;
+    bnd = fabsf(A) * (gymax[0] + fabsf(db) + gymax[1] * fabsf(dg));
+  }
+#pragma unroll
+  for (int d = 32; d >= 1; d >>= 1) bnd = fmaxf(bnd, __shfl_xor(bnd, d));
+  if ((threadIdx.x & 63) == 0) wmax[threadIdx.x >> 6] = bnd;
+  __syncthreads();
+  if (threadIdx.x == 0) {
+    const float mx = fmaxf(fmaxf(wmax[0], wmax[1]), fmaxf(wmax[2], wmax[3]));
+    if (mx > 0.f) atomicMax((unsigned*)xmax + (blockIdx.x & 31), __float_as_uint(mx));
+  }
+}
+hipError_t launch_bn_bwd_coef(const float* mean, const float* rstd, const float* gamma, float* gamma_grad, float* beta_grad,
+                              size_t npix, int C, hipStream_t st, const double* rep, int nrep, int rep_stride, const float* gymax,
+                              float* coef, float* xmax, hipEvent_t done) {
+  if (!rep || !gymax || !coef || !xmax || C <= 0 || (C & 3)) return hipErrorInvalidValue;
+  const int Q = C >> 2, nq = Q < 256 ? Q : 256, CB = 256 / (256 / nq);
+  const unsigned nb = (unsigned)((C + CB - 1) / CB);
+  if (done)
+    hipExtLaunchKernelGGL(bn_bwd_coef_kernel, dim3(nb), dim3(256), 0, st, nullptr, done, 0, mean, rstd, gamma, gamma_grad, beta_grad, C,
+                          (float)(1.0 / (double)npix), rep, nrep < 1 ? 1 : nrep, rep_stride, gymax, coef, xmax);
+  else
+    hipLaunchKernelGGL(bn_bwd_coef_kernel, dim3(nb), dim3(256), 0, st, mean, rstd, gamma, gamma_grad, beta_grad, C,
+                       (float)(1.0 / (double)npix), rep, nrep < 1 ? 1 : nrep, rep_stride, gymax, coef, xmax);
+  return hipGetLastError();
+}
+
+__global__ __launch_bounds__(256) void bn_gymax_kernel(const float* __restrict__ g, const float* __restrict__ y, const float* __restrict__ mean,
+                                                       const float* __restrict__ rstd, size_t n4, int C, float* out2) {
+  __shared__ float wm[8];
+  float gm = 0.f, ym = 0.f;
+  for (size_t i = blockIdx.x * (size_t)blockDim.x + threadIdx.x; i < n4; i += (size_t)gridDim.x * blockDim.x) {
+    const int c = (int)((i * 4) % (size_t)C);
+    const f4 gv = *(const f4*)(g + i * 4), yh = (*(const f4*)(y + i * 4) - *(const f4*)(mean + c)) * *(const f4*)(rstd + c);
+    gm = fmaxf(gm, fmaxf(fmaxf(fabsf(gv.x), fabsf(gv.y)), fmaxf(fabsf(gv.z), fabsf(gv.w))));
+    ym = fmaxf(ym, fmaxf(fmaxf(fabsf(yh.x), fabsf(yh.y)), fmaxf(fabsf(yh.z), fabsf(yh.w))));
+  }
+#pragma unroll
+  for (int d = 32; d >= 1; d >>= 1) { gm = fmaxf(gm, __shfl_xor(gm, d)); ym = fmaxf(ym, __shfl_xor(ym, d)); }
+  if ((threadIdx.x & 63) == 0) { wm[(threadIdx.x >> 6) * 2] = gm; wm[(threadIdx.x >> 6) * 2 + 1] = ym; }
+  __syncthreads();
+  if (threadIdx.x == 0) {
+    for (int w = 1; w < 4; ++w) { gm = fmaxf(gm, wm[w * 2]); ym = fmaxf(ym, wm[w * 2 + 1]); }
+    if (gm > 0.f) atomicMax((unsigned*)out2, __float_as_uint(gm));
+    if (ym > 0.f) atomicMax((unsigned*)out2 + 1, __float_as_uint(ym));
+  }
+}
+hipError_t launch_bn_gymax(const float* g, const float* y, const float* mean, const float* rstd, size_t npix, int C, float* out2, hipStream_t st) {
+  if (C <= 0 || (C & 3)) return hipErrorInvalidValue;
+  hipError_t e = hipMemsetAsync(out2, 0, 2 * sizeof(float), st);
+  if (e != hipSuccess) return e;
+  const size_t n4 = npix * C / 4;
+  hipLaunchKernelGGL(bn_gymax_kernel, dim3(nblocks(n4, 256 * 8)), dim3(256), 0, st, g, y, mean, rstd, n4, C, out2);
+  return hipGetLastError();
+}
+
 __global__ void upsplit_prev_kernel(const float* __restrict__ dcat, int H, int W, int C0, int Ct, float* __restrict__ gprev,
                                     const float* __restrict__ pmask, const float* __restrict__ pscale,
                                     const float* __restrict__ pshift, size_t total, int accumulate) {
diff --git a/unet-watermark_amd/csrc/uwm_abi.inc b/unet-watermark_amd/csrc/uwm_abi.inc
--- a/unet-watermark_amd/csrc/uwm_abi.inc
+++ b/unet-watermark_amd/csrc/uwm_abi.inc
@@ -12,6 +12,7 @@
   if (build_model(m)) { delete m; return 1; }
   const char* e = getenv("UWM_SIDE_STREAM");
   m->use_side = e ? atoi(e) : 1;
+  if (const char* fe = getenv("UWM_DY_FOLD")) m->dy_fold = atoi(fe) != 0;
   if (const char* pe = getenv("UWM_PRECISION")) {
     static const char* names[7] = {"f32", "bf16x3", "bf16x3_all", "f16x3", "f16x3_all", "f16x1", "f16x3_bwd2"};
     int found = -1;
@@ -407,6 +408,13 @@
   h->use_side = on != 0; return 0;
 }
 
+int uwm_set_dy_fold(uwm_handle h, int on) {
+  if (!h) return fail("uwm_set_dy_fold: null handle");
+  h->dy_fold = on != 0; return 0;
+}
+int uwm_get_dy_fold(uwm_handle h) { return h ? h->dy_fold : 0; }
+long long uwm_apply_launches(uwm_handle h) { return h ? h->apply_launches : 0; }
+
 int uwm_prof_enable(int on) { prof_enable(on != 0); return 0; }
 int uwm_prof_collect(double* out, int max_classes) {
   if (!out || max_classes < kProfClasses) return fail("uwm_prof_collect: need room for %d classes (4 doubles each)", (int)kProfClasses);
@@ -728,6 +736,68 @@
   LCHK(launch_bn_bwd_apply(g, y, mean, rstd, gamma, scratch2c, scratch2c + C, dy, dgamma, dbeta, (size_t)npix, C, st));
   return 0;
 }
+int uwm_op_bn_backward_fold(const float* g, const float* y, const float* mean, const float* rstd, const float* gamma, double* scratch,
+                            float* coef, float* xmax, float* dgamma, float* dbeta, long long npix, int C, uwm_stream stream) {
+  if (!g || !y || !mean || !rstd || !gamma || !scratch || !coef || !xmax || !dgamma || !dbeta || npix < 1 || C < 4 || (C & 3))
+    return fail("uwm_op_bn_backward_fold: bad argument");
+  hipStream_t st = (hipStream_t)stream;
+  HIPCHK(hipMemsetAsync(scratch, 0, (2 * (size_t)C + 1) * sizeof(double), st));
+  HIPCHK(hipMemsetAsync(xmax, 0, 32 * sizeof(float), st));
+  LCHK(launch_bn_bwd_reduce(g, y, mean, rstd, scratch + C, scratch, (size_t)npix, C, st));
+  float* gymax = (float*)(scratch + 2 * (size_t)C);
+  LCHK(launch_bn_gymax(g, y, mean, rstd, (size_t)npix, C, gymax, st));
+  LCHK(launch_bn_bwd_coef(mean, rstd, gamma, dgamma, dbeta, (size_t)npix, C, st, scratch, 1, 2 * C, gymax, coef, xmax));
+  return 0;
+}
+int uwm_op_dgrad_fold(const float* g, const float* y, const float* coef, const float* xmax, int N, int H, int W, int Cout,
+                      const float* w, int Kpad, int Cin, float* dx, float* gprev, int up_c0, const float* up_mask, int variant,
+                      int nprod, uwm_stream stream) {
+  const bool reuse_bank = (variant & 16) != 0;
+  variant &= 15;
+  if (!g || !xmax || !w || (!dx && !gprev) || (y && !coef) || variant < 0 || variant > 2) return fail("uwm_op_dgrad_fold: bad argument");
+  hipStream_t st = (hipStream_t)stream;
+  ConvArgs a; memset(&a, 0, sizeof(a));
+  a.s0 = mk_src(g, Cout, H, W); a.s1 = a.s0; a.C0 = Cout; a.Ctot = Cout;
+  a.wrows = Cin; a.Kpad = (int)rup(9LL * Cout, 32); a.ntaps = 9; a.kw = 3;
+  a.N = N; a.Ho = H; a.Wo = W; a.Cout = Cin; a.M = N * H * W;
+  a.Hl = H; a.Wl = W; a.smul = 1; a.rmul = -1; a.off = 1; a.sdiv = 1;
+  a.out = dx; a.live_ch = Cout;
+  if (gprev) { a.out_up = gprev; a.up_c0 = up_c0; a.up_mask = up_mask; }
+  a.dv_ctot = make_fastdiv(a.Ctot); a.dv_kw = make_fastdiv(a.kw);
+  if ((Cout & 31) || (Cin & 3) || H < 8 || W < 16) return fail("uwm_op_dgrad_fold: needs Cout %% 32 == 0, H >= 8, W >= 16");
+  static float* buf = nullptr; static size_t cap = 0;
+  const size_t need = f16x3_bank_floats(Cin, Cout);
+  if (need > cap) {
+    HIPCHK(hipDeviceSynchronize());
+    if (buf) HIPCHK(hipFree(buf));
+    HIPCHK(hipMalloc((void**)&buf, need * sizeof(float))); cap = need;
+  }
+  WinoJobs jobs; jobs.n = 1;
+  WinoJob& j = jobs.j[0];
+  j.w = w; j.ut = buf; j.rows = Cin; j.chans = Cout; j.Kpad = Kpad; j.mode = 2; j.src_rows = Cout; j.pad_ = 0;
+  if (!reuse_bank) LCHK(launch_f16x3_weights_multi(jobs, st));
+  a.wu = buf; a.wu_layout = 0; a.wu_ncb = f16x3_nj(Cin); a.wu_rinv_off = (int)f16x3_rinv_off(Cin, Cout); a.prec = 2;
+  a.xmax = xmax; a.nprod = nprod;
+  if (y) { a.dy_y = y; a.dy_coef = coef; }
+  LCHK(launch_conv(a, st, 600 + variant));
+  return 0;
+}
+int uwm_op_wgrad_fold(const uwm_src* s0, const uwm_src* s1, const float* g, const float* y, const float* coef, const float* xmax,
+                      int N, int Ho, int Wo, int Cout, int wrows, int Kpad, float* dw, int nprod, uwm_stream stream) {
+  if (!s0 || !g || !xmax || !dw || (y && !coef)) return fail("uwm_op_wgrad_fold: bad argument");
+  WgradArgs a; memset(&a, 0, sizeof(a));
+  a.s0 = to_src(s0); a.C0 = a.s0.C;
+  if (s1) { a.s1 = to_src(s1); a.Ctot = a.C0 + a.s1.C; } else { a.s1 = a.s0; a.Ctot = a.C0; }
+  a.dy = g; a.dw = dw; a.wrows = wrows; a.Kpad = Kpad; a.ntaps = 9; a.kw = 3;
+  a.N = N; a.Ho = Ho; a.Wo = Wo; a.Cout = Cout; a.M = N * Ho * Wo;
+  a.Hl = a.s0.H << a.s0.up; a.Wl = a.s0.W << a.s0.up; a.stride = 1; a.pad = 1;
+  a.dv_ctot = make_fastdiv(a.Ctot); a.dv_kw = make_fastdiv(a.kw);
+  a.prec = 2; a.xmax = xmax; a.nprod = nprod; a.force_igemm = 6;
+  if (y) { a.dy_y = y; a.dy_coef = coef; }
+  if (!wgrad_f16x3_applicable(a)) return fail("uwm_op_wgrad_fold: not a wgrad_f16x3 shape");
+  LCHK(launch_wgrad(a, (hipStream_t)stream));
+  return 0;
+}
 int uwm_op_bn_backward_act(const float* g, const float* y, const float* mean, const float* rstd, const float* gamma,
                            const float* scale, const float* shift, const float* se_s, const float* gpool, int N, long long hw,
                            int C, double* scratch2c, float* dy, float* dgamma, float* dbeta, float* xmax, uwm_stream stream) {
diff --git a/unet-watermark_amd/csrc/uwm_backward.inc b/unet-watermark_amd/csrc/uwm_backward.inc
--- a/unet-watermark_amd/csrc/uwm_backward.inc
+++ b/unet-watermark_amd/csrc/uwm_backward.inc
@@ -18,6 +18,7 @@
   std::vector<char>& out_sums = m->out_sums;
   if (sb <= 0 || out_sums.size() != first_blk[3] + m->stages[3].size()) out_sums.assign(first_blk[3] + m->stages[3].size(), 0);
   if (sb <= 0 || m->dy_max_made.size() != m->bns.size()) m->dy_max_made.assign(m->bns.size(), 0);
+  if (sb <= 0 || m->gy_max_made.size() != m->bns.size()) { m->gy_max_made.assign(m->bns.size(), 0); m->dy_fold_g.assign(m->bns.size(), nullptr); }
   m->disp_cov.clear();
   if (sb <= 0) m->rq = ReduceQueue();
   if (sb <= 0 && se > 0) {
diff --git a/unet-watermark_amd/csrc/uwm_kernels.h b/unet-watermark_amd/csrc/uwm_kernels.h
--- a/unet-watermark_amd/csrc/uwm_kernels.h
+++ b/unet-watermark_amd/csrc/uwm_kernels.h
@@ -72,12 +72,20 @@
   int ig16;
   int nprod;
   int wu_layout;
+  const float* dy_y; const float* dy_coef;
+  float* bnb_max;
 };
 
 template <class A> static inline int route_N(const A& a) { return a.route_n > 0 ? a.route_n : a.N; }
 template <class A> static inline long route_M(const A& a) { return a.N > 0 ? (long)a.M / a.N * route_N(a) : (long)a.M; }
 
 #if defined(__HIPCC__)
+template <class T4> __device__ __forceinline__ T4 bn_dy(T4 g, T4 y, T4 A, T4 B, T4 K) {
+  T4 r;
+#pragma unroll
+  for (int e = 0; e < 4; ++e) r[e] = __builtin_fmaf(g[e], A[e], __builtin_fmaf(y[e], B[e], K[e]));
+  return r;
+}
 typedef unsigned uwm_u2 __attribute__((ext_vector_type(2)));
 __device__ __forceinline__ void uwm_split4(float x0, float x1, float x2, float x3, uwm_u2& hi, uwm_u2& lo) {
   typedef _Float16 h2_ __attribute__((ext_vector_type(2)));
@@ -122,6 +130,7 @@
   int cu_share;
   int route_n;
   int nprod;
+  const float* dy_y; const float* dy_coef;
 };
 
 enum { kProfClasses = 64 };
@@ -205,6 +214,7 @@
 size_t f16x3_rinv_off(int rows, int chans);
 hipError_t launch_f16x3_weights_multi(const WinoJobs& jobs, hipStream_t st);
 bool conv_f16x3_applicable(const ConvArgs& a);
+bool conv_f16x3_four_wave(long wgs);
 static inline __host__ __device__ size_t f16x3_rinv_off_floats(int rows, int chans) { return (size_t)(chans / 16) * 5 * (size_t)(((rows + 63) / 64) * 4) * 512; }
 bool f16x3v2_shape(int Ho, int Wo, int rows, int chans, int dgrad);
 int f16x3v2_nf(int rows);
@@ -246,6 +256,11 @@
                                float* gamma_grad, float* beta_grad, size_t npix, int C, hipStream_t st,
                                const double* rep = nullptr, int nrep = 0, int rep_stride = 0, hipEvent_t done = nullptr,
                                float* xmax = nullptr);
+hipError_t launch_bn_bwd_coef(const float* mean, const float* rstd, const float* gamma, float* gamma_grad, float* beta_grad,
+                              size_t npix, int C, hipStream_t st, const double* rep, int nrep, int rep_stride, const float* gymax,
+                              float* coef, float* xmax, hipEvent_t done = nullptr);
+hipError_t launch_bn_gymax(const float* g, const float* y, const float* mean, const float* rstd, size_t npix, int C, float* out2,
+                           hipStream_t st);
 hipError_t launch_upsplit(const float* dcat, int N, int H, int W, int C0, int C1, float* gprev,
                           const float* pmask, const float* pscale, const float* pshift, float* gskip,
                           hipStream_t st, int accumulate_prev = 0);
diff --git a/unet-watermark_amd/csrc/uwm_launch.inc b/unet-watermark_amd/csrc/uwm_launch.inc
--- a/unet-watermark_amd/csrc/uwm_launch.inc
+++ b/unet-watermark_amd/csrc/uwm_launch.inc
@@ -35,6 +35,23 @@
     return fail_launch("internal: the fp16x3 %s of %s has no max|dY| producer (dy_max_needed / run_bn_bwd*)", pass, cv.name.c_str());
   *slot = (const float*)c.D(c.m->bns[cv.bn].xmax_off());
   return hipSuccess;
+}
+
+static bool dy_fold_on(const uwm_model* m, size_t ci) {
+  const ConvL& cv = m->convs[ci];
+  if (!m->dy_fold || cv.bn < 0 || (cv.CoutP & 31) || cv.CoutP != cv.Cout || m->bns[cv.bn].C != cv.CoutP) return false;
+  if (!(f3_dgrad_on(m, ci) && f3_layout(m, ci, true) == 0 && f3_wgrad_on(m, ci) && !up2_f16_on(m, ci, true))) return false;
+  static const int max_cin = dbg_int("UWM_DY_FOLD_MAX_CIN", 128);
+  static const int classes = dbg_int("UWM_DY_FOLD_CLASSES", 3);
+  const Plan& p = m->plan;
+  const long wgs = (long)(m->route_n > 0 ? m->route_n : p.N) * ((p.oh[ci] + 15) / 16) * ((p.ow[ci] + 15) / 16) * ((cv.CinP + 63) / 64);
+  return cv.CinP <= max_cin && ((conv_f16x3_four_wave(wgs) ? 1 : 2) & classes) != 0;
+}
+static const float* dy_fold_src(const Ctx& c, int ci, const float** y, const float** coef) {
+  const ConvL& cv = c.m->convs[ci];
+  if (cv.bn < 0 || cv.bn >= (int)c.m->dy_fold_g.size() || !c.m->dy_fold_g[cv.bn]) return nullptr;
+  *y = c.F(c.m->plan.y[ci]); *coef = c.F(c.m->bns[cv.bn].coef_foff());
+  return c.m->dy_fold_g[cv.bn];
 }
 
 static hipError_t route_rec(const Ctx& c, const char* pass, int ci, hipError_t e) {
@@ -114,6 +131,12 @@
     const hipError_t e = dy_max_slot(c, ci, "dgrad", &a.xmax);
     if (e != hipSuccess) return e;
   }
+  if (const float* fg = dy_fold_src(c, ci, &a.dy_y, &a.dy_coef)) {
+    if (a.prec != 2 || a.wu_layout != 0 || a.ig16)
+      return fail_launch("internal: the BatchNorm backward of %s was folded but its dgrad does not run on conv_f16x3 (dy_fold_on / run_dgrad)", cv.name.c_str());
+    a.s0.ptr = fg; a.s1.ptr = fg;
+    a.bytes += 4.0 * (double)c.N * Ho * Wo * cv.CoutP;
+  }
   if (us) { a.out_up = us->gprev; a.up_c0 = us->C0; a.up_mask = us->pmask; a.up_mscale = us->pscale; a.up_mshift = us->pshift; a.up_accum = us->accumulate; }
   if (fused) *fused = false;
   static const bool no_fuse = dbg_flag("UWM_NO_BN_FUSE");
@@ -125,6 +148,10 @@
       a.bnb_mean = f; a.bnb_rstd = f + b.C;
       a.ssum = c.D(b.d_off) + 2 * b.C; a.ssq = a.ssum + b.C; a.srep = b.nrep; a.sstride = 2 * b.C;
       *fused = true;
+      if (c.m->dy_fold && a.prec == 2 && a.wu_layout == 0 && !us && bn_fuse < (int)c.m->gy_max_made.size()) {
+        a.bnb_max = c.F(b.gymax_foff());
+        c.m->gy_max_made[bn_fuse] = 1;
+      }
     }
   }
   if (!fused || !*fused) a.bnb_y = nullptr;
@@ -152,6 +179,12 @@
     const hipError_t e = dy_max_slot(c, ci, "wgrad", &a.xmax);
     if (e != hipSuccess) return e;
   }
+  if (const float* fg = dy_fold_src(c, ci, &a.dy_y, &a.dy_coef)) {
+    if (!f3_wgrad_on(c.m, (size_t)ci) || !wgrad_f16x3_applicable(a))
+      return fail_launch("internal: the BatchNorm backward of %s was folded but its wgrad does not run on wgrad_f16x3 (dy_fold_on / run_wgrad)", cv.name.c_str());
+    a.dy = dy = fg;
+    a.bytes += 4.0 * (double)a.M * cv.CoutP;
+  }
   static const bool no_defer = dbg_flag("UWM_NO_DEFER_REDUCE");
   ReduceQueue& rq = c.m->rq;
   const size_t cap = wgrad_wino_scratch_floats();
@@ -197,6 +230,17 @@
   }
   hipError_t e = hipSuccess;
   float* xmax = dy_max_needed(m, (size_t)ci) ? (float*)c.D(b.xmax_off()) : nullptr;
+  if (cv.bn < (int)m->dy_fold_g.size()) m->dy_fold_g[cv.bn] = nullptr;
+  if (sums_fused && xmax && cv.bn < (int)m->dy_fold_g.size() && m->gy_max_made[cv.bn] && dy_fold_on(m, (size_t)ci)) {
+    e = launch_bn_bwd_coef(f, f + b.C, m->params + b.g_off, m->grads + b.g_off, m->grads + b.b_off, npix, b.C, c.st,
+                           c.D(b.d_off) + 2 * b.C, b.nrep, 2 * b.C, c.F(b.gymax_foff()), c.F(b.coef_foff()), xmax, done);
+    if (e != hipSuccess) return e;
+    m->dy_fold_g[cv.bn] = g;
+    if (done) m->disp_cov.push_back(g);
+    m->dy_max_made[cv.bn] = 1;
+    return e;
+  }
+  ++m->apply_launches;
   if (sums_fused)
     e = launch_bn_bwd_apply(g, y, f, f + b.C, m->params + b.g_off, nullptr, nullptr, dy, m->grads + b.g_off, m->grads + b.b_off,
                             npix, b.C, c.st, c.D(b.d_off) + 2 * b.C, b.nrep, 2 * b.C, done, xmax);
diff --git a/unet-watermark_amd/csrc/uwm_model.hip b/unet-watermark_amd/csrc/uwm_model.hip
--- a/unet-watermark_amd/csrc/uwm_model.hip
+++ b/unet-watermark_amd/csrc/uwm_model.hip
@@ -32,6 +32,8 @@
   int nrep;
   size_t dcount() const { return 2 * (size_t)C + (size_t)nrep * 2 * C + 16; }
   size_t xmax_off() const { return d_off + dcount() - 16; }
+  size_t coef_foff() const { return 2 * d_off; }
+  size_t gymax_foff() const { return 2 * d_off + 3 * (size_t)C; }
   size_t f_off;
   size_t fz_off = 0;
   float eps = 0.f, mom = 0.f;
@@ -132,6 +134,10 @@
   std::vector<signed char> fz_form;
   long long prep_launches = 0;
   std::vector<char> out_sums;
+  int dy_fold = 1;
+  std::vector<char> gy_max_made;
+  std::vector<const float*> dy_fold_g;
+  long long apply_launches = 0;
 };
 
 static int add_bn(uwm_model* m, const std::string& name, int C, int stage, float eps = 0.f, float mom = 0.f) {
diff --git a/unet-watermark_amd/csrc/wgrad_f16x3.hip b/unet-watermark_amd/csrc/wgrad_f16x3.hip
--- a/unet-watermark_amd/csrc/wgrad_f16x3.hip
+++ b/unet-watermark_amd/csrc/wgrad_f16x3.hip
@@ -35,7 +35,7 @@
   return __builtin_bit_cast(h8, v);
 }
 
-template <int WX, int NP = 3>
+template <int WX, int NP = 3, bool FOLD = false>
 __global__ __launch_bounds__(768, 1) void wgrad_f16x3_kernel(const WgradArgs a, int stages_per_split, int nstages) {
   constexpr int kWR = WG16<WX>::kWR, kWX = WX, kWPW = WG16<WX>::kWPW, kWPH = WG16<WX>::kWPH, kWStage = WG16<WX>::kWStage, kWXRounds = WG16<WX>::kWXRounds;
   constexpr int kKS = 4, kRK = 32 / WX;
@@ -84,7 +84,10 @@
     const bool xhas = s.scale != nullptr;
     if (xhas) { xsc = *(const f4*)(s.scale + cl + xcu * 4); xsh = *(const f4*)(s.shift + cl + xcu * 4); }
     const int xrelu = s.relu;
-    struct Stage { f4 dv[kWDyRounds]; f4 xv[kWXRounds]; unsigned xok; };
+    struct Stage { f4 dv[kWDyRounds]; f4 yv[FOLD ? kWDyRounds : 1]; f4 xv[kWXRounds]; unsigned xok; };
+    f4 cA = {0.f, 0.f, 0.f, 0.f}, cB = cA, cK = cA;
+    if (FOLD && dok) { const float* cf = a.dy_coef + a0 + dcu * 4; cA = *(const f4*)cf; cB = *(const f4*)(cf + a.Cout); cK = *(const f4*)(cf + 2 * a.Cout); }
+    const ptrdiff_t ydel = FOLD ? a.dy_y - a.dy : 0;
     int dgo[kWDyRounds], dlo[kWDyRounds], xpy[kWXRounds], xlo[kWXRounds];
 #pragma unroll
     for (int rd = 0; rd < kWDyRounds; ++rd) {
@@ -109,7 +112,10 @@
       const int y0 = ty * kWR, x0 = tx * kWX;
       const float* const dbase = dyp + (((size_t)n * a.Ho + y0) * a.Wo + x0) * a.Cout;
 #pragma unroll
-      for (int rd = 0; rd < kWDyRounds; ++rd) sg.dv[rd] = dok ? *(const f4*)(dbase + dgo[rd]) : (f4){0.f, 0.f, 0.f, 0.f};
+      for (int rd = 0; rd < kWDyRounds; ++rd) {
+        sg.dv[rd] = dok ? *(const f4*)(dbase + dgo[rd]) : (f4){0.f, 0.f, 0.f, 0.f};
+        if (FOLD) sg.yv[FOLD ? rd : 0] = dok ? *(const f4*)(dbase + dgo[rd] + ydel) : (f4){0.f, 0.f, 0.f, 0.f};
+      }
       sg.xok = 0;
       const int nb = n * s.H;
 #pragma unroll
@@ -135,7 +141,10 @@
       char* const dyb = wsm + buf * kWStage;
       char* const xb = dyb + kWDyB;
 #pragma unroll
-      for (int rd = 0; rd < kWDyRounds; ++rd) split_store(dyb + dlo[rd], dyb + (dlo[rd] ^ 128), sg.dv[rd] * xs, false);
+      for (int rd = 0; rd < kWDyRounds; ++rd) {
+        const f4 dv = FOLD ? bn_dy(sg.dv[rd], sg.yv[FOLD ? rd : 0], cA, cB, cK) : sg.dv[rd];
+        split_store(dyb + dlo[rd], dyb + (dlo[rd] ^ 128), dv * xs, false);
+      }
 #pragma unroll
       for (int rd = 0; rd < kWXRounds; ++rd) {
         if (xpy[rd] >= 0) {
@@ -253,6 +262,13 @@
 static hipError_t launch_wg16p(WgradArgs& a, hipStream_t st, int pairs, int sps, int nstages) {
   const size_t lds = (size_t)2 * WG16<WX>::kWStage;
   static DevOnce lds_attr;
+  if (a.dy_y) {
+    static DevOnce lds_attr_f;
+    { hipError_t e = lds_attr_f.set_max_lds((const void*)wgrad_f16x3_kernel<WX, NP, true>, lds); if (e != hipSuccess) return e; }
+    UWM_LAUNCH(43, a.flops, a.bytes, (wgrad_f16x3_kernel<WX, NP, true>), dim3((unsigned)(pairs * a.nsplit)), dim3(768), lds, st, a, sps, nstages);
+    route_note("(wgrad_f16x3_kernel<WX, NP>)");
+    return hipGetLastError();
+  }
   { hipError_t e = lds_attr.set_max_lds((const void*)wgrad_f16x3_kernel<WX, NP>, lds); if (e != hipSuccess) return e; }
   UWM_LAUNCH(43, a.flops, a.bytes, (wgrad_f16x3_kernel<WX, NP>), dim3((unsigned)(pairs * a.nsplit)), dim3(768), lds, st, a, sps, nstages);
   return hipGetLastError();
@@ -265,7 +281,7 @@
 
 hipError_t launch_wgrad_f16x3(const WgradArgs& a0, hipStream_t st) {
   WgradArgs a = a0;
-  if (!wgrad_f16x3_applicable(a)) return hipErrorInvalidValue;
+  if (!wgrad_f16x3_applicable(a) || (a.dy_y && !a.dy_coef)) return hipErrorInvalidValue;
   const int wx = wgrad_f16x3_wx(a);
   const int pairs = ((a.wrows + 63) / 64) * (a.Ctot / 32);
   const int nstages = a.N * (a.Ho / (128 / wx)) * (a.Wo / wx);
diff --git a/unet-watermark_amd/csrc/wgrad_igemm.hip b/unet-watermark_amd/csrc/wgrad_igemm.hip
--- a/unet-watermark_amd/csrc/wgrad_igemm.hip
+++ b/unet-watermark_amd/csrc/wgrad_igemm.hip
@@ -279,6 +279,7 @@
     fprintf(stderr, "wgrad N=%d Ctot=%d(C0=%d) Cout=%d wrows=%d Ho=%d Wo=%d Hl=%d Wl=%d taps=%d stride=%d wino=%d patch=%d gflop=%.2f\n", a0.N, a0.Ctot,
             a0.C0, a0.Cout, a0.wrows, a0.Ho, a0.Wo, a0.Hl, a0.Wl, a0.ntaps, a0.stride, (int)(wino_mode_of(a0.wino) != 0 && wgrad_wino_applicable(a0)),
             (int)wgrad_patch_applicable(a0), a0.flops * 1e-9);
+  if (a0.dy_y) return (a0.prec == 2 && wgrad_f16x3_applicable(a0)) ? launch_wgrad_f16x3(a0, st) : hipErrorInvalidValue;
   if ((a0.force_igemm & 0xff) == 4) return launch_wgrad_gemm(a0, st);
   static const bool no_up2 = dbg_flag("UWM_NO_UP2") || dbg_flag("UWM_NO_UP2_WGRAD");
   if (((a0.force_igemm & 0xff) == 0 || (a0.force_igemm & 0xff) == 6) && a0.prec == 2 && a0.xmax && !no_up2 && wgrad_up2_applicable(a0) && wgrad_up2_f16_shape(a0))
diff --git a/unet-watermark_amd/model.py b/unet-watermark_amd/model.py
--- a/unet-watermark_amd/model.py
+++ b/unet-watermark_amd/model.py
@@ -261,6 +261,13 @@
     def prep_launches(self) -> int:
         return int(L.lib().uwm_prep_launches(self._h))
 
+    def set_dy_fold(self, on: bool = True):
+        L.check(L.lib().uwm_set_dy_fold(self._h, int(bool(on))))
+        return self
+
+    def apply_launches(self) -> int:
+        return int(L.lib().uwm_apply_launches(self._h))
+
     def train(self, mode: bool = True):
         if mode:
             self.unfreeze()
```

Measured after the change: 1193 images/s, median of 6. About the same (+0.6%).
